# hkchengrex/Cutie

Measured on AMD Instinct MI355X. Metric: frames/sec (480p, 3 objects), higher is better.
Workload: dtype bf16

## Files before the change

cutie_amd/_lib.py:

```python
import ctypes
import os

_HERE = os.path.dirname(os.path.abspath(__file__))
LIB_PATH = os.environ.get('CUTIE_AMD_LIB') or os.path.join(_HERE, 'libcutie_hip.so')
ABI_VERSION = 11
OP_STRUCT_SIZE = 256

_lib = None


class HipLibraryError(RuntimeError):
    pass


def load():
    global _lib
    if _lib is not None:
        return _lib
    if not os.path.exists(LIB_PATH):
        raise HipLibraryError(
            f'{LIB_PATH} not found: build it with `python -c "import __graft_entry__ as g; g.build()"` '
            f'(or `make -C cutie_amd/csrc`).  cutie_amd has no CPU fallback.')
    lib = ctypes.CDLL(LIB_PATH)
    lib.cutie_exec.argtypes = [ctypes.c_void_p, ctypes.c_int, ctypes.c_void_p]
# ... 7 lines not shown
    lib.cutie_graph_destroy.argtypes = [ctypes.c_void_p]
    lib.cutie_graph_destroy.restype = None
    lib.cutie_time_ops.argtypes = [ctypes.c_void_p, ctypes.c_int, ctypes.c_int, ctypes.c_void_p]
    lib.cutie_time_ops.restype = ctypes.c_float
    lib.cutie_hip_last_error.argtypes = []
    lib.cutie_hip_last_error.restype = ctypes.c_char_p
    lib.cutie_hip_abi_version.restype = ctypes.c_int
    lib.cutie_op_struct_size.restype = ctypes.c_int
    lib.cutie_hip_build_flags.restype = ctypes.c_int
    if lib.cutie_hip_abi_version() != ABI_VERSION or lib.cutie_op_struct_size() != OP_STRUCT_SIZE:
        raise HipLibraryError(f'{LIB_PATH} is stale (ABI {lib.cutie_hip_abi_version()}, '
                              f'op size {lib.cutie_op_struct_size()}); rebuild it.')
    _lib = lib
    return lib


EXPORTED_SYMBOLS = ['cutie_exec', 'cutie_exec_one', 'cutie_graph_capture', 'cutie_graph_launch',
                    'cutie_graph_destroy', 'cutie_time_ops', 'cutie_hip_last_error',
                    'cutie_hip_abi_version', 'cutie_op_struct_size', 'cutie_hip_build_flags']


def has_diag_kernels():
    return bool(load().cutie_hip_build_flags() & 1)


def has_png_decode():
    return bool(load().cutie_hip_build_flags() & 2)


def has_jpeg_batch():
    return bool(load().cutie_hip_build_flags() & 4)


def has_mixed_lockstep():
    return bool(load().cutie_hip_build_flags() & 8)


def has_track_stats():
    return bool(load().cutie_hip_build_flags() & 16)


def has_region_filter():
    return bool(load().cutie_hip_build_flags() & 32)


def has_edt_band():
    return bool(load().cutie_hip_build_flags() & 64)


def has_polygons():
    return bool(load().cutie_hip_build_flags() & 128)


class HipExecutor:
    is_mock = False

    def __init__(self):
        import torch
        self.lib = load()
        if not torch.cuda.is_available():
            raise HipLibraryError('no HIP device visible: cutie_amd runs on MI355X only (no CPU fallback).')
        self._torch = torch
        self._raw_stream = getattr(torch._C, '_cuda_getCurrentRawStream', None)
        self.graph_stats = [0, 0]
        self._warned = False

    def stream(self):
        raw = self._raw_stream
        if raw is not None:
            return raw(self._torch.cuda.current_device())
        return self._torch.cuda.current_stream().cuda_stream

    def run(self, arr):
        rc = self.lib.cutie_exec(arr.ctypes.data, len(arr), self.stream())
        if rc != 0:
            raise RuntimeError('cutie_exec failed: ' + self.lib.cutie_hip_last_error().decode())

    def run_on(self, arr, stream):
        rc = self.lib.cutie_exec(arr.ctypes.data, len(arr), stream.cuda_stream)
        if rc != 0:
            raise RuntimeError('cutie_exec failed: ' + self.lib.cutie_hip_last_error().decode())

    GRAPH_CACHE_ENTRIES = 24

    def run_cached(self, arr, cache, head=0):
        if head:
            self.run(arr[:head])
            arr = arr[head:]
        key = arr['p'].tobytes()
        ent = cache.get(key)
        if ent is None:
            if len(cache) >= self.GRAPH_CACHE_ENTRIES:
                old = cache.pop(next(iter(cache)))
                if old not in (0, -1):
                    self.lib.cutie_graph_destroy(old)
            cache[key] = 0
            self.graph_stats[0] += 1
            return self.run(arr)
        if ent == 0:
            ent = self.lib.cutie_graph_capture(arr.ctypes.data, len(arr), self.stream()) or -1
            cache[key] = ent
            if ent == -1 and not self._warned:
                self._warned = True
                import warnings
                warnings.warn('HIP graph capture of a launch plan failed (%s); such plans keep running launch by launch'
                              % self.lib.cutie_hip_last_error().decode())
# ... 28 lines not shown
```

cutie_amd/csrc/api.hip:

```cpp
#include "common.h"
#include <stdarg.h>
#include <stdio.h>
#include <string.h>

static thread_local char g_err[512] = "";

void cutie_set_error(const char* fmt, ...) {
    va_list ap;
    va_start(ap, fmt);
    vsnprintf(g_err, sizeof(g_err), fmt, ap);
    va_end(ap);
}

static int dispatch(const cutie_op* op, hipStream_t s) {
    switch (op->kind) {
        case CUTIE_OP_CONV: return launch_conv(op, s);
        case CUTIE_OP_QUERY_INIT: return (op->flags & 1) ? launch_attention(op, s) : launch_elementwise(op, s);
        case CUTIE_OP_QFFN: return launch_qchain(op, s);
        case CUTIE_OP_STEM: return launch_stem(op, s);
        case CUTIE_OP_ATTN_Q2P: case CUTIE_OP_ATTN_SELF: case CUTIE_OP_ATTN_P2Q:
            return (op->flags & 12) ? launch_qchain(op, s) : launch_attention(op, s);
        case CUTIE_OP_AUX_MASK:
            return launch_attention(op, s);
        case CUTIE_OP_KEY_PREP: case CUTIE_OP_AFF_SCORE: case CUTIE_OP_AFF_SELECT: case CUTIE_OP_AFF_READOUT:
// ... 53 lines not shown
        if (graph) hipGraphDestroy(graph);
        if (rc == 0) cutie_set_error("graph: end capture failed (%d)", (int)e);
        (void)hipGetLastError();
        return nullptr;
    }
    hipGraphExec_t exec = nullptr;
    if (hipGraphInstantiate(&exec, graph, nullptr, nullptr, 0) != hipSuccess) {
        hipGraphDestroy(graph);
        (void)hipGetLastError();
        cutie_set_error("graph: instantiate failed");
        return nullptr;
    }
    GraphHandle* h = new GraphHandle{graph, exec};
    return h;
}

int cutie_graph_launch(void* graph, void* stream) {
    GraphHandle* h = (GraphHandle*)graph;
    if (!h) { cutie_set_error("graph: null handle"); return -4; }
    hipError_t e = hipGraphLaunch(h->exec, (hipStream_t)stream);
    if (e != hipSuccess) { cutie_set_error("graph launch: %s", hipGetErrorString(e)); return -1; }
    return 0;
}

void cutie_graph_destroy(void* graph) {
    GraphHandle* h = (GraphHandle*)graph;
    if (!h) return;
    hipGraphExecDestroy(h->exec);
    hipGraphDestroy(h->graph);
    delete h;
}

float cutie_time_ops(const cutie_op* ops, int n, int iters, void* stream) {
    hipStream_t s = (hipStream_t)stream;
    hipEvent_t a, b;
    if (hipEventCreate(&a) != hipSuccess || hipEventCreate(&b) != hipSuccess) { cutie_set_error("time: event create failed"); return -1.f; }
    if (cutie_exec(ops, n, stream) != 0) return -1.f;
    hipEventRecord(a, s);
    for (int it = 0; it < iters; ++it)
        if (cutie_exec(ops, n, stream) != 0) return -1.f;
    hipEventRecord(b, s);
    hipEventSynchronize(b);
    float ms = 0.f;
    hipEventElapsedTime(&ms, a, b);
    hipEventDestroy(a);
    hipEventDestroy(b);
    return ms / (float)iters;
}

const char* cutie_hip_last_error(void) { return g_err; }
int cutie_hip_abi_version(void) { return 11; }
int cutie_op_struct_size(void) { return (int)sizeof(cutie_op); }
int cutie_hip_build_flags(void) {
    const int forms = 2 | 4 | 8 | 16 | 32 | 64 | 128;
#ifdef CUTIE_DIAG
    return forms | 1;
#else
    return forms;
#endif
}

}
```

cutie_amd/csrc/common.h:

```cpp
#pragma once
#include <hip/hip_runtime.h>
#include <stdint.h>
#include "../../include/cutie_hip.h"

typedef unsigned short bf16_t;
typedef __attribute__((ext_vector_type(8))) __bf16 bf16x8;
typedef __attribute__((ext_vector_type(4))) float f32x4;

__device__ __forceinline__ float bf2f(bf16_t v) { return __uint_as_float(((uint32_t)v) << 16); }

typedef __attribute__((ext_vector_type(2))) __bf16 bf16x2_t;
__device__ __forceinline__ bf16_t f2bf(float f) { return __builtin_bit_cast(bf16_t, (__bf16)f); }

__device__ __forceinline__ uint32_t pack_bf2(float a, float b) {
    const bf16x2_t v = {(__bf16)a, (__bf16)b};
    return __builtin_bit_cast(uint32_t, v);
}

__device__ __forceinline__ uint32_t relu_bf2(uint32_t w) {
    uint32_t neg = (w >> 15) & 0x00010001u;
    return w & ~(neg * 0xffffu);
}

__device__ __forceinline__ float sigmoidf_(float x) { return 1.0f / (1.0f + __expf(-x)); }
// ... 19 lines not shown
    v += __builtin_amdgcn_update_dpp(0, v, 0x141, 0xf, 0xf, false);
    v += __builtin_amdgcn_update_dpp(0, v, 0x140, 0xf, 0xf, false);
    auto r = __builtin_amdgcn_permlane16_swap((unsigned)v, (unsigned)v, false, false);
    const unsigned a = r[0] + r[1];
    auto r2 = __builtin_amdgcn_permlane32_swap(a, a, false, false);
    return (int)(r2[0] + r2[1]);
}

__device__ __forceinline__ float wave_sum(float v) {
#pragma unroll
    for (int o = 32; o > 0; o >>= 1) v += __shfl_xor(v, o, 64);
    return v;
}
__device__ __forceinline__ float wave_sum_dpp(float v) {
    v += __uint_as_float(__builtin_amdgcn_update_dpp(0, (int)__float_as_uint(v), 0xB1, 0xf, 0xf, false));
    v += __uint_as_float(__builtin_amdgcn_update_dpp(0, (int)__float_as_uint(v), 0x4E, 0xf, 0xf, false));
    v += __uint_as_float(__builtin_amdgcn_update_dpp(0, (int)__float_as_uint(v), 0x141, 0xf, 0xf, false));
    v += __uint_as_float(__builtin_amdgcn_update_dpp(0, (int)__float_as_uint(v), 0x140, 0xf, 0xf, false));
    return rows_sum(v);
}
__device__ __forceinline__ float wave_max(float v) {
#pragma unroll
    for (int o = 32; o > 0; o >>= 1) v = fmaxf(v, __shfl_xor(v, o, 64));
    return v;
}

__host__ __device__ __forceinline__ int mixed_count(unsigned word, int clip) { return (int)((word >> (3 * clip)) & 7u); }
__host__ __device__ __forceinline__ int mixed_start(unsigned word, int clip) {
    int s = 0;
    for (int c = 0; c < clip; ++c) s += mixed_count(word, c);
    return s;
}
__host__ __device__ __forceinline__ int mixed_clip_of(unsigned word, int b, int& start) {
    int c = 0, s = 0;
#pragma unroll
    for (int q = 0; q < 7; ++q) {
        const int n = mixed_count(word, c);
        const bool past = b >= s + n;
        s += past ? n : 0;
        c += past ? 1 : 0;
    }
    start = s;
    return c;
}
static inline int mixed_clips(unsigned word, int* objects) {
    int n = 0, total = 0;
    if (word >> 24) { *objects = 0; return 0; }
    while (n < 8 && mixed_count(word, n)) total += mixed_count(word, n++);
    if (n < 8 && (word >> (3 * n))) { *objects = 0; return 0; }
    *objects = total;
    return n;
}

int launch_conv(const cutie_op* op, hipStream_t s);
int launch_elementwise(const cutie_op* op, hipStream_t s);
int launch_attention(const cutie_op* op, hipStream_t s);
int launch_stem(const cutie_op* op, hipStream_t s);
int launch_qchain(const cutie_op* op, hipStream_t s);
int launch_affinity(const cutie_op* op, hipStream_t s);
int launch_bank(const cutie_op* op, hipStream_t s);
int launch_resize_ingest(const cutie_op* op, hipStream_t s);
int launch_jpeg(const cutie_op* op, hipStream_t s);
int launch_png_decode(const cutie_op* op, hipStream_t s);
int launch_png_deflate(const cutie_op* op, int H, int W, hipStream_t s);
int launch_rle_encode(const cutie_op* op, hipStream_t s);
int launch_jf_counts(const cutie_op* op, hipStream_t s);
int launch_jpeg_encode(const cutie_op* op, hipStream_t s);
int launch_matte_composite(const cutie_op* op, hipStream_t s);
int launch_matte_soft(const cutie_op* op, hipStream_t s);
int launch_track_stats(const cutie_op* op, hipStream_t s);
int launch_region_filter(const cutie_op* op, hipStream_t s);
int launch_edt_band(const cutie_op* op, hipStream_t s);
int launch_polygon_trace(const cutie_op* op, hipStream_t s);
void cutie_set_error(const char* fmt, ...);
```

cutie_amd/csrc/conv_igemm.hip:

```cpp
#include "conv_common.h"

template <int BM, int BN, int WM, int WN, int BK, int S, int OCC, int WK>
__global__ __launch_bounds__(WM * WN * WK * 64) void conv_igemm_kernel(ConvParams p) {
    if (p.flags & CUTIE_F_PRIO) __builtin_amdgcn_s_setprio(1);
    constexpr int NTB = WM * WN * WK * 64;
    constexpr int NT = WM * WN * 64;
    constexpr int CPR = BK / 8;
    constexpr int RPT = NT / CPR;
    constexpr int NX = (BM * CPR) / NT;
    constexpr int NWC = (BN * CPR + NT - 1) / NT;
    constexpr int TM = BM / WM / 16;
    constexpr int TN = BN / WN / 16;
    constexpr int KSUB = BK / 32;
    constexpr int NWRAP = BK == 32 ? 4 : BK / 32;
    static_assert((NT == 256 || NT == 512) && NTB <= 1024 && NX >= 1 && TM >= 1 && TN >= 1 && S >= 2 && (BM * CPR) % NT == 0, "bad tile");
    constexpr int LDC = BN + 4;
    constexpr int GRP_CHUNKS = 2 * (BM + BN) * CPR;
    extern __shared__ __attribute__((aligned(16))) u32x4 smem_raw[];
    const int grp = threadIdx.x / NT;
    u32x4 (*smem)[(BM + BN) * CPR] = reinterpret_cast<u32x4 (*)[(BM + BN) * CPR]>(smem_raw + grp * GRP_CHUNKS);

    const int tid = threadIdx.x % NT, lane = tid & 63, wave = tid >> 6;
    int m0, n0;
    {
// ... 400 lines not shown
        if (cl == 0 && x < p.W && oy < p.H) {
            float v = acc + bias0;
            if (act == CUTIE_ACT_RELU) v = fmaxf(v, 0.f);
            else if (act == CUTIE_ACT_SIGMOID) v = sigmoidf_(v);
            else if (act == CUTIE_ACT_SQ1) v = v * v + 1.f;
            const long m = ((long)b * p.H + oy) * p.W + x;
            if (p.flags & CUTIE_F_OUT_F32) reinterpret_cast<float*>(p.y)[m * p.ldy] = v;
            else reinterpret_cast<bf16_t*>(p.y)[m * p.ldy] = f2bf(v);
        }
    }
}

template <int BM, int BN, int WM, int WN, int BK, int S, int OCC, int WK = 1>
static int launch_cfg(ConvParams p, hipStream_t s) {
    if (p.Kpad % BK) { cutie_set_error("conv: Kpad %d not a multiple of BK %d", p.Kpad, BK); return -2; }
    if (BK > 32 && p.Cin < 32) { cutie_set_error("conv: BK %d needs Cin >= 32 (Cin=%d)", BK, p.Cin); return -2; }
    const int nk_all = p.Kpad / BK;
    if (p.splitk > nk_all) { cutie_set_error("conv: splitk %d > K tiles %d", p.splitk, nk_all); return -2; }
    if (nk_all % (p.splitk * WK)) { cutie_set_error("conv: splitk %d x %d K groups must divide the %d K tiles", p.splitk, WK, nk_all); return -2; }
    p.Kslice = p.Kpad / p.splitk;
    constexpr int lds = conv_lds_bytes<BM, BN, BK, WK>();
    static bool attr_set = false;
    if (!attr_set) {
        if (lds > 65536 && hipFuncSetAttribute(reinterpret_cast<const void*>(conv_igemm_kernel<BM, BN, WM, WN, BK, S, OCC, WK>),
                                               hipFuncAttributeMaxDynamicSharedMemorySize, lds) != hipSuccess) {
            cutie_set_error("conv: cannot raise the dynamic LDS limit to %d bytes", lds);
            return -2;
        }
        attr_set = true;
    }
    dim3 grid((p.M + BM - 1) / BM, (p.Cout + BN - 1) / BN, p.splitk);
    hipLaunchKernelGGL((conv_igemm_kernel<BM, BN, WM, WN, BK, S, OCC, WK>), grid, dim3(WM * WN * WK * 64), lds, s, p);
    if (p.splitk > 1) {
        const long nq = (long)p.M * (p.ldp >> 3);
        hipLaunchKernelGGL(conv_splitk_reduce_kernel, dim3((unsigned)((nq + 255) / 256)), dim3(256), 0, s, p);
    }
    return (int)hipGetLastError();
}

int launch_conv(const cutie_op* op, hipStream_t s) {
    ConvParams p;
    p.x1 = (const bf16_t*)op->p[0]; p.x2 = (const bf16_t*)op->p[1]; p.w = (const bf16_t*)op->p[2];
    p.bias = (const float*)op->p[3]; p.res = (const bf16_t*)op->p[4]; p.y = (void*)op->p[5];
    const int32_t* i = op->i;
    p.B = i[0]; p.H = i[1]; p.W = i[2]; p.C1 = i[3]; p.C2 = i[4]; p.ldx1 = i[5]; p.ldx2 = i[6];
    p.OH = i[7]; p.OW = i[8]; p.Cout = i[9]; p.ldy = i[10]; p.KH = i[11]; p.KW = i[12];
    p.stride = i[13]; p.pad = i[14]; p.ldr = i[15]; p.Kpad = i[16];
    p.flags = op->flags; p.OHW = p.OH * p.OW; p.M = p.B * p.OHW; p.Cin = p.C1 + p.C2;
    p.splitk = i[19] > 1 ? i[19] : 1; p.part = (float*)op->p[6];
    p.ldp = (p.Cout + 7) & ~7;
    p.gap = (long long*)op->p[7]; p.zero = (unsigned long long*)op->p[8]; p.nzero = i[21];
    p.pf = (const unsigned char*)op->p[9]; p.pf_bytes = op->p[9] ? i[22] : 0;
    p.pf2 = (const unsigned char*)op->p[10]; p.pf2_bytes = op->p[10] ? i[23] : 0;
    p.res_grp_rows = p.res_grp_stride = 0;
    if ((p.flags & CUTIE_F_RES_BCAST) && op->f[0] > 0.f) {
        const int kg = (int)op->f[0];
        if (kg <= 0 || p.B % kg || op->f[1] < (float)p.OHW || op->f[1] != (float)(int)op->f[1]) { cutie_set_error("conv: residual groups of %d objects do not divide B = %d (or stride %g < OH*OW)", kg, p.B, (double)op->f[1]); return -2; }
        p.res_grp_rows = kg * p.OHW; p.res_grp_stride = (int)op->f[1];
    }
    if ((p.gap || p.zero) && (i[17] < 60 || i[17] >= 200 || ((p.flags & CUTIE_F_OUT_F32) && p.gap) || (p.Cout & 7) || (p.ldy & 7) || (p.res && (p.ldr & 7)))) {
        cutie_set_error("conv: GAP accumulation / zero job need an LDS-DMA tile (60..199), bf16 output, Cout %% 8 == 0 (tile %d)", i[17]);
        return -2;
    }
    if (p.splitk > 1 && (!p.part || (long)p.splitk * p.M * p.ldp > (long)i[20] * 1024)) {
        cutie_set_error("conv: split-K %d needs the fp32 partial scratch (p6, capacity i20 KiB-floats)", p.splitk);
        return -2;
    }
    if ((p.C1 & 7) || (p.C2 & 7) || (p.ldx1 & 7) || (p.C2 && (p.ldx2 & 7)) || (p.Kpad & 31) ||
        p.Kpad < p.KH * p.KW * p.Cin || p.M <= 0 || p.Cout <= 0) {
        cutie_set_error("conv: bad geometry C1=%d C2=%d ldx1=%d ldx2=%d Kpad=%d M=%d Cout=%d",
                        p.C1, p.C2, p.ldx1, p.ldx2, p.Kpad, p.M, p.Cout);
        return -2;
    }
    if (i[17] == 19) {
        const int LP = p.Cin >> 3;
        if (p.Cout != 1 || p.C2 != 0 || p.res || LP > 64 || (LP & (LP - 1)) || LP < 1) {
            cutie_set_error("conv cout1: needs Cout=1, single source, no residual, Cin/8 a power of two <= 64 (Cin=%d)", p.Cin);
            return -2;
        }
        const int ppb = 256 / LP;
        if (!(p.flags & CUTIE_F_PLAIN) && p.KH == 3 && p.KW == 3 && p.stride == 1 && p.pad == 1 && p.OH == p.H && p.OW == p.W && LP >= 8 && LP <= 32 && p.H * p.W >= 4096) {
            if (LP == 16 && !(p.flags & CUTIE_F_TILE_OFF)) {
                constexpr int TR = 8;
                const int blocks = p.B * ((p.H + TR - 1) / TR) * ((p.W + 15) / 16);
                hipLaunchKernelGGL(conv_cout1_tile_kernel<TR>, dim3(blocks), dim3(256), 0, s, p);
                return (int)hipGetLastError();
            }
            constexpr int R = 4;
            const int blocks = p.B * ((p.H + R - 1) / R) * ((p.W + ppb - 1) / ppb);
            hipLaunchKernelGGL(conv_cout1_rows_kernel<R>, dim3(blocks), dim3(256), 0, s, p);
            return (int)hipGetLastError();
        }
        hipLaunchKernelGGL(conv_cout1_kernel, dim3((p.M + ppb - 1) / ppb), dim3(256), (size_t)p.KH * p.KW * LP * 16, s, p);
        return (int)hipGetLastError();
    }
    if (i[17] >= 60 && i[17] < 90) return launch_conv_dma(p, i[17], s);
    if (i[17] >= 100 && i[17] < 200) return launch_conv_pc(p, i[17], s);
    switch (i[17]) {
        case 0: return launch_cfg<128, 128, 2, 2, 32, 4, 2>(p, s);
        case 1: return launch_cfg<128, 64, 2, 2, 32, 4, 3>(p, s);
        case 2: return launch_cfg<64, 64, 2, 2, 32, 4, 4>(p, s);
        case 3: return launch_cfg<256, 16, 4, 1, 32, 4, 3>(p, s);
        case 4: return launch_cfg<64, 128, 2, 2, 32, 4, 3>(p, s);
        case 5: return launch_cfg<64, 64, 2, 2, 64, 4, 3>(p, s);
        case 6: return launch_cfg<64, 128, 2, 2, 64, 3, 2>(p, s);
        case 7: return launch_cfg<128, 128, 2, 2, 64, 2, 2>(p, s);
// ... 26 lines not shown
```

cutie_amd/csrc/conv_pc.hip:

```cpp
#include "conv_common.h"

typedef __amdgpu_buffer_rsrc_t rsrc_t;
#define PC_WORD3 0x00020000
#define PC_RECORDS 0x7fffffff
#define PC_OOB 0x80000000u
#define LDS_PTR(p) ((__attribute__((address_space(3))) void*)(p))
#define PC_WAIT_VM(N) __builtin_amdgcn_s_waitcnt(((N) & 15) | (((N) >> 4) << 14) | (7 << 4) | (15 << 8))
#define PC_WAIT_LGKM0() __builtin_amdgcn_s_waitcnt(15 | (3 << 14) | (7 << 4) | (0 << 8))
#define PC_BARRIER() { asm volatile("" ::: "memory"); __builtin_amdgcn_s_barrier(); asm volatile("" ::: "memory"); }
#ifdef PC_ABL_NO_LOOPBAR
#define PC_LOOP_BARRIER() { asm volatile("" ::: "memory"); }
#else
#define PC_LOOP_BARRIER() PC_BARRIER()
#endif
#ifdef PC_ABL_NO_WAIT
#define PC_LOOP_WAIT_VM(N) ((void)0)
#else
#define PC_LOOP_WAIT_VM(N) PC_WAIT_VM(N)
#endif
#ifdef PC_ABL_SAME_TILE
#define PC_SAME_TILE_GUARD(...)
#else
#define PC_SAME_TILE_GUARD(...) __VA_ARGS__
#endif
// ... 477 lines not shown
                        case 6: if constexpr (NXP > 6) PCH_XPIECE(NXP > 6 ? 6 : 0, sl + 1) break;
                        default: if constexpr (NXP > 7) PCH_XPIECE(NXP > 7 ? 7 : 0, sl + 1) break;
                    }
                }
                PCH_WTILE()
                TL(4)
                const int xin = NS == 3 ? xp : xp + xprev;
                if (xin == 0) { PC_LOOP_WAIT_VM((NS - 2) * NWI); } else if (xin == 1) { PC_LOOP_WAIT_VM((NS - 2) * NWI + 1); } else { PC_LOOP_WAIT_VM((NS - 2) * NWI + 2); }
                TL(5)
                PC_LOOP_BARRIER()
                xprev = xp;
                ++tap;
                if (tap == 9) { tap = 0; ++sl; }
            }
            for (; kt < nk; ++kt) {
                PC_WAIT_VM(0);
                PC_LOOP_BARRIER()
            }
            } else {
            static_assert(NXP <= 8 && NP <= 3, "pair steps: two patch pieces per iteration over four iterations");
            int t = nk < NS - 1 ? nk : NS - 1;
            const int P = (nk + 1) >> 1;
            int ps = 0, pk = 0, pnext = 5;
            int u = 0;
            for (; 2 * (u + NP - 1) + 1 < nk; ++u) {
                TL(3)
                if (u == pnext) { ++ps; pk = 0; pnext += (ps & 1) ? 4 : 5; }
                if (ps + 1 < nslice && pk < 4) {
                    switch (pk) {
                        case 0: if constexpr (NXP > 0) PCH_XPIECE(0, ps + 1) if constexpr (NXP > 1) PCH_XPIECE(NXP > 1 ? 1 : 0, ps + 1) break;
                        case 1: if constexpr (NXP > 2) PCH_XPIECE(NXP > 2 ? 2 : 0, ps + 1) if constexpr (NXP > 3) PCH_XPIECE(NXP > 3 ? 3 : 0, ps + 1) break;
                        case 2: if constexpr (NXP > 4) PCH_XPIECE(NXP > 4 ? 4 : 0, ps + 1) if constexpr (NXP > 5) PCH_XPIECE(NXP > 5 ? 5 : 0, ps + 1) break;
                        default: if constexpr (NXP > 6) PCH_XPIECE(NXP > 6 ? 6 : 0, ps + 1) if constexpr (NXP > 7) PCH_XPIECE(NXP > 7 ? 7 : 0, ps + 1) break;
                    }
                    ++pk;
                }
                for (; t <= 2 * (u + NP - 1) + 1; ++t) PCH_WTILE()
                TL(4)
                PC_LOOP_WAIT_VM((NP - 2) * 2 * NWI);
                TL(5)
                PC_LOOP_BARRIER()
            }
            for (; u < P; ++u) {
                for (; t < nk && t <= 2 * (u + NP - 1) + 1; ++t) PCH_WTILE()
                PC_WAIT_VM(0);
                PC_LOOP_BARRIER()
            }
            }
#undef PCH_WTILE
#undef PCH_XPIECE
        }
        TLE(6)
        TL_DUMP(logical, nb, NC + NPW)
        if (p.pf_bytes > 0) {
            const int id = blockIdx.y * gridDim.x + blockIdx.x;
            const int nbx = (nb + 7) >> 3, kq = id >> 3;
            u32x4 t = {0u, 0u, 0u, 0u};
#pragma unroll
            for (int r = 0; r < 2; ++r) {
                const unsigned char* base = r ? p.pf2 : p.pf;
                const int bytes = r ? p.pf2_bytes : p.pf_bytes;
                const int chunk = (((bytes + nbx - 1) / nbx) + 1023) & ~1023;
                const int b0 = kq * chunk, b1 = min(b0 + chunk, bytes & ~15);
                for (int o = b0 + (pw * 64 + lane) * 16; o < b1; o += NPW * 1024)
                    asm volatile("global_load_dwordx4 %0, %1, off" : "+v"(t) : "v"(base + o) : "memory");
            }
            asm volatile("s_waitcnt vmcnt(0)" : "+v"(t) :: "memory");
        }
        return;
    }

    const int wm = wave / WN, wn = wave % WN;
    const int pm0 = wm * (BM / WM), cn0 = wn * (BN / WN);
    int mrow[TM];
    bool mval[TM];
    int xbase[TM];
#pragma unroll
    for (int b = 0; b < TM; ++b) {
        const int q = pm0 + b * 16 + l15;
        if (HALO) {
            const int qq = q < TH * TW ? q : TH * TW - 1;
            const int qy = qq / TW, qx = qq - qy * TW;
            const int gy = ty0 + qy, gx = tx0 + qx;
            mval[b] = q < TH * TW && gy < p.H && gx < p.W;
            mrow[b] = (bimg * p.H + min(gy, p.H - 1)) * p.W + min(gx, p.W - 1);
            xbase[b] = qy * PW + qx;
        } else {
            mrow[b] = m0 + q;
            mval[b] = mrow[b] < p.M;
            xbase[b] = 0;
        }
    }
    TL(11)
    const bool out_f32 = p.flags & CUTIE_F_OUT_F32;
    const bool vec_ok = (out_f32 ? (p.ldy & 3) == 0 : (p.ldy & (NCH - 1)) == 0) && (!p.res || (p.ldr & (NCH - 1)) == 0);
    float bias[TNP][NCH];
    const float* const bias_p = p.bias ? p.bias : reinterpret_cast<const float*>(p.w);
    const int bias_lim = p.bias ? p.Cout : 0;
    typedef const __attribute__((address_space(1))) float* pc_gf32;
    const pc_gf32 bias_g = (pc_gf32)bias_p;
#pragma unroll
    for (int a = 0; a < TNP; ++a) {
        const int ch0 = n0 + cn0 + a * (PAIR ? 32 : 16) + l4 * NCH;
#pragma unroll
        for (int r = 0; r < NCH; ++r) {
            const float t = bias_g[min(ch0 + r, p.Cout - 1)];
            bias[a][r] = ch0 + r < bias_lim ? t : 0.f;
        }
    }
    unsigned rpre[PRE_RES ? TM : 1][PRE_RES ? TNP : 1][NCH / 2];
    const bool have_res = PRE_RES && p.res && vec_ok;
    if (PRE_RES) {
#pragma unroll
        for (int b = 0; b < TM; ++b)
#pragma unroll
            for (int a = 0; a < TNP; ++a) {
                const int ch0 = n0 + cn0 + a * (PAIR ? 32 : 16) + l4 * NCH;
#pragma unroll
                for (int r = 0; r < NCH / 2; ++r) rpre[b][a][r] = 0u;
                if (have_res && mval[b] && ch0 + NCH <= p.Cout) {
                    const int mres = pc_res_row(p, mrow[b]);
// ... 289 lines not shown
```

cutie_amd/csrc/elementwise.hip:

```cpp
#include "common.h"
#include <math.h>

#define GRID1D(n, bs) dim3((unsigned)(((long)(n) + (bs) - 1) / (bs)))
__global__ void memset32_kernel(uint32_t* d, long n, uint32_t v);

__global__ void maxpool_kernel(const uint4* __restrict__ x, uint4* __restrict__ y, int B, int H, int W, int C8,
                               int OH, int OW, int relu) {
    long idx = (long)blockIdx.x * blockDim.x + threadIdx.x;
    long total = (long)B * OH * OW * C8;
    if (idx >= total) return;
    int c = idx % C8; long t = idx / C8;
    int ow = t % OW; t /= OW; int oh = t % OH; int b = t / OH;
    float m[8];
#pragma unroll
    for (int i = 0; i < 8; ++i) m[i] = relu ? 0.f : -INFINITY;
    for (int dy = 0; dy < 3; ++dy) {
        int ih = oh * 2 - 1 + dy;
        if ((unsigned)ih >= (unsigned)H) continue;
        for (int dx = 0; dx < 3; ++dx) {
            int iw = ow * 2 - 1 + dx;
            if ((unsigned)iw >= (unsigned)W) continue;
            uint4 v = x[(((long)b * H + ih) * W + iw) * C8 + c];
            uint32_t u[4] = {v.x, v.y, v.z, v.w};
#pragma unroll
            for (int i = 0; i < 4; ++i) {
                m[2 * i] = fmaxf(m[2 * i], __uint_as_float(u[i] << 16));
                m[2 * i + 1] = fmaxf(m[2 * i + 1], __uint_as_float(u[i] & 0xffff0000u));
            }
        }
    }
    y[idx] = make_uint4(pack_bf2(m[0], m[1]), pack_bf2(m[2], m[3]), pack_bf2(m[4], m[5]), pack_bf2(m[6], m[7]));
}

__global__ void img_prep_kernel(const float* __restrict__ img, const float* __restrict__ masks, uint4* __restrict__ y,
                                int h0, int w0, int H, int W, int pl, int pt, int K,
                                float m0, float m1, float m2, float s0, float s1, float s2) {
    long idx = (long)blockIdx.x * blockDim.x + threadIdx.x;
    long HW = (long)H * W;
    if (idx >= HW * K) return;
    int k = idx / HW; long pix = idx - (long)k * HW;
    int yy = pix / W, xx = pix - (long)yy * W;
    int sy = yy - pt, sx = xx - pl;
    float r = 0.f, g = 0.f, b = 0.f;
    if ((unsigned)sy < (unsigned)h0 && (unsigned)sx < (unsigned)w0) {
        long o = (long)sy * w0 + sx, plane = (long)h0 * w0;
        r = img[o]; g = img[plane + o]; b = img[2 * plane + o];
    }
    r = (r - m0) / s0; g = (g - m1) / s1; b = (b - m2) / s2;
    float mk = 0.f, others = 0.f;
    if (masks) {
        float sum = 0.f;
        for (int j = 0; j < K; ++j) sum += masks[(long)j * HW + pix];
        mk = masks[(long)k * HW + pix];
        others = fminf(fmaxf(sum - mk, 0.f), 1.f);
    }
    y[idx] = make_uint4(pack_bf2(r, g), pack_bf2(b, mk), pack_bf2(others, 0.f), 0u);
}

__device__ __forceinline__ void up_coord(int o, int n_in, float scale, int& i0, int& i1, float& lam) {
    float src = ((float)o + 0.5f) * scale - 0.5f;
    if (src < 0.f) src = 0.f;
    i0 = (int)src;
    if (i0 > n_in - 1) i0 = n_in - 1;
    i1 = i0 + (i0 < n_in - 1 ? 1 : 0);
    lam = src - (float)i0;
}

template <bool MIXED = false>
__global__ void upsample2x_add_kernel(const uint4* __restrict__ g, const uint4* __restrict__ skip, uint4* __restrict__ y,
                                      int B, int h, int w, int C8, int Kg, long gstride, int prio) {
    if (prio) __builtin_amdgcn_s_setprio(1);
    long idx = (long)blockIdx.x * blockDim.x + threadIdx.x;
    int OH = 2 * h, OW = 2 * w;
    long total = (long)B * OH * OW * C8;
    if (idx >= total) return;
    int c = idx % C8; long t = idx / C8;
    int ox = t % OW; t /= OW; int oy = t % OH; int b = t / OH;
    int y0, y1, x0, x1; float ly, lx;
    up_coord(oy, h, 0.5f, y0, y1, ly);
    up_coord(ox, w, 0.5f, x0, x1, lx);
    const uint4* gb = g + (long)b * h * w * C8;
    uint4 v00 = gb[((long)y0 * w + x0) * C8 + c], v01 = gb[((long)y0 * w + x1) * C8 + c];
    uint4 v10 = gb[((long)y1 * w + x0) * C8 + c], v11 = gb[((long)y1 * w + x1) * C8 + c];
    long grp;
    if (MIXED) { int st; grp = mixed_clip_of((unsigned)Kg, b, st); }
    else grp = Kg > 0 ? b / Kg : 0;
    uint4 sk = skip[(grp * gstride + (long)oy * OW + ox) * C8 + c];
    const uint32_t* a = &v00.x; const uint32_t* bq = &v01.x; const uint32_t* cq = &v10.x; const uint32_t* d = &v11.x;
    const uint32_t* s = &sk.x;
    float w00 = (1.f - ly) * (1.f - lx), w01 = (1.f - ly) * lx, w10 = ly * (1.f - lx), w11 = ly * lx;
    uint32_t out[4];
#pragma unroll
    for (int i = 0; i < 4; ++i) {
        float lo = w00 * __uint_as_float(a[i] << 16) + w01 * __uint_as_float(bq[i] << 16) +
                   w10 * __uint_as_float(cq[i] << 16) + w11 * __uint_as_float(d[i] << 16) + __uint_as_float(s[i] << 16);
        float hi = w00 * __uint_as_float(a[i] & 0xffff0000u) + w01 * __uint_as_float(bq[i] & 0xffff0000u) +
                   w10 * __uint_as_float(cq[i] & 0xffff0000u) + w11 * __uint_as_float(d[i] & 0xffff0000u) +
                   __uint_as_float(s[i] & 0xffff0000u);
        out[i] = pack_bf2(lo, hi);
    }
    y[idx] = make_uint4(out[0], out[1], out[2], out[3]);
}

template <int R = 0>
__device__ __forceinline__ void area_down_bf16_body(const bf16_t* __restrict__ x, bf16_t* __restrict__ y, int B, int H, int W, int C,
                                                    int ldx, int ldy, int rrt, long idx) {
    const int r = R > 0 ? R : rrt;
    int C8 = C >> 3, OH = H / r, OW = W / r;
    long total = (long)B * OH * OW * C8;
    if (idx >= total) return;
    int c = idx % C8; long t = idx / C8;
    int ox = t % OW; t /= OW; int oy = t % OH; int b = t / OH;
    float acc[8] = {0, 0, 0, 0, 0, 0, 0, 0};
    if (R > 0) {
        uint4 v[R > 0 ? R * R : 1];
#pragma unroll
        for (int dy = 0; dy < R; ++dy)
#pragma unroll
            for (int dx = 0; dx < R; ++dx)
                v[dy * R + dx] = *reinterpret_cast<const uint4*>(x + (((long)b * H + oy * R + dy) * W + ox * R + dx) * ldx + c * 8);
#pragma unroll
        for (int e = 0; e < R * R; ++e) {
            const uint32_t* u = &v[e].x;
#pragma unroll
            for (int i = 0; i < 4; ++i) {
                acc[2 * i] += __uint_as_float(u[i] << 16);
                acc[2 * i + 1] += __uint_as_float(u[i] & 0xffff0000u);
            }
        }
    } else
    for (int dy = 0; dy < r; ++dy)
        for (int dx = 0; dx < r; ++dx) {
            const uint4 v = *reinterpret_cast<const uint4*>(x + (((long)b * H + oy * r + dy) * W + ox * r + dx) * ldx + c * 8);
            const uint32_t* u = &v.x;
#pragma unroll
            for (int i = 0; i < 4; ++i) {
                acc[2 * i] += __uint_as_float(u[i] << 16);
                acc[2 * i + 1] += __uint_as_float(u[i] & 0xffff0000u);
            }
        }
    float inv = 1.f / (float)(r * r);
    uint4 o = make_uint4(pack_bf2(acc[0] * inv, acc[1] * inv), pack_bf2(acc[2] * inv, acc[3] * inv),
                         pack_bf2(acc[4] * inv, acc[5] * inv), pack_bf2(acc[6] * inv, acc[7] * inv));
    *reinterpret_cast<uint4*>(y + (((long)b * OH + oy) * OW + ox) * ldy + c * 8) = o;
}
__global__ void area_down_bf16_kernel(const bf16_t* __restrict__ x, bf16_t* __restrict__ y, int B, int H, int W, int C,
                                      int ldx, int ldy, int r) {
    area_down_bf16_body(x, y, B, H, W, C, ldx, ldy, r, (long)blockIdx.x * blockDim.x + threadIdx.x);
}

template <int R = 0>
__device__ __forceinline__ void area_down_f32_body(const float* __restrict__ x, bf16_t* __restrict__ y, int B, int H, int W, int C,
                                                   int ldx, int ldy, int rrt, int Cz, long idx) {
    const int r = R > 0 ? R : rrt;
    int OH = H / r, OW = W / r;
    long total = (long)B * OH * OW;
    if (idx >= total) return;
    int ox = idx % OW; long t = idx / OW; int oy = t % OH; int b = t / OH;
    float inv = 1.f / (float)(r * r);
    bf16_t* yp = y + idx * ldy;
    for (int c = 0; c < C; ++c) {
        float acc = 0.f;
        if (R > 0) {
            float v[R > 0 ? R * R : 1];
#pragma unroll
            for (int dy = 0; dy < R; ++dy)
#pragma unroll
                for (int dx = 0; dx < R; ++dx) v[dy * R + dx] = x[(((long)b * H + oy * R + dy) * W + ox * R + dx) * ldx + c];
#pragma unroll
            for (int e = 0; e < R * R; ++e) acc += v[e];
        } else
        for (int dy = 0; dy < r; ++dy)
            for (int dx = 0; dx < r; ++dx) acc += x[(((long)b * H + oy * r + dy) * W + ox * r + dx) * ldx + c];
        yp[c] = f2bf(acc * inv);
    }
    for (int c = C; c < Cz; ++c) yp[c] = 0;
}
__global__ void area_down_f32_kernel(const float* __restrict__ x, bf16_t* __restrict__ y, int B, int H, int W, int C,
                                     int ldx, int ldy, int r, int Cz) {
    area_down_f32_body(x, y, B, H, W, C, ldx, ldy, r, Cz, (long)blockIdx.x * blockDim.x + threadIdx.x);
}
struct AreaSeg { const void* x; bf16_t* y; int B, H, W, C, ldx, ldy, r, Cz, f32; long n; };
struct Area3 { AreaSeg s[3]; int rt; int prio; };
__global__ void area_down3_kernel(Area3 a) {
    const int prio = a.prio;
    if (prio) __builtin_amdgcn_s_setprio(1);
    long idx = (long)blockIdx.x * blockDim.x + threadIdx.x;
#pragma unroll
    for (int q = 0; q < 3; ++q) {
        const AreaSeg& g = a.s[q];
        if (idx < g.n) {
            const int rr = a.rt ? 0 : g.r;
            if (g.f32) {
                if (rr == 2) area_down_f32_body<2>((const float*)g.x, g.y, g.B, g.H, g.W, g.C, g.ldx, g.ldy, 2, g.Cz, idx);
                else if (rr == 4) area_down_f32_body<4>((const float*)g.x, g.y, g.B, g.H, g.W, g.C, g.ldx, g.ldy, 4, g.Cz, idx);
                else area_down_f32_body<0>((const float*)g.x, g.y, g.B, g.H, g.W, g.C, g.ldx, g.ldy, g.r, g.Cz, idx);
            } else {
                if (rr == 2) area_down_bf16_body<2>((const bf16_t*)g.x, g.y, g.B, g.H, g.W, g.C, g.ldx, g.ldy, 2, idx);
                else if (rr == 4) area_down_bf16_body<4>((const bf16_t*)g.x, g.y, g.B, g.H, g.W, g.C, g.ldx, g.ldy, 4, idx);
                else area_down_bf16_body<0>((const bf16_t*)g.x, g.y, g.B, g.H, g.W, g.C, g.ldx, g.ldy, g.r, idx);
            }
            return;
        }
        idx -= g.n;
    }
}

__global__ void mask_down_mean_kernel(const float* __restrict__ m, float* __restrict__ m16, int K, int H, int W, int r) {
    int h = H / r, w = W / r;
    long idx = (long)blockIdx.x * (blockDim.x >> 6) + (threadIdx.x >> 6);
    int lane = threadIdx.x & 63;
    if (idx >= (long)K * h * w) return;
    int ox = idx % w; long t = idx / w; int oy = t % h; int k = t / h;
    float acc = 0.f;
    for (int e = lane; e < r * r; e += 64) {
        int dy = e / r, dx = e - dy * r;
        acc += m[((long)k * H + oy * r + dy) * W + ox * r + dx];
    }
    acc = wave_sum(acc);
    if (lane == 0) m16[idx] = acc / (float)(r * r);
}
__global__ void mask_down_pair_kernel(const float* __restrict__ m, float* __restrict__ m16, uint4* __restrict__ y, int K, int H, int W, int r,
                                      int ld8) {
    const int h = H / r, w = W / r, hw = h * w;
    const long px = (long)blockIdx.x * (blockDim.x >> 6) + (threadIdx.x >> 6);
    const int lane = threadIdx.x & 63;
    if (px >= hw) return;
    const int ox = px % w, oy = px / w;
    float sum = 0.f;
    for (int k0 = 0; k0 < K; k0 += 4) {
        float acc[4] = {0.f, 0.f, 0.f, 0.f};
        for (int e = lane; e < r * r; e += 64) {
            const int dy = e / r, dx = e - dy * r;
            float v[4];
#pragma unroll
            for (int u = 0; u < 4; ++u) v[u] = m[((long)min(k0 + u, K - 1) * H + oy * r + dy) * W + ox * r + dx];
#pragma unroll
            for (int u = 0; u < 4; ++u) acc[u] += v[u];
        }
#pragma unroll
        for (int u = 0; u < 4; ++u) {
            if (k0 + u >= K) break;
            const float a = wave_sum(acc[u]) / (float)(r * r);
            sum += a;
            if (lane == 0) m16[(long)(k0 + u) * hw + px] = a;
        }
    }
    if (lane == 0)
        for (int k = 0; k < K; ++k) {
            const float mk = m16[(long)k * hw + px];
            const float others = fminf(fmaxf(sum - mk, 0.f), 1.f);
            y[((long)k * hw + px) * ld8] = make_uint4(pack_bf2(mk, others), 0u, 0u, 0u);
        }
}
__global__ void mask_pair_kernel(const float* __restrict__ m16, uint4* __restrict__ y, int K, int hw) {
    long idx = (long)blockIdx.x * blockDim.x + threadIdx.x;
    if (idx >= (long)K * hw) return;
    int k = idx / hw; int p = idx - (long)k * hw;
    float sum = 0.f;
    for (int j = 0; j < K; ++j) sum += m16[(long)j * hw + p];
    float mk = m16[idx];
    float others = fminf(fmaxf(sum - mk, 0.f), 1.f);
    y[idx] = make_uint4(pack_bf2(mk, others), 0u, 0u, 0u);
}

__global__ __launch_bounds__(256) void gap_partial_kernel(const bf16_t* __restrict__ x, float* __restrict__ part, int HW, int C) {
    __shared__ float red[2048 + 32];
    const int b = blockIdx.y, p0 = blockIdx.x * 64;
    const int C8 = C >> 3;
    const int c8 = threadIdx.x % C8, rg = threadIdx.x / C8, nrg = 256 / C8;
    float acc[8] = {0, 0, 0, 0, 0, 0, 0, 0};
    for (int r = rg; r < 64; r += nrg) {
        int p = p0 + r;
        if (p < HW) {
            uint4 v = *reinterpret_cast<const uint4*>(x + ((long)b * HW + p) * C + c8 * 8);
            acc[0] += __uint_as_float(v.x << 16); acc[1] += __uint_as_float(v.x & 0xffff0000u);
            acc[2] += __uint_as_float(v.y << 16); acc[3] += __uint_as_float(v.y & 0xffff0000u);
            acc[4] += __uint_as_float(v.z << 16); acc[5] += __uint_as_float(v.z & 0xffff0000u);
            acc[6] += __uint_as_float(v.w << 16); acc[7] += __uint_as_float(v.w & 0xffff0000u);
        }
    }
#pragma unroll
    for (int i = 0; i < 8; ++i) red[rg * (C + 1) + c8 * 8 + i] = acc[i];
    __syncthreads();
    for (int c = threadIdx.x; c < C; c += 256) {
        float sum = 0.f;
        for (int g = 0; g < nrg; ++g) sum += red[g * (C + 1) + c];
        part[((long)b * gridDim.x + blockIdx.x) * C + c] = sum;
    }
}
__global__ void gap_final_kernel(const float* __restrict__ part, float* __restrict__ y, int nchunk, int C, float inv) {
    const int b = blockIdx.x;
    for (int c = threadIdx.x; c < C; c += blockDim.x) {
        float sum = 0.f;
        for (int k = 0; k < nchunk; ++k) sum += part[((long)b * nchunk + k) * C + c];
        y[(long)b * C + c] = sum * inv;
    }
}

__global__ __launch_bounds__(256) void eca_apply_kernel(const bf16_t* __restrict__ x, const float* __restrict__ part,
                                                        const float* __restrict__ wk, const bf16_t* __restrict__ r,
                                                        bf16_t* __restrict__ y, float* __restrict__ gap_out, int HW, int C, int nchunk,
                                                        const long long* __restrict__ fixed, const bf16_t* __restrict__ pw,
                                                        const float* __restrict__ pb, float* __restrict__ plog, int prio) {
    if (prio) __builtin_amdgcn_s_setprio(1);
    __shared__ float gap[256 + 4], sc[256];
    const int b = blockIdx.y, tid = threadIdx.x;
    const float inv = 1.f / (float)HW;
    const int C8 = C >> 3;
    const int p0 = blockIdx.x * 32;
    uint4 xv[4], rv[4];
    long offs[4];
#pragma unroll
    for (int it = 0; it < 4; ++it) {
        const int q = tid + it * 256;
        const int pp = q / C8, c8 = q - pp * C8, p = p0 + pp;
        const bool ok = q < 32 * C8 && p < HW;
        offs[it] = ok ? ((long)b * HW + p) * C + c8 * 8 : -1;
        const long o = ok ? offs[it] : 0;
        xv[it] = *reinterpret_cast<const uint4*>(x + o);
        rv[it] = *reinterpret_cast<const uint4*>(r + o);
    }
    if (fixed) {
        for (int c = tid; c < C; c += 256) {
            const float mean = (float)((double)fixed[(long)b * C + c] * (1.0 / 16777216.0)) * inv;
            gap[c + 2] = mean;
            if (gap_out && blockIdx.x == 0) gap_out[(long)b * C + c] = mean;
        }
    } else
    for (int c = tid; c < C; c += 256) {
        float sum = 0.f;
        for (int k0 = 0; k0 < nchunk; k0 += 8) {
            float v[8];
#pragma unroll
            for (int u = 0; u < 8; ++u) v[u] = part[((long)b * nchunk + min(k0 + u, nchunk - 1)) * C + c];
#pragma unroll
            for (int u = 0; u < 8; ++u) sum += k0 + u < nchunk ? v[u] : 0.f;
        }
        gap[c + 2] = sum * inv;
        if (gap_out && blockIdx.x == 0) gap_out[(long)b * C + c] = sum * inv;
    }
    if (tid < 2) { gap[tid] = 0.f; gap[C + 2 + tid] = 0.f; }
    __syncthreads();
    for (int c = tid; c < C; c += 256) {
        float a = wk[0] * gap[c] + wk[1] * gap[c + 1] + wk[2] * gap[c + 2] + wk[3] * gap[c + 3] + wk[4] * gap[c + 4];
        sc[(c & 7) * 32 + (c >> 3)] = sigmoidf_(a);
    }
    __syncthreads();
#pragma unroll
    for (int it = 0; it < 4; ++it) {
        if (offs[it] < 0) continue;
        const int q = tid + it * 256;
        const int c8 = q % C8;
        const uint32_t* xu = &xv[it].x; const uint32_t* ru = &rv[it].x;
        uint32_t o[4];
#pragma unroll
        for (int i = 0; i < 4; ++i) {
            float lo = __uint_as_float(xu[i] << 16) * sc[(2 * i) * 32 + c8] + __uint_as_float(ru[i] << 16);
            float hi = __uint_as_float(xu[i] & 0xffff0000u) * sc[(2 * i + 1) * 32 + c8] + __uint_as_float(ru[i] & 0xffff0000u);
            o[i] = pack_bf2(lo, hi);
        }
        *reinterpret_cast<uint4*>(y + offs[it]) = make_uint4(o[0], o[1], o[2], o[3]);
    }
    if (pw) {
        const int c8 = tid & 31;
        const uint4 wv = *reinterpret_cast<const uint4*>(pw + c8 * 8);
        const uint32_t* wu = &wv.x;
        const float bias = pb ? pb[0] : 0.f;
#pragma unroll
        for (int it = 0; it < 4; ++it) {
            float part = 0.f;
            if (offs[it] >= 0) {
                const uint32_t* xu = &xv[it].x; const uint32_t* ru = &rv[it].x;
#pragma unroll
                for (int i = 0; i < 4; ++i) {
                    const float lo = __uint_as_float(xu[i] << 16) * sc[(2 * i) * 32 + c8] + __uint_as_float(ru[i] << 16);
                    const float hi = __uint_as_float(xu[i] & 0xffff0000u) * sc[(2 * i + 1) * 32 + c8] + __uint_as_float(ru[i] & 0xffff0000u);
                    const uint32_t st = pack_bf2(lo, hi);
                    part += fmaxf(__uint_as_float(st << 16), 0.f) * __uint_as_float(wu[i] << 16);
                    part += fmaxf(__uint_as_float(st & 0xffff0000u), 0.f) * __uint_as_float(wu[i] & 0xffff0000u);
                }
            }
            part += __uint_as_float(__builtin_amdgcn_update_dpp(0, (int)__float_as_uint(part), 0xB1, 0xf, 0xf, false));
            part += __uint_as_float(__builtin_amdgcn_update_dpp(0, (int)__float_as_uint(part), 0x4E, 0xf, 0xf, false));
            part += __uint_as_float(__builtin_amdgcn_update_dpp(0, (int)__float_as_uint(part), 0x141, 0xf, 0xf, false));
            part += __uint_as_float(__builtin_amdgcn_update_dpp(0, (int)__float_as_uint(part), 0x140, 0xf, 0xf, false));
            const unsigned pu = __float_as_uint(part);
            const auto rr = __builtin_amdgcn_permlane16_swap(pu, pu, false, false);
            const float tot = __uint_as_float(rr[0]) + __uint_as_float(rr[1]);
            const int q = tid + it * 256, p = p0 + q / C8;
            if (c8 == 0 && offs[it] >= 0) plog[(long)b * HW + p] = tot + bias;
        }
    }
}

__global__ void gru4_kernel(const float* __restrict__ v, float* __restrict__ h, bf16_t* __restrict__ hb, long n, int C, int prio) {
    if (prio) __builtin_amdgcn_s_setprio(1);
    const long idx = (long)blockIdx.x * blockDim.x + threadIdx.x;
    const int C4 = C >> 2;
    if (idx >= n * C4) return;
    const long row = idx / C4; const int c = (int)(idx - row * C4) * 4;
    const float* vr = v + row * 3 * C + c;
    const float4 f4 = *reinterpret_cast<const float4*>(vr), u4 = *reinterpret_cast<const float4*>(vr + C), n4 = *reinterpret_cast<const float4*>(vr + 2 * C);
    const float4 h4 = *reinterpret_cast<const float4*>(h + row * C + c);
    const float fa[4] = {f4.x, f4.y, f4.z, f4.w}, ua[4] = {u4.x, u4.y, u4.z, u4.w}, na[4] = {n4.x, n4.y, n4.z, n4.w}, ha[4] = {h4.x, h4.y, h4.z, h4.w};
    float o[4];
#pragma unroll
    for (int i = 0; i < 4; ++i) {
        const float f = sigmoidf_(fa[i]), u = sigmoidf_(ua[i]), nv = tanhf(na[i]);
        o[i] = f * ha[i] * (1.f - u) + u * nv;
    }
    *reinterpret_cast<float4*>(h + row * C + c) = make_float4(o[0], o[1], o[2], o[3]);
    *reinterpret_cast<uint2*>(hb + row * C + c) = make_uint2(pack_bf2(o[0], o[1]), pack_bf2(o[2], o[3]));
}

__global__ void gru_kernel(const float* __restrict__ v, float* __restrict__ h, bf16_t* __restrict__ hb, long n, int C) {
    long idx = (long)blockIdx.x * blockDim.x + threadIdx.x;
    if (idx >= n * C) return;
    long row = idx / C; int c = idx - row * C;
    const float* vr = v + row * 3 * C;
    float f = sigmoidf_(vr[c]), u = sigmoidf_(vr[C + c]), nv = tanhf(vr[2 * C + c]);
    float nh = f * h[idx] * (1.f - u) + u * nv;
    h[idx] = nh;
    hb[idx] = f2bf(nh);
}

__device__ __forceinline__ float clamp_logit(float p) {
    p = fminf(fmaxf(p, 1e-7f), 1.f - 1e-7f);
    return logf(p / (1.f - p));
}

__global__ void seg_agg_kernel(const float* __restrict__ lg, float* __restrict__ agg, int K, int hw) {
    int p = blockIdx.x * blockDim.x + threadIdx.x;
    if (p >= hw) return;
    float bg = 1.f;
    for (int k = 0; k < K; ++k) {
        float pr = 1.f / (1.f + expf(-lg[(long)k * hw + p]));
        bg *= (1.f - pr);
        agg[(long)(k + 1) * hw + p] = clamp_logit(pr);
    }
    agg[p] = clamp_logit(bg);
}

__global__ void up4_softmax_kernel(const float* __restrict__ agg, float* __restrict__ prob, float* __restrict__ lup,
                                   int P, int h, int w) {
    int OH = 4 * h, OW = 4 * w;
    long idx = (long)blockIdx.x * blockDim.x + threadIdx.x;
    if (idx >= (long)OH * OW) return;
    int ox = idx % OW, oy = idx / OW;
    int y0, y1, x0, x1; float ly, lx;
    up_coord(oy, h, 0.25f, y0, y1, ly);
    up_coord(ox, w, 0.25f, x0, x1, lx);
    float w00 = (1.f - ly) * (1.f - lx), w01 = (1.f - ly) * lx, w10 = ly * (1.f - lx), w11 = ly * lx;
    long o00 = (long)y0 * w + x0, o01 = (long)y0 * w + x1, o10 = (long)y1 * w + x0, o11 = (long)y1 * w + x1;
    long hw = (long)h * w, OHW = (long)OH * OW;
    float mx = -INFINITY;
    for (int c = 0; c < P; ++c) {
        const float* a = agg + c * hw;
        float v = w00 * a[o00] + w01 * a[o01] + w10 * a[o10] + w11 * a[o11];
        if (lup) lup[c * OHW + idx] = v;
        mx = fmaxf(mx, v);
    }
    float sum = 0.f;
    for (int c = 0; c < P; ++c) {
        const float* a = agg + c * hw;
        float v = w00 * a[o00] + w01 * a[o01] + w10 * a[o10] + w11 * a[o11];
// ... 214 lines not shown
    float lo[PMAX][4];
    if (SH) {
        if (lane < 36) {
            const int sly = lane / 6, slx = lane - sly * 6;
            const long o = (long)min(max(4 * cy - 1 + sly, 0), h - 1) * w + min(max(4 * cx - 1 + slx, 0), w - 1);
            float raw[PMAX - 1], Lp[PMAX];
#pragma unroll
            for (int k = 0; k < PMAX - 1; ++k)
                if (k < K) raw[k] = lg[(long)k * h * w + o];
            up4_src<PMAX>(raw, K, Lp);
#pragma unroll
            for (int p = 0; p < PMAX; ++p)
                if (p <= K) srcw[p * 36 + lane] = Lp[p];
        }
        __builtin_amdgcn_wave_barrier();
        __builtin_amdgcn_s_waitcnt(0xc07f);
        __builtin_amdgcn_wave_barrier();
    }
    up4_four<PMAX, KC, SH>(lg, K, h, w, oy, j, out, lo, srcw, 4 * cy - 1, 4 * cx - 1);
    const long base = (long)oy * OW + 4 * j;
#pragma unroll
    for (int p = 0; p < PMAX; ++p)
        if (p <= K) {
            if (lup) *reinterpret_cast<float4*>(lup + p * OHW + base) = make_float4(lo[p][0], lo[p][1], lo[p][2], lo[p][3]);
            *reinterpret_cast<float4*>(prob + p * OHW + base) = make_float4(out[p][0], out[p][1], out[p][2], out[p][3]);
            if (p >= 1) *reinterpret_cast<float4*>(&cellw[(p - 1) * 256 + r * 16 + 4 * q4]) = make_float4(out[p][0], out[p][1], out[p][2], out[p][3]);
        }
    __builtin_amdgcn_wave_barrier();
    __builtin_amdgcn_s_waitcnt(0xc07f);
    float sum = 0.f, mk[PMAX - 1];
#pragma unroll
    for (int k = 0; k < PMAX - 1; ++k)
        if (k < K) {
            float acc = 0.f;
#pragma unroll
            for (int i = 0; i < 4; ++i) acc += cellw[k * 256 + lane + 64 * i];
            const float a = wave_sum(acc) / 256.f;
            sum += a;
            mk[k] = a;
        }
    if (lane == 0) {
#pragma unroll
        for (int k = 0; k < PMAX - 1; ++k)
            if (k < K) {
                m16[(long)k * ncell + cid] = mk[k];
                const float others = fminf(fmaxf(sum - mk[k], 0.f), 1.f);
                pair[((long)k * ncell + cid) * ld8] = make_uint4(pack_bf2(mk[k], others), 0u, 0u, 0u);
            }
    }
}

template <int PMAX, int KC = 0, bool SH = false>
__global__ __launch_bounds__(256) void up4_softmax_md_kernel(const float* __restrict__ lg, float* __restrict__ prob, float* __restrict__ lup,
                                                             int Krt, int h, int w, float* __restrict__ m16, uint4* __restrict__ pair, int ld8, int prio) {
    if (prio) __builtin_amdgcn_s_setprio(1);
    const int K = KC > 0 ? KC : Krt;
    __shared__ float cell[4][PMAX - 1][256];
    __shared__ float srcL[4][SH ? PMAX : 1][36];
    const int OH = 4 * h, OW = 4 * w, ch = OH >> 4, cw = OW >> 4, ncell = ch * cw;
    const int wave = threadIdx.x >> 6, lane = threadIdx.x & 63;
    const int cid = blockIdx.x * 4 + wave;
    if (cid >= ncell) return;
    {
        const long cl = blockIdx.y;
        lg += cl * K * h * w; prob += cl * (K + 1) * (long)OH * OW;
        if (lup) lup += cl * (K + 1) * (long)OH * OW;
        m16 += cl * K * ncell; pair += cl * K * ncell * ld8;
    }
    const int cy = cid / cw, cx = cid - cy * cw;
    const int r = lane >> 2, q4 = lane & 3;
    const int oy = cy * 16 + r, j = cx * 4 + q4;
    const long OHW = (long)OH * OW;
    float out[PMAX][4];
    float lo[PMAX][4];
    if (SH) {
        if (lane < 36) {
            const int sly = lane / 6, slx = lane - sly * 6;
            const long o = (long)min(max(4 * cy - 1 + sly, 0), h - 1) * w + min(max(4 * cx - 1 + slx, 0), w - 1);
            float raw[PMAX - 1], Lp[PMAX];
#pragma unroll
            for (int k = 0; k < PMAX - 1; ++k)
                if (k < K) raw[k] = lg[(long)k * h * w + o];
            up4_src<PMAX>(raw, K, Lp);
#pragma unroll
            for (int p = 0; p < PMAX; ++p)
                if (p <= K) srcL[wave][SH ? p : 0][lane] = Lp[p];
        }
        __builtin_amdgcn_wave_barrier();
        __builtin_amdgcn_s_waitcnt(0xc07f);
        __builtin_amdgcn_wave_barrier();
    }
    up4_four<PMAX, KC, SH>(lg, K, h, w, oy, j, out, lo, &srcL[wave][0][0], 4 * cy - 1, 4 * cx - 1);
    const long base = (long)oy * OW + 4 * j;
#pragma unroll
    for (int p = 0; p < PMAX; ++p)
        if (p <= K) {
            if (lup) *reinterpret_cast<float4*>(lup + p * OHW + base) = make_float4(lo[p][0], lo[p][1], lo[p][2], lo[p][3]);
            *reinterpret_cast<float4*>(prob + p * OHW + base) = make_float4(out[p][0], out[p][1], out[p][2], out[p][3]);
            if (p >= 1) *reinterpret_cast<float4*>(&cell[wave][p - 1][r * 16 + 4 * q4]) = make_float4(out[p][0], out[p][1], out[p][2], out[p][3]);
        }
    __builtin_amdgcn_wave_barrier();
    __builtin_amdgcn_s_waitcnt(0xc07f);
    float sum = 0.f, mk[PMAX - 1];
#pragma unroll
    for (int k = 0; k < PMAX - 1; ++k)
        if (k < K) {
            float acc = 0.f;
#pragma unroll
            for (int i = 0; i < 4; ++i) acc += cell[wave][k][lane + 64 * i];
            const float a = wave_sum(acc) / 256.f;
            sum += a;
            mk[k] = a;
        }
    if (lane == 0) {
#pragma unroll
        for (int k = 0; k < PMAX - 1; ++k)
            if (k < K) {
                m16[(long)k * ncell + cid] = mk[k];
                const float others = fminf(fmaxf(sum - mk[k], 0.f), 1.f);
                pair[((long)k * ncell + cid) * ld8] = make_uint4(pack_bf2(mk[k], others), 0u, 0u, 0u);
            }
    }
}

template <int PMAX, bool SH>
__global__ __launch_bounds__(256) void up4_softmax_md_mixed_kernel(const float* __restrict__ lg, float* __restrict__ prob, float* __restrict__ lup,
                                                                   unsigned counts, int h, int w, float* __restrict__ m16, uint4* __restrict__ pair, int ld8, int prio) {
    if (prio) __builtin_amdgcn_s_setprio(1);
    __shared__ float cell[4][PMAX - 1][256];
    __shared__ float srcL[4][SH ? PMAX : 1][36];
    const int cl = blockIdx.y, Kc = mixed_count(counts, cl), st = mixed_start(counts, cl);
    const long ncell = (long)(h >> 2) * (w >> 2), OHW = (long)16 * h * w;
    lg += (long)st * h * w; prob += (long)(st + cl) * OHW;
    if (lup) lup += (long)(st + cl) * OHW;
    m16 += (long)st * ncell; pair += (long)st * ncell * ld8;
    const int wave = threadIdx.x >> 6;
#define UP4_BODY_(KC) up4_md_body<PMAX, KC, SH>(lg, prob, lup, KC, h, w, m16, pair, ld8, &cell[wave][0][0], &srcL[wave][0][0])
    UP4_MIXED_SWITCH(UP4_BODY_)
#undef UP4_BODY_
}

__global__ void mask_merge_kernel(const void* __restrict__ inmask, const float* __restrict__ pred, const int* __restrict__ src,
                                  float* __restrict__ planes, int h0, int w0, int H, int W, int pl, int pt, int Knew,
                                  int Kold, int nfloat, int fmode) {
    long idx = (long)blockIdx.x * blockDim.x + threadIdx.x;
    long HW = (long)H * W;
    if (idx >= HW) return;
    int yy = idx / W, xx = idx - (long)yy * W;
    int sy = yy - pt, sx = xx - pl;
    bool inside = (unsigned)sy < (unsigned)h0 && (unsigned)sx < (unsigned)w0;
    long so = (long)sy * w0 + sx, plane = (long)h0 * w0;
    int iv = 0; bool covered = false;
    if (!fmode) {
        iv = inside ? ((const int*)inmask)[so] : 0;
        covered = iv > 0;
    } else {
        float mx = 0.f;
        if (inside) { mx = -INFINITY; for (int c = 0; c < nfloat; ++c) mx = fmaxf(mx, ((const float*)inmask)[c * plane + so]); }
        covered = mx > 0.5f;
    }
    for (int t = 0; t < Knew; ++t) {
        int s = src[t];
        float v;
        if (s >= 0) {
            if (!fmode) v = (iv == s) ? 1.f : 0.f;
            else v = inside ? ((const float*)inmask)[s * plane + so] : 0.f;
        } else {
            v = (pred && t < Kold && !covered) ? pred[(long)(t + 1) * HW + idx] : 0.f;
        }
        planes[(long)t * HW + idx] = v;
    }
}

__global__ void agg_softmax_kernel(const float* __restrict__ planes, float* __restrict__ prob, int K, long HW) {
    long p = (long)blockIdx.x * blockDim.x + threadIdx.x;
// ... 453 lines not shown
            for (int k = 0; k < 4; ++k) {
                const int ox = min(ox0 + k, OW - 1);
                const float fx = fmaxf((ox + 0.5f) * sx - 0.5f, 0.f);
                const int x0 = min((int)fx, W - 1), x1 = min(x0 + 1, W - 1);
                const float lx = fx - (float)x0;
                const float a = r0[x0], b = r0[x1], cc = r1[x0], d = r1[x1];
                const float v = (1.f - ly) * ((1.f - lx) * a + lx * b) + ly * ((1.f - lx) * cc + lx * d);
                sum[k] += (int)(uint8_t)(int)(v * 255.f);
            }
        }
#pragma unroll
        for (int k = 0; k < 4; ++k)
            if (q == 0 || sum[k] > best[k]) { best[k] = sum[k]; arg[k] = q; }
    }
    OUT* o = out + (long)oy * OW + ox0;
    if constexpr (sizeof(OUT) == 1) {
        if (packed) {
            *(uint32_t*)o = (uint32_t)(uint8_t)lut[arg[0]] | (uint32_t)(uint8_t)lut[arg[1]] << 8 | (uint32_t)(uint8_t)lut[arg[2]] << 16 |
                            (uint32_t)(uint8_t)lut[arg[3]] << 24;
            return;
        }
    } else {
        if (packed) {
            *(int4*)o = make_int4(lut[arg[0]], lut[arg[1]], lut[arg[2]], lut[arg[3]]);
            return;
        }
    }
#pragma unroll
    for (int k = 0; k < 4; ++k)
        if (ox0 + k < OW) o[k] = (OUT)lut[arg[k]];
}

int launch_elementwise(const cutie_op* op, hipStream_t s) {
    const int32_t* i = op->i;
    const uint64_t* p = op->p;
    const int BS = 256;
    const int PRIO = (op->flags & CUTIE_F_PRIO) ? 1 : 0;
    switch (op->kind) {
        case CUTIE_OP_MAXPOOL: {
            int C8 = i[3] / 8;
            long n = (long)i[0] * i[4] * i[5] * C8;
            hipLaunchKernelGGL(maxpool_kernel, GRID1D(n, BS), dim3(BS), 0, s, (const uint4*)p[0], (uint4*)p[1], i[0], i[1], i[2], C8, i[4], i[5], op->flags & 1);
            break;
        }
        case CUTIE_OP_IMG_PREP: {
            int K = p[1] ? i[6] : 1;
            long n = (long)i[2] * i[3] * K;
            hipLaunchKernelGGL(img_prep_kernel, GRID1D(n, BS), dim3(BS), 0, s, (const float*)p[0], (const float*)p[1], (uint4*)p[2],
                               i[0], i[1], i[2], i[3], i[4], i[5], K, op->f[0], op->f[1], op->f[2], op->f[3], op->f[4], op->f[5]);
            break;
        }
        case CUTIE_OP_UPSAMPLE2X_ADD: {
            int C8 = i[3] / 8;
            long n = (long)i[0] * 4 * i[1] * i[2] * C8;
            if (i[6]) {
                int objs; const int nc = mixed_clips((unsigned)i[6], &objs);
                if (nc < 1 || objs != i[0] || i[4] != 0 || i[5] < 4 * i[1] * i[2]) { cutie_set_error("upsample2x_add (mixed form): the counts 0x%x do not add up to B = %d (or i4 != 0, or the stride is below one map)", i[6], i[0]); return -2; }
                hipLaunchKernelGGL(upsample2x_add_kernel<true>, GRID1D(n, BS), dim3(BS), 0, s, (const uint4*)p[0], (const uint4*)p[1], (uint4*)p[2], i[0], i[1], i[2], C8, i[6], (long)i[5], PRIO);
                break;
            }
            if (i[4] < 0 || (i[4] > 0 && (i[0] % i[4] || i[5] < 4 * i[1] * i[2]))) { cutie_set_error("upsample2x_add: skip groups of %d objects do not divide B = %d (or their stride is below one map)", i[4], i[0]); return -2; }
            hipLaunchKernelGGL(upsample2x_add_kernel<false>, GRID1D(n, BS), dim3(BS), 0, s, (const uint4*)p[0], (const uint4*)p[1], (uint4*)p[2], i[0], i[1], i[2], C8, i[4], (long)i[5], PRIO);
            break;
        }
        case CUTIE_OP_AREA_DOWN: {
            int r = i[6];
            long np = (long)i[0] * (i[1] / r) * (i[2] / r);
            if (op->flags & 1)
                hipLaunchKernelGGL(area_down_f32_kernel, GRID1D(np, BS), dim3(BS), 0, s, (const float*)p[0], (bf16_t*)p[1], i[0], i[1], i[2], i[3], i[4], i[5], r, i[7]);
            else
                hipLaunchKernelGGL(area_down_bf16_kernel, GRID1D(np * (i[3] / 8), BS), dim3(BS), 0, s, (const bf16_t*)p[0], (bf16_t*)p[1], i[0], i[1], i[2], i[3], i[4], i[5], r);
            break;
        }
        case CUTIE_OP_AREA_DOWN3: {
            Area3 a;
            long total = 0;
            for (int q = 0; q < 3; ++q) {
                const int32_t* j = i + 8 * q;
                AreaSeg& g = a.s[q];
                g.x = (const void*)p[2 * q]; g.y = (bf16_t*)p[2 * q + 1];
                g.B = j[0]; g.H = j[1]; g.W = j[2]; g.C = j[3]; g.ldx = j[4]; g.ldy = j[5]; g.r = j[6]; g.Cz = j[7];
                g.f32 = (op->flags >> q) & 1;
                if (g.r < 1 || (!g.f32 && (g.C & 7))) { cutie_set_error("area_down3: segment %d: r >= 1, C %% 8 for bf16 input", q); return -2; }
                const long np = (long)g.B * (g.H / g.r) * (g.W / g.r);
                g.n = g.f32 ? np : np * (g.C / 8);
                total += g.n;
            }
            a.rt = (op->flags >> 3) & 1;
            a.prio = PRIO;
            hipLaunchKernelGGL(area_down3_kernel, GRID1D(total, BS), dim3(BS), 0, s, a);
            break;
        }
        case CUTIE_OP_MASK_DOWN: {
            int K = i[0], r = i[3], h = i[1] / r, w = i[2] / r;
            long n = (long)K * h * w;
            float* m16 = (float*)p[2];
            if (!m16) { cutie_set_error("mask_down: m16 buffer required"); return -2; }
            hipLaunchKernelGGL(mask_down_pair_kernel, GRID1D((long)h * w * 64, BS), dim3(BS), 0, s, (const float*)p[0], m16, (uint4*)p[1], K, i[1], i[2], r,
                               i[4] > 8 ? i[4] / 8 : 1);
            break;
        }
        case CUTIE_OP_GAP: {
            if (i[2] > 256 || (i[2] & 7) || 256 % (i[2] / 8)) { cutie_set_error("gap: C must divide 256 octet-wise (C=%d)", i[2]); return -2; }
            if (!p[2]) { cutie_set_error("gap: scratch buffer required"); return -2; }
            int nchunk = (i[1] + 63) / 64;
            hipLaunchKernelGGL(gap_partial_kernel, dim3(nchunk, i[0]), dim3(256), 0, s, (const bf16_t*)p[0], (float*)p[2], i[1], i[2]);
            if (!(op->flags & 1))
                hipLaunchKernelGGL(gap_final_kernel, dim3(i[0]), dim3(256), 0, s, (const float*)p[2], (float*)p[1], nchunk, i[2], 1.f / (float)i[1]);
            break;
        }
        case CUTIE_OP_ECA_APPLY: {
            if (i[2] > 256 || (i[2] & 7)) { cutie_set_error("eca: C <= 256, C %% 8"); return -2; }
            if (p[6] && (i[2] != 256 || !p[8])) { cutie_set_error("eca: the fused 1x1 head needs C = 256 and an output"); return -2; }
            int nchunk = (i[1] + 63) / 64;
            hipLaunchKernelGGL(eca_apply_kernel, dim3((i[1] + 31) / 32, i[0]), dim3(256), 0, s, (const bf16_t*)p[0], (const float*)p[5], (const float*)p[2],
                               (const bf16_t*)p[3], (bf16_t*)p[4], (float*)p[1], i[1], i[2], nchunk, (op->flags & 1) ? (const long long*)p[5] : nullptr,
                               (const bf16_t*)p[6], (const float*)p[7], (float*)p[8], PRIO);
            break;
        }
        case CUTIE_OP_GRU: {
            long n = (long)i[0] * i[1];
            if (!(op->flags & 1) && (i[1] & 3) == 0 && (((uintptr_t)p[0] | (uintptr_t)p[1]) & 15) == 0 && ((uintptr_t)p[2] & 7) == 0)
                hipLaunchKernelGGL(gru4_kernel, GRID1D(n / 4, BS), dim3(BS), 0, s, (const float*)p[0], (float*)p[1], (bf16_t*)p[2], (long)i[0], i[1], PRIO);
            else
                hipLaunchKernelGGL(gru_kernel, GRID1D(n, BS), dim3(BS), 0, s, (const float*)p[0], (float*)p[1], (bf16_t*)p[2], (long)i[0], i[1]);
            break;
        }
        case CUTIE_OP_SEG_AGG:
            hipLaunchKernelGGL(seg_agg_kernel, GRID1D(i[1], BS), dim3(BS), 0, s, (const float*)p[0], (float*)p[1], i[0], i[1]);
            break;
        case CUTIE_OP_UP4_SOFTMAX: {
            long n = (long)16 * i[1] * i[2];
            if (op->flags & 1) {
                if (i[0] > 16) { cutie_set_error("up4_softmax: the fused form holds P <= 16 planes in registers (P=%d)", i[0]); return -2; }
                const bool vec = !(op->flags & 2) && i[0] <= 8 && (((uintptr_t)p[1] | (uintptr_t)p[2]) & 15) == 0;
                const int nclip = i[4] > 1 ? i[4] : 1;
                if (nclip > 1 && !vec) { cutie_set_error("up4_softmax: several clips per launch need the four-pixel form (P <= 8, aligned outputs)"); return -2; }
                if (i[5]) {
                    int objs; const int nc = mixed_clips((unsigned)i[5], &objs);
                    if (nc < 1 || nc != i[4] || !vec || (op->flags & 8)) { cutie_set_error("up4_softmax (mixed form): %d clips in the counts 0x%x, i4 = %d; needs the four-pixel form with compile-time object counts", nc, i[5], i[4]); return -2; }
                    if (op->flags & 4) {
                        if (!p[3] || !p[4] || (i[1] & 3) || (i[2] & 3) || i[3] < 8 || (i[3] & 7)) { cutie_set_error("up4_softmax: the mask-down form needs h, w multiples of 4, m16 and pair"); return -2; }
                        const int ncell = (i[1] / 4) * (i[2] / 4);
                        if (op->flags & 16)
                            hipLaunchKernelGGL((up4_softmax_md_mixed_kernel<8, false>), dim3((ncell + 3) / 4, nc), dim3(256), 0, s, (const float*)p[0], (float*)p[1], (float*)p[2], (unsigned)i[5],
                                               i[1], i[2], (float*)p[3], (uint4*)p[4], i[3] / 8, PRIO);
                        else
                            hipLaunchKernelGGL((up4_softmax_md_mixed_kernel<8, true>), dim3((ncell + 3) / 4, nc), dim3(256), 0, s, (const float*)p[0], (float*)p[1], (float*)p[2], (unsigned)i[5],
                                               i[1], i[2], (float*)p[3], (uint4*)p[4], i[3] / 8, PRIO);
                    } else {
                        const long n4 = (long)4 * i[1] * i[2];
                        hipLaunchKernelGGL(up4_softmax_fused4_mixed_kernel<8>, dim3((unsigned)((n4 + BS - 1) / BS), nc), dim3(BS), 0, s, (const float*)p[0], (float*)p[1], (float*)p[2], (unsigned)i[5], i[1], i[2], PRIO);
                    }
                    break;
                }
                if (op->flags & 4) {
                    if (!vec || !p[3] || !p[4] || (i[1] & 3) || (i[2] & 3) || i[3] < 8 || (i[3] & 7)) { cutie_set_error("up4_softmax: the mask-down form needs P <= 8, h, w multiples of 4, m16 and pair"); return -2; }
                    const int ncell = (i[1] / 4) * (i[2] / 4);
#define UP4_MD_(KC, SH) hipLaunchKernelGGL((up4_softmax_md_kernel<8, KC, SH>), dim3((ncell + 3) / 4, nclip), dim3(256), 0, s, (const float*)p[0], (float*)p[1], (float*)p[2], i[0] - 1, \
                                       i[1], i[2], (float*)p[3], (uint4*)p[4], i[3] / 8, PRIO)
#define UP4_MD(KC) { if (op->flags & 16) UP4_MD_(KC, false); else UP4_MD_(KC, true); }
                    switch ((op->flags & 8) ? 0 : i[0] - 1) {
                        case 1: UP4_MD(1); break; case 2: UP4_MD(2); break; case 3: UP4_MD(3); break; case 4: UP4_MD(4); break;
                        case 5: UP4_MD(5); break; case 6: UP4_MD(6); break; case 7: UP4_MD(7); break; default: UP4_MD(0); break;
                    }
#undef UP4_MD
#undef UP4_MD_
                    break;
                }
                if (vec) {
                    const long n4 = (long)4 * i[1] * i[2];
#define UP4_F4(KC) hipLaunchKernelGGL((up4_softmax_fused4_kernel<8, KC>), dim3((unsigned)((n4 + BS - 1) / BS), nclip), dim3(BS), 0, s, (const float*)p[0], (float*)p[1], (float*)p[2], i[0] - 1, i[1], i[2], PRIO)
                    switch ((op->flags & 8) ? 0 : i[0] - 1) {
                        case 1: UP4_F4(1); break; case 2: UP4_F4(2); break; case 3: UP4_F4(3); break; case 4: UP4_F4(4); break;
                        case 5: UP4_F4(5); break; case 6: UP4_F4(6); break; case 7: UP4_F4(7); break; default: UP4_F4(0); break;
                    }
#undef UP4_F4
                    break;
                }
                if (i[0] <= 8) hipLaunchKernelGGL(up4_softmax_fused_kernel<8>, GRID1D(n, BS), dim3(BS), 0, s, (const float*)p[0], (float*)p[1], (float*)p[2], i[0] - 1, i[1], i[2]);
                else hipLaunchKernelGGL(up4_softmax_fused_kernel<16>, GRID1D(n, BS), dim3(BS), 0, s, (const float*)p[0], (float*)p[1], (float*)p[2], i[0] - 1, i[1], i[2]);
                break;
            }
            hipLaunchKernelGGL(up4_softmax_kernel, GRID1D(n, BS), dim3(BS), 0, s, (const float*)p[0], (float*)p[1], (float*)p[2], i[0], i[1], i[2]);
            break;
        }
        case CUTIE_OP_MASK_MERGE: {
            long n = (long)i[2] * i[3];
            hipLaunchKernelGGL(mask_merge_kernel, GRID1D(n, BS), dim3(BS), 0, s, (const void*)p[0], (const float*)p[1], (const int*)p[2], (float*)p[3],
                               i[0], i[1], i[2], i[3], i[4], i[5], i[6], i[7], i[8], op->flags & 1);
            break;
        }
        case CUTIE_OP_AGG_SOFTMAX:
            hipLaunchKernelGGL(agg_softmax_kernel, GRID1D(i[1], BS), dim3(BS), 0, s, (const float*)p[0], (float*)p[1], i[0], (long)i[1]);
            break;
        case CUTIE_OP_LINEAR: {
            if ((i[2] & 7) || (i[3] & 3) || i[2] < 256) { cutie_set_error("linear: Kd %% 8, ldx %% 4, Kd >= 256 required (Kd=%d)", i[2]); return -2; }
            const int add_rows = i[5] > 0 ? i[5] : 1;
            const bool ln = op->flags & 2;
            if (ln && (i[2] != 256 || !p[6] || !p[7] || (i[3] & 3))) { cutie_set_error("linear: fused LayerNorm needs Kd == 256, gamma and beta"); return -2; }
            if ((ln || i[6] > 0) && (i[2] & 127)) { cutie_set_error("linear: LayerNorm / add_cols need Kd %% 128 == 0"); return -2; }
            if (i[6] > 0 && (i[6] & 15)) { cutie_set_error("linear: add_cols must be a multiple of 16"); return -2; }
            if ((i[2] & 511) == 0 && i[2] >= 1024 && !ln)
                hipLaunchKernelGGL(linear_mfma_kernel<16>, dim3((i[1] + 15) / 16, (i[0] + 15) / 16), dim3(1024), 0, s, (const float*)p[0], (const float*)p[1], (const bf16_t*)p[2],
                                   (const float*)p[3], (const float*)p[4], (float*)p[5], i[0], i[1], i[2], i[3], i[4], add_rows, op->flags & 1, i[6],
                                   (const float*)nullptr, (const float*)nullptr, (float*)nullptr, 1e-5f);
            else if ((i[2] & 127) == 0)
                hipLaunchKernelGGL(linear_mfma_kernel<4>, dim3((i[1] + 15) / 16, (i[0] + 15) / 16), dim3(256), 0, s, (const float*)p[0], (const float*)p[1], (const bf16_t*)p[2],
                                   (const float*)p[3], (const float*)p[4], (float*)p[5], i[0], i[1], i[2], i[3], i[4], add_rows, op->flags & 1, i[6],
                                   ln ? (const float*)p[6] : nullptr, (const float*)p[7], (float*)p[8], op->f[0] > 0.f ? op->f[0] : 1e-5f);
            else if (i[2] >= 512)
                hipLaunchKernelGGL(linear_small_kernel<64>, dim3((i[1] + 3) / 4, (i[0] + 15) / 16), dim3(256), 0, s, (const float*)p[0], (const float*)p[1], (const bf16_t*)p[2],
                                   (const float*)p[3], (const float*)p[4], (float*)p[5], i[0], i[1], i[2], i[3], i[4], add_rows, op->flags & 1);
// ... 161 lines not shown
```

cutie_amd/csrc/qchain.hip:

```cpp
#include "attention_common.h"

#define QACC_SCALE 4294967296.f
#define QACC_INV (1.f / 4294967296.f)

struct QIn {
    const float* x;
    const long long* acc;
    const float* abias;
    const float* add;
    const float* ln_g; const float* ln_b;
    float* ln_out;
    float* x_out;
    const bf16_t* W; const float* bias;
    unsigned long long* tl;
    int prio;
};
struct QOut { const bf16_t* W; long long* acc; };

#ifdef ATT_TIMELINE
#define ATL(ID) { if (in.tl && (threadIdx.x & 63) == 0) { unsigned long long* o_ = in.tl + ((((long)blockIdx.z * gridDim.y + blockIdx.y) * gridDim.x + blockIdx.x) * 16 + (threadIdx.x >> 6)) * 16; \
                  o_[ID] = __builtin_readcyclecounter(); if ((ID) == 0) o_[14] = wall_clock64(); else o_[15] = wall_clock64(); } }
#else
#define ATL(ID)
#endif
// ... 60 lines not shown
#pragma unroll
    for (int j = 0; j < 4; ++j) { uint32_t h_, l_; split_bf2(v[2 * j], v[2 * j + 1], h_, l_); hi[j] = h_; lo[j] = l_; }
}
__device__ __forceinline__ void split4(const float* v, proj_u4& hi, proj_u4& lo) {
#pragma unroll
    for (int j = 0; j < 2; ++j) { uint32_t h_, l_; split_bf2(v[2 * j], v[2 * j + 1], h_, l_); hi[j] = h_; lo[j] = l_; }
    hi[2] = hi[3] = lo[2] = lo[3] = 0u;
}

#define Q2C_PF 4
#define Q2C_VLD 40
struct Q2CChunk { q2p_u32x4 k[2], v[2]; };
__device__ __forceinline__ void q2c_load(Q2CChunk& L, const bf16_t* __restrict__ kvb, int p0, int HW, int ldkv, int voff, int lane) {
    const int c16 = lane & 15, g = lane >> 4;
#pragma unroll
    for (int t = 0; t < 2; ++t) {
        const int p = min(p0 + t * 16 + c16, HW - 1);
        L.k[t] = *reinterpret_cast<const q2p_u32x4*>(kvb + (long)p * ldkv + 8 * g);
    }
    const bf16_t* vp = kvb + (long)min(p0 + (lane >> 1), HW - 1) * ldkv + voff + (lane & 1) * 16;
    L.v[0] = *reinterpret_cast<const q2p_u32x4*>(vp);
    L.v[1] = *reinterpret_cast<const q2p_u32x4*>(vp + 8);
}

template <int KT>
__device__ __forceinline__ bool aux_fg_vals(const float* v, int K, int k) {
    float bg = 1.f, mx = 0.f, mine_l = 0.f;
#pragma unroll
    for (int j = 0; j < KT; ++j) {
        const float pr = __frcp_rn(1.f + __expf(-v[j]));
        bg *= j < K ? (1.f - pr) : 1.f;
        mx = fmaxf(mx, j < K ? pr : 0.f);
        mine_l = j == k ? v[j] : mine_l;
    }
    const float lo = 1e-7f, hi = 1.f - 1e-7f;
    const float mine = fminf(fmaxf(__frcp_rn(1.f + __expf(-mine_l)), lo), hi);
    return mine >= fminf(fmaxf(mx, lo), hi) && mine >= fminf(fmaxf(bg, lo), hi);
}
__device__ __forceinline__ bool aux_fg_late(const float* __restrict__ lg, int K, int HW, int k, int p) {
    float bg = 1.f, mx = 0.f, mine = 0.f;
    for (int j = 0; j < K; ++j) {
        const float pr = __frcp_rn(1.f + __expf(-lg[(long)j * HW + p]));
        bg *= (1.f - pr);
        mx = fmaxf(mx, pr);
        mine = j == k ? pr : mine;
    }
    const float lo = 1e-7f, hi = 1.f - 1e-7f;
    mine = fminf(fmaxf(mine, lo), hi);
    return mine >= fminf(fmaxf(mx, lo), hi) && mine >= fminf(fmaxf(bg, lo), hi);
}

template <bool QPRE, bool ACC, int KT, int NW, bool MIXED = false>
__global__ __launch_bounds__(NW * 64) void q2p_chain_kernel(QIn in, QOut out, const bf16_t* __restrict__ kv, const float* __restrict__ lg,
                                                           int HW, int HWp, int ldkv, int voff, int hstride, const float* __restrict__ qpre, int Kg) {
    if (in.prio) __builtin_amdgcn_s_setprio(1);
    constexpr int Q = 16, NT = NW * 64;
    constexpr bool EARLY = KT > 0;
    constexpr int PPT = 2048 / NT;
    constexpr int UPW = 16 / NW;
    constexpr int SO_BYTES = NW * 16 * 33 * 4, ST_BYTES = 16 * PROJ_XLD * 4 + NW * 64 * 16;
    __shared__ __attribute__((aligned(16))) unsigned char sbuf[SO_BYTES > ST_BYTES ? SO_BYTES : ST_BYTES];
    float (*sO)[16][33] = reinterpret_cast<float (*)[16][33]>(sbuf);
    __shared__ float sM[NW][16], sL[NW][16];
    __shared__ float sQ[16][33];
    __shared__ int sCnt;
    extern __shared__ uint8_t dynlds[];
    const int hh = blockIdx.x, k = blockIdx.y;
    int K, kin;
    if (MIXED) {
        int st;
        const int cl = mixed_clip_of((unsigned)Kg, k, st);
        K = mixed_count((unsigned)Kg, cl); kin = k - st;
    } else {
        K = Kg; kin = k % Kg;
    }
    lg += (long)(k - kin) * HW;
    const int wave = threadIdx.x >> 6, lane = threadIdx.x & 63;
    const int c16 = lane & 15, g = lane >> 4;
    uint8_t* sFg = dynlds;
    bf16_t* sV = reinterpret_cast<bf16_t*>(dynlds + HWp) + wave * 32 * Q2C_VLD;
    const float scale = rsqrtf(32.f);
    ATL(0)
    QRows<UPW> R;
    float4 qp0, qp1;
    if (QPRE) {
        const float* qr = qpre + ((long)k * 16 + c16) * 256 + hh * 32 + 8 * g;
        qp0 = *reinterpret_cast<const float4*>(qr); qp1 = *reinterpret_cast<const float4*>(qr + 4);
    } else {
        qrows_issue<NW, UPW, ACC, true, true>(in, k, R);
    }
    float lgv[EARLY ? PPT : 1][EARLY ? KT : 1];
    if (EARLY) {
#pragma unroll
        for (int i = 0; i < PPT; ++i) {
            const int p = min((int)threadIdx.x + NT * i, HW - 1);
#pragma unroll
            for (int j = 0; j < KT; ++j) lgv[i][j] = lg[(long)min(j, K - 1) * HW + p];
        }
    }
    const int tile = wave & 1, ks0 = (wave >> 1) * UPW;
    proj_u4 wq[UPW], wo[UPW];
    if (!QPRE) proj16_load<UPW>(in.W, hh * 32 + tile * 16, ks0, wq);
#pragma unroll
    for (int t = 0; t < UPW; ++t) proj16_load<1>(out.W, (wave * UPW + t) * 16, hh, &wo[t]);
    const bf16_t* kvb = kv + (long)k * HW * ldkv + hh * hstride;
    const int nchunk = (HW + 31) >> 5;
    if (threadIdx.x == 0) sCnt = 0;
// ... 99 lines not shown
        o0 = __builtin_amdgcn_mfma_f32_16x16x32_bf16(va0.b, ph.b, o0, 0, 0, 0);
        o0 = __builtin_amdgcn_mfma_f32_16x16x32_bf16(va0.b, pl.b, o0, 0, 0, 0);
        o1 = __builtin_amdgcn_mfma_f32_16x16x32_bf16(va1.b, ph.b, o1, 0, 0, 0);
        o1 = __builtin_amdgcn_mfma_f32_16x16x32_bf16(va1.b, pl.b, o1, 0, 0, 0);
    };
#pragma unroll
    for (int j = 0; j < Q2C_PF; ++j)
        if (wave + NW * j < nchunk) chunk(pf[j], (wave + NW * j) * 32);
    for (int ch = wave + NW * Q2C_PF; ch < nchunk; ch += NW) {
        Q2CChunk L;
        q2c_load(L, kvb, ch * 32, HW, ldkv, voff, lane);
        chunk(L, ch * 32);
    }
    ATL(3)
    l = rows_sum(l);
    if (g == 0) { sM[wave][c16] = m; sL[wave][c16] = l; }
#pragma unroll
    for (int r = 0; r < 4; ++r) { sO[wave][c16][4 * g + r] = o0[r]; sO[wave][c16][16 + 4 * g + r] = o1[r]; }
    QSYNC();
    ATL(4)
    for (int e = threadIdx.x; e < 512; e += NT) {
        const int i = e >> 5, d = e & 31;
        float Mg = -INFINITY;
#pragma unroll
        for (int w = 0; w < NW; ++w) Mg = fmaxf(Mg, sM[w][i]);
        float num = 0.f, den = 0.f;
#pragma unroll
        for (int w = 0; w < NW; ++w) {
            const float f = (sM[w][i] == -INFINITY) ? 0.f : __expf(sM[w][i] - Mg);
            num += sO[w][i][d] * f;
            den += sL[w][i] * f;
        }
        sQ[i][d] = num / den;
    }
    QSYNC();
    ATL(5)
    {
        proj_u4 hi, lo;
#pragma unroll
        for (int j = 0; j < 4; ++j) { uint32_t h_, l_; split_bf2(sQ[c16][8 * g + 2 * j], sQ[c16][8 * g + 2 * j + 1], h_, l_); hi[j] = h_; lo[j] = l_; }
#pragma unroll
        for (int t = 0; t < UPW; ++t) {
            f32x4 acc = {0.f, 0.f, 0.f, 0.f};
            acc = __builtin_amdgcn_mfma_f32_16x16x32_bf16(as_frag(lo), as_frag(wo[t]), acc, 0, 0, 0);
            acc = __builtin_amdgcn_mfma_f32_16x16x32_bf16(as_frag(hi), as_frag(wo[t]), acc, 0, 0, 0);
            long long* ap = out.acc + ((long)k * 16 + 4 * g) * 256 + (wave * UPW + t) * 16 + c16;
#pragma unroll
            for (int r = 0; r < 4; ++r) qacc_add(ap + r * 256, acc[r]);
        }
    }
    ATL(6)
}

__global__ __launch_bounds__(512) void self_chain_kernel(QIn in, QOut out) {
    if (in.prio) __builtin_amdgcn_s_setprio(1);
    __shared__ float sX[2][16 * PROJ_XLD];
    __shared__ f32x4 sRed[4][6][64];
    __shared__ float sP[3][16][33];
    const int hh = blockIdx.x, k = blockIdx.y, lane = threadIdx.x & 63, wave = threadIdx.x >> 6, c = lane & 15, g = lane >> 4;
    const int kq = wave & 3, th = wave >> 2;
    const float scale = rsqrtf(32.f);
    ATL(0)
    QRows<2> R;
    qrows_issue<8, 2, true, true, true>(in, k, R);
    proj_u4 wv[3][2];
#pragma unroll
    for (int t = 0; t < 3; ++t) { const int tl_ = th * 3 + t; proj16_load<2>(in.W, (tl_ >> 1) * 256 + hh * 32 + (tl_ & 1) * 16, 2 * kq, wv[t]); }
    proj_u4 wo[2];
#pragma unroll
    for (int t = 0; t < 2; ++t) {
        const bf16_t* wr = out.W + (long)((wave * 2 + t) * 16 + c) * 256 + hh * 32 + 4 * g;
        const uint2 a = *reinterpret_cast<const uint2*>(wr), b = *reinterpret_cast<const uint2*>(wr + 16);
        wo[t][0] = a.x; wo[t][1] = a.y; wo[t][2] = b.x; wo[t][3] = b.y;
    }
    qrows_finish<8, 2, true, true, true>(in, k, R, sX[0], sX[1], hh == 0);
    ATL(1)
    QSYNC();
#pragma unroll
    for (int t = 0; t < 3; ++t) sRed[kq][th * 3 + t][lane] = proj16_mma<2>(sX[th * 3 + t < 4 ? 0 : 1], 2 * kq, wv[t]);
    QSYNC();
    ATL(2)
    if (threadIdx.x < 6 * 64) {
        const int t = threadIdx.x >> 6;
        f32x4 a = sRed[0][t][lane];
#pragma unroll
        for (int w = 1; w < 4; ++w) { const f32x4 b = sRed[w][t][lane]; a[0] += b[0]; a[1] += b[1]; a[2] += b[2]; a[3] += b[3]; }
        const int col = (t & 1) * 16 + c;
        const float bv = in.bias[(t >> 1) * 256 + hh * 32 + col];
#pragma unroll
        for (int r = 0; r < 4; ++r) sP[t >> 1][4 * g + r][col] = (a[r] + bv) * (t < 2 ? scale : 1.f);
    }
    QSYNC();
    ATL(3)
    float kf[8], qf[8];
#pragma unroll
    for (int j = 0; j < 8; ++j) { kf[j] = sP[1][c][8 * g + j]; qf[j] = sP[0][c][8 * g + j]; }
    proj_u4 khi, klo, qhi, qlo;
    split8(kf, khi, klo);
    split8(qf, qhi, qlo);
    f32x4 s = {0.f, 0.f, 0.f, 0.f};
    s = mfma3(khi, klo, qhi, qlo, s);
    const float mx = rows_max(fmaxf(fmaxf(s[0], s[1]), fmaxf(s[2], s[3])));
    float pe[4];
#pragma unroll
    for (int r = 0; r < 4; ++r) pe[r] = __expf(s[r] - mx);
    const float inv = 1.f / rows_sum((pe[0] + pe[1]) + (pe[2] + pe[3]));
#pragma unroll
    for (int r = 0; r < 4; ++r) pe[r] *= inv;
    proj_u4 phi, plo;
    split4(pe, phi, plo);
    float ot[2][4];
#pragma unroll
    for (int dt = 0; dt < 2; ++dt) {
        float vf[4];
#pragma unroll
        for (int j = 0; j < 4; ++j) vf[j] = sP[2][4 * g + j][dt * 16 + c];
        proj_u4 vhi, vlo;
        split4(vf, vhi, vlo);
        f32x4 o = {0.f, 0.f, 0.f, 0.f};
        o = mfma3(vhi, vlo, phi, plo, o);
#pragma unroll
        for (int r = 0; r < 4; ++r) ot[dt][r] = o[r];
    }
    ATL(4)
    {
        const float of[8] = {ot[0][0], ot[0][1], ot[0][2], ot[0][3], ot[1][0], ot[1][1], ot[1][2], ot[1][3]};
        proj_u4 ohi, olo;
        split8(of, ohi, olo);
#pragma unroll
        for (int t = 0; t < 2; ++t) {
            f32x4 acc = {0.f, 0.f, 0.f, 0.f};
            acc = __builtin_amdgcn_mfma_f32_16x16x32_bf16(as_frag(olo), as_frag(wo[t]), acc, 0, 0, 0);
            acc = __builtin_amdgcn_mfma_f32_16x16x32_bf16(as_frag(ohi), as_frag(wo[t]), acc, 0, 0, 0);
            long long* ap = out.acc + ((long)k * 16 + 4 * g) * 256 + (wave * 2 + t) * 16 + c;
#pragma unroll
            for (int r = 0; r < 4; ++r) qacc_add(ap + r * 256, acc[r]);
        }
    }
    ATL(5)
}

struct QFfn { const bf16_t* W1; const float* b1; const bf16_t* W2; long long* acc; int FF; };
template <int HS>
__global__ __launch_bounds__(256) void qffn_kernel(QIn in, QFfn a) {
    if (in.prio) __builtin_amdgcn_s_setprio(1);
    constexpr int T1 = HS / 64;
    constexpr int KS2 = HS / 32;
    constexpr int HLD = HS + 4;
    __shared__ float sX[16 * PROJ_XLD];
    __shared__ float sH[16 * HLD];
    const int sl = blockIdx.x, k = blockIdx.y, wave = threadIdx.x >> 6, lane = threadIdx.x & 63, c = lane & 15, g = lane >> 4;
    ATL(0)
    QRows<4> R;
    qrows_issue<4, 4, true, false, true>(in, k, R);
    proj_u4 w1[T1][8], w2[4][KS2];
#pragma unroll
    for (int t = 0; t < T1; ++t) proj16_load<8>(a.W1, sl * HS + (wave * T1 + t) * 16, 0, w1[t]);
#pragma unroll
    for (int t = 0; t < 4; ++t) proj16_load<KS2>(a.W2, (wave * 4 + t) * 16, sl * KS2, w2[t], a.FF);
    qrows_finish<4, 4, true, false, true>(in, k, R, sX, nullptr, sl == 0);
    ATL(1)
    QSYNC();
#pragma unroll
    for (int t = 0; t < T1; ++t) {
        const f32x4 acc = proj16_mma<8>(sX, 0, w1[t]);
        const int col = (wave * T1 + t) * 16 + c;
        const float bv = a.b1[sl * HS + col];
#pragma unroll
        for (int r = 0; r < 4; ++r) sH[(4 * g + r) * HLD + col] = fmaxf(acc[r] + bv, 0.f);
    }
    ATL(2)
    QSYNC();
#pragma unroll
    for (int t = 0; t < 4; ++t) {
        const f32x4 acc = proj16_mma<KS2>(sH, 0, w2[t], HLD);
        long long* ap = a.acc + ((long)k * 16 + 4 * g) * 256 + (wave * 4 + t) * 16 + c;
#pragma unroll
        for (int r = 0; r < 4; ++r) qacc_add(ap + r * 256, acc[r]);
    }
    ATL(3)
}

struct NextQ { const float* ln_g; const float* ln_b; const bf16_t* W; const float* bias; float* q_out; float* xn_out; };
__global__ __launch_bounds__(256) void p2q_chain_kernel(QIn in, const bf16_t* __restrict__ q, bf16_t* __restrict__ y, int HW, int ldq, NextQ nq) {
    if (in.prio) __builtin_amdgcn_s_setprio(1);
    constexpr int C = 256;
    __shared__ float sX[2][16 * PROJ_XLD];
    __shared__ float ks[16][36], vs[16][36];
    const int hh = blockIdx.y, k = blockIdx.z;
    const int wave = threadIdx.x >> 6, lane = threadIdx.x & 63, c = lane & 15, g = lane >> 4;
    const int isv = wave >> 1, col = (wave & 1) * 16;
    const float scale = rsqrtf(32.f);
    ATL(0)
    if (nq.W && blockIdx.x == gridDim.x - 1) {
        QIn in2 = in;
        in2.ln_g = nq.ln_g; in2.ln_b = nq.ln_b; in2.ln_out = nq.xn_out;
        QRows<4> R2;
        qrows_issue<4, 4, true, true, true>(in2, k, R2);
        proj_u4 wq[4];
        proj16_load<4>(nq.W, hh * 32 + col, 4 * isv, wq);
        qrows_finish<4, 4, true, true, true>(in2, k, R2, sX[0], nullptr, hh == 0);
        QSYNC();
        f32x4* red = reinterpret_cast<f32x4*>(sX[1]);
        red[wave * 64 + lane] = proj16_mma<4>(sX[0], 4 * isv, wq);
        QSYNC();
        if (wave < 2) {
            const f32x4 a = red[wave * 64 + lane], b = red[(wave + 2) * 64 + lane];
            const float bv = nq.bias[hh * 32 + col + c];
#pragma unroll
            for (int r = 0; r < 4; ++r) nq.q_out[((long)k * 16 + 4 * g + r) * C + hh * 32 + col + c] = (a[r] + b[r] + bv) * scale;
        }
        return;
    }
    QRows<4> R;
    qrows_issue<4, 4, true, true, false>(in, k, R);
    proj_u4 wv[8];
    proj16_load<8>(in.W, isv * C + hh * 32 + col, 0, wv);
    const int pbase = blockIdx.x * 256 + wave * 64;
    proj_u4 qv[4];
#pragma unroll
    for (int t = 0; t < 4; ++t) {
        const int p = min(pbase + t * 16 + c, HW - 1);
        qv[t] = *reinterpret_cast<const proj_u4*>(q + ((long)k * HW + p) * ldq + hh * 32 + 8 * g);
    }
    qrows_finish<4, 4, true, true, false>(in, k, R, sX[0], sX[1], false);
    ATL(1)
    QSYNC();
    {
        const f32x4 a = proj16_mma<8>(sX[isv], 0, wv);
        const float bv = in.bias[isv * C + hh * 32 + col + c];
#pragma unroll
        for (int r = 0; r < 4; ++r) {
            if (isv) vs[4 * g + r][col + c] = a[r] + bv;
            else ks[4 * g + r][col + c] = (a[r] + bv) * scale;
        }
    }
    QSYNC();
    ATL(2)
    if (pbase >= HW) return;
    float kf[8];
#pragma unroll
    for (int j = 0; j < 8; ++j) kf[j] = ks[c][8 * g + j];
    proj_u4 khi, klo, vhi[2], vlo[2];
    split8(kf, khi, klo);
#pragma unroll
    for (int dt = 0; dt < 2; ++dt) {
        float vf[4];
#pragma unroll
        for (int j = 0; j < 4; ++j) vf[j] = vs[4 * g + j][dt * 16 + c];
        split4(vf, vhi[dt], vlo[dt]);
    }
#pragma unroll
    for (int t = 0; t < 4; ++t) {
        const int p = pbase + t * 16 + c;
        f32x4 s = {0.f, 0.f, 0.f, 0.f};
        s = __builtin_amdgcn_mfma_f32_16x16x32_bf16(as_frag(klo), as_frag(qv[t]), s, 0, 0, 0);
        s = __builtin_amdgcn_mfma_f32_16x16x32_bf16(as_frag(khi), as_frag(qv[t]), s, 0, 0, 0);
        const float mx = rows_max(fmaxf(fmaxf(s[0], s[1]), fmaxf(s[2], s[3])));
        float pe[4];
#pragma unroll
        for (int r = 0; r < 4; ++r) pe[r] = __expf(s[r] - mx);
        const float inv = 1.f / rows_sum((pe[0] + pe[1]) + (pe[2] + pe[3]));
#pragma unroll
        for (int r = 0; r < 4; ++r) pe[r] *= inv;
        proj_u4 phi, plo;
        split4(pe, phi, plo);
#pragma unroll
        for (int dt = 0; dt < 2; ++dt) {
            f32x4 o = {0.f, 0.f, 0.f, 0.f};
            o = mfma3(vhi[dt], vlo[dt], phi, plo, o);
            if (p < HW)
                *reinterpret_cast<uint2*>(y + ((long)k * HW + p) * C + hh * 32 + dt * 16 + 4 * g) = make_uint2(pack_bf2(o[0], o[1]), pack_bf2(o[2], o[3]));
        }
    }
    ATL(3)
}

#ifdef CUTIE_DIAG
struct P2QOut { const bf16_t* Wo; const float* bo; const bf16_t* res; };
#define P2O_LD 264
#define P2O_LDS_BYTES (2 * 16 * PROJ_XLD * 4 + 8 * 2 * 16 * 36 * 4 + 64 * P2O_LD * 2)
__global__ __launch_bounds__(512) void p2q_out_kernel(QIn in, const bf16_t* __restrict__ q, bf16_t* __restrict__ y, int HW, int ldq, NextQ nq, P2QOut po, int ntiles) {
    constexpr int C = 256;
    extern __shared__ uint8_t dynlds[];
    float* const sX0 = reinterpret_cast<float*>(dynlds);
    float* const sX1 = sX0 + 16 * PROJ_XLD;
    float (*sKV)[16][36] = reinterpret_cast<float (*)[16][36]>(dynlds + 2 * 16 * PROJ_XLD * 4);
    bf16_t* const sO = reinterpret_cast<bf16_t*>(dynlds + 2 * 16 * PROJ_XLD * 4 + 8 * 2 * 16 * 36 * 4);
    const int k = blockIdx.y;
    const int wave = threadIdx.x >> 6, lane = threadIdx.x & 63, c = lane & 15, g = lane >> 4;
    const float scale = rsqrtf(32.f);
    ATL(0)
    if ((int)blockIdx.x >= ntiles) {
        const int hh = blockIdx.x - ntiles, isv = (wave >> 1) & 1, col = (wave & 1) * 16;
        QIn in2 = in;
        in2.ln_g = nq.ln_g; in2.ln_b = nq.ln_b; in2.ln_out = nq.xn_out;
        QRows<2> R2;
        qrows_issue<8, 2, true, true, true>(in2, k, R2);
        proj_u4 wq[4];
        if (wave < 4) proj16_load<4>(nq.W, hh * 32 + col, 4 * isv, wq);
        qrows_finish<8, 2, true, true, true>(in2, k, R2, sX0, nullptr, hh == 0);
        QSYNC();
        f32x4* red = reinterpret_cast<f32x4*>(sX1);
        if (wave < 4) red[wave * 64 + lane] = proj16_mma<4>(sX0, 4 * isv, wq);
        QSYNC();
        if (wave < 2) {
            const f32x4 a = red[wave * 64 + lane], b = red[(wave + 2) * 64 + lane];
            const float bv = nq.bias[hh * 32 + col + c];
#pragma unroll
            for (int r = 0; r < 4; ++r) nq.q_out[((long)k * 16 + 4 * g + r) * C + hh * 32 + col + c] = (a[r] + b[r] + bv) * scale;
        }
        return;
    }
    const int hh = wave;
    QRows<2> R;
    qrows_issue<8, 2, true, true, false>(in, k, R);
    proj_u4 wk[2][8], wv[2][8];
#pragma unroll
    for (int t = 0; t < 2; ++t) proj16_load<8>(in.W, hh * 32 + t * 16, 0, wk[t]);
#pragma unroll
    for (int t = 0; t < 2; ++t) proj16_load<8>(in.W, C + hh * 32 + t * 16, 0, wv[t]);
    const int pbase = blockIdx.x * 64;
    proj_u4 qv[4];
#pragma unroll
    for (int t = 0; t < 4; ++t) {
        const int p = min(pbase + t * 16 + c, HW - 1);
        qv[t] = *reinterpret_cast<const proj_u4*>(q + ((long)k * HW + p) * ldq + hh * 32 + 8 * g);
    }
// ... 91 lines not shown
#pragma unroll
            for (int t = 0; t < 4; ++t) acc[ct][t] = f32x4{0.f, 0.f, 0.f, 0.f};
#pragma unroll
        for (int s_ = 0; s_ < 8; ++s_) {
#pragma unroll
            for (int t = 0; t < 4; ++t) {
                const proj_u4 b = *reinterpret_cast<const proj_u4*>(sO + (t * 16 + c) * P2O_LD + s_ * 32 + 8 * g);
#pragma unroll
                for (int ct = 0; ct < 2; ++ct) acc[ct][t] = __builtin_amdgcn_mfma_f32_16x16x32_bf16(as_frag(wo[ct][s_]), as_frag(b), acc[ct][t], 0, 0, 0);
            }
        }
#pragma unroll
        for (int t = 0; t < 4; ++t) {
            const int p = pbase + t * 16 + c;
#pragma unroll
            for (int ct = 0; ct < 2; ++ct) {
                float v[4] = {acc[ct][t][0] + bo[ct].x, acc[ct][t][1] + bo[ct].y, acc[ct][t][2] + bo[ct].z, acc[ct][t][3] + bo[ct].w};
                v[0] += __uint_as_float(rs[ct][t].x << 16); v[1] += __uint_as_float(rs[ct][t].x & 0xffff0000u);
                v[2] += __uint_as_float(rs[ct][t].y << 16); v[3] += __uint_as_float(rs[ct][t].y & 0xffff0000u);
                if (p < HW)
                    *reinterpret_cast<uint2*>(y + ((long)k * HW + p) * C + hh * 32 + ct * 16 + 4 * g) = make_uint2(pack_bf2(v[0], v[1]), pack_bf2(v[2], v[3]));
            }
        }
    }
    ATL(4)
}

#endif

static bool qin_from_op(const cutie_op* op, QIn& in, QOut& out, const char* who, int xslot, int lnout_slot, bool no_proj = false) {
    const uint64_t* p = op->p;
    in = QIn{};
    out = QOut{};
    in.prio = (op->flags & CUTIE_F_PRIO) ? 1 : 0;
    in.x = (const float*)p[xslot];
    in.ln_out = lnout_slot >= 0 ? (float*)p[lnout_slot] : nullptr;
    in.W = (const bf16_t*)p[5]; in.bias = (const float*)p[6]; in.add = (const float*)p[7];
    in.ln_g = (const float*)p[8]; in.ln_b = (const float*)p[9];
    if (op->flags & 4) {
        if (!p[10]) { cutie_set_error("%s: flags&4 needs p10 = the fixed-point accumulator", who); return false; }
        in.acc = (const long long*)p[10]; in.abias = (const float*)p[11];
    }
    if (op->flags & 8) {
        if (!p[12] || !p[13]) { cutie_set_error("%s: flags&8 needs p12 = Wo and p13 = the accumulator", who); return false; }
        out.W = (const bf16_t*)p[12]; out.acc = (long long*)p[13];
    }
#ifdef ATT_TIMELINE
    in.tl = (unsigned long long*)p[15];
#endif
    if (!in.x || (!in.W && !no_proj)) { cutie_set_error("%s: chain form needs the rows and the projection weight", who); return false; }
    return true;
}

int launch_qchain(const cutie_op* op, hipStream_t s) {
    const int32_t* i = op->i;
    const uint64_t* p = op->p;
    QIn in; QOut out;
    switch (op->kind) {
        case CUTIE_OP_ATTN_Q2P: {
            if (i[1] != 16 || i[3] != 256 || i[4] != 8 || (i[7] > 0 && i[7] != 256)) { cutie_set_error("attn_q2p (chain form): Q = 16, C = 256, 8 heads, dense rows"); return -2; }
            if ((op->flags & 11) != 11) { cutie_set_error("attn_q2p (chain form): flags 1 | 2 | 8 required"); return -2; }
            if (!qin_from_op(op, in, out, "attn_q2p", 0, 3, (op->flags & 16) != 0)) return -2;
            if (!p[1] || !p[2]) { cutie_set_error("attn_q2p (chain form): kv and the mask logits required"); return -2; }
            const int HWp = (i[2] + 15) & ~15;
            const bool qp = (op->flags & 16) != 0, ac = !qp && (op->flags & 4);
            const float* qpre = nullptr;
            if (qp) { qpre = (const float*)p[0]; in.x = nullptr; in.W = nullptr; in.ln_out = nullptr; }
            else if (!in.add || !in.ln_g || !in.ln_b || !in.bias || (ac && !in.abias)) {
                cutie_set_error("attn_q2p (chain form): query embedding, LayerNorm, the projection bias and (flags&4) the accumulator's bias are required");
                return -2;
            }
            const bool mixed = i[10] != 0;
            int Kg = i[9] > 0 ? i[9] : i[0];
            if (mixed) {
                int objs; const int nc = mixed_clips((unsigned)i[10], &objs);
                if (nc < 1 || objs != i[0] || i[9] != 0) { cutie_set_error("attn_q2p (chain form, mixed): the counts 0x%x do not add up to K = %d (or i9 != 0)", i[10], i[0]); return -2; }
                Kg = i[10];
            } else if (i[0] % Kg) { cutie_set_error("attn_q2p (chain form): clips of %d objects do not divide K = %d", Kg, i[0]); return -2; }
            const int kt = Kg <= 4 ? 1 : Kg <= 8 ? 2 : 0;
            const int var = mixed ? 9 + (qp ? 2 : ac ? 1 : 0) : (qp ? 6 : ac ? 3 : 0) + kt;
            constexpr int NWV = 8;
            typedef void (*Kern)(QIn, QOut, const bf16_t*, const float*, int, int, int, int, int, const float*, int);
            static const Kern kerns[12] = {
                q2p_chain_kernel<false, false, 0, NWV>, q2p_chain_kernel<false, false, 4, NWV>, q2p_chain_kernel<false, false, 8, NWV>,
                q2p_chain_kernel<false, true, 0, NWV>, q2p_chain_kernel<false, true, 4, NWV>, q2p_chain_kernel<false, true, 8, NWV>,
                q2p_chain_kernel<true, false, 0, NWV>, q2p_chain_kernel<true, false, 4, NWV>, q2p_chain_kernel<true, false, 8, NWV>,
                q2p_chain_kernel<false, false, 8, NWV, true>, q2p_chain_kernel<false, true, 8, NWV, true>, q2p_chain_kernel<true, false, 8, NWV, true>};
            const Kern kern = kerns[var];
            const size_t dyn = (size_t)HWp + NWV * 32 * Q2C_VLD * 2;
            if (dyn > 96 * 1024) { cutie_set_error("attn_q2p (chain form): HW = %d does not fit the LDS flag array", i[2]); return -2; }
            static bool attr_set[12] = {};
            if (!attr_set[var]) {
                if (hipFuncSetAttribute(reinterpret_cast<const void*>(kern), hipFuncAttributeMaxDynamicSharedMemorySize, 96 * 1024) != hipSuccess) {
                    cutie_set_error("attn_q2p (chain form): cannot raise the dynamic LDS limit");
                    return -2;
                }
                attr_set[var] = true;
            }
            const int hstride = i[8] > 0 ? i[8] : 32;
            hipLaunchKernelGGL(kern, dim3(8, i[0]), dim3(NWV * 64), dyn, s, in, out, (const bf16_t*)p[1], (const float*)p[2], i[2], HWp, i[5], i[6], hstride, qpre, Kg);
            break;
        }
        case CUTIE_OP_ATTN_SELF:
            if (i[1] != 16 || i[2] != 256 || i[3] != 8 || (i[6] > 0 && i[6] != 256)) { cutie_set_error("attn_self (chain form): Q = 16, C = 256, 8 heads, dense rows"); return -2; }
            if ((op->flags & 14) != 14) { cutie_set_error("attn_self (chain form): flags 2 | 4 | 8 required"); return -2; }
            if (!qin_from_op(op, in, out, "attn_self", 0, 3)) return -2;
            if (!in.add || !in.ln_g || !in.ln_b || !in.bias || !in.abias) { cutie_set_error("attn_self (chain form): query embedding, LayerNorm and both biases are required"); return -2; }
            hipLaunchKernelGGL(self_chain_kernel, dim3(8, i[0]), dim3(512), 0, s, in, out);
            break;
        case CUTIE_OP_ATTN_P2Q:
            if (i[1] != 16 || i[3] != 256 || i[4] != 8 || (i[7] > 0 && i[7] != 256)) { cutie_set_error("attn_p2q (chain form): Q = 16, C = 256, 8 heads, dense rows"); return -2; }
            if ((op->flags & 6) != 6) { cutie_set_error("attn_p2q (chain form): flags 2 | 4 required"); return -2; }
            if (!qin_from_op(op, in, out, "attn_p2q", 1, -1)) return -2;
            in.ln_g = in.ln_b = nullptr;
            if (!p[0] || !p[3]) { cutie_set_error("attn_p2q (chain form): q and y required"); return -2; }
            if (!in.add || !in.bias || !in.abias) { cutie_set_error("attn_p2q (chain form): query embedding and both biases are required"); return -2; }
        {
            NextQ nq = {};
            if (op->flags & 16) {
                if (!p[8] || !p[9] || !p[12] || !p[13] || !p[14] || !p[15]) { cutie_set_error("attn_p2q (chain form): flags&16 needs p8, p9, p12, p13, p14, p15"); return -2; }
                nq = NextQ{(const float*)p[8], (const float*)p[9], (const bf16_t*)p[12], (const float*)p[13], (float*)p[14], (float*)p[15]};
            }
#ifdef CUTIE_DIAG
            if (op->flags & 32) {
                if (!p[2] || !p[4] || (p[2] & 15) || (p[4] & 7) || (p[3] & 7) || p[3] == p[0]) { cutie_set_error("attn_p2q (flags&32): p2 = Wo | bias (16-byte aligned), p4 = residual, y 8-byte aligned required"); return -2; }
                static bool attr_set = false;
                if (!attr_set) {
                    if (hipFuncSetAttribute(reinterpret_cast<const void*>(p2q_out_kernel), hipFuncAttributeMaxDynamicSharedMemorySize, P2O_LDS_BYTES) != hipSuccess) {
                        cutie_set_error("attn_p2q (flags&32): cannot raise the dynamic LDS limit");
                        return -2;
                    }
                    attr_set = true;
                }
                const bf16_t* Wo = (const bf16_t*)p[2];
                const P2QOut po = {Wo, reinterpret_cast<const float*>(Wo + 256 * 256), (const bf16_t*)p[4]};
                const int ntiles = (i[2] + 63) / 64;
                hipLaunchKernelGGL(p2q_out_kernel, dim3(ntiles + (nq.W ? 8 : 0), i[0]), dim3(512), P2O_LDS_BYTES, s, in, (const bf16_t*)p[0], (bf16_t*)p[3], i[2], i[5], nq, po, ntiles);
                break;
            }
#else
            if (op->flags & 32) { cutie_set_error("attn_p2q (flags&32: output projection inside): only in the diagnostic library (make DIAG=1)"); return -2; }
#endif
            hipLaunchKernelGGL(p2q_chain_kernel, dim3((i[2] + 255) / 256 + (nq.W ? 1 : 0), 8, i[0]), dim3(256), 0, s, in, (const bf16_t*)p[0], (bf16_t*)p[3], i[2], i[5], nq);
        }
            break;
        case CUTIE_OP_QFFN: {
            const int HS = i[2] > 0 ? i[2] : 64;
            if ((i[0] & 15) || i[1] < HS || (i[1] % HS) || (HS != 64 && HS != 128) || !p[0] || !p[2] || !p[3] || !p[4] || !p[6] || !p[7]) {
                cutie_set_error("qffn: rows %% 16, FF %% slice == 0, slice 64 | 128 and x, gamma, beta, W1, W2, accumulator required (rows=%d FF=%d slice=%d)", i[0], i[1], HS);
                return -2;
            }
            in = QIn{};
            in.prio = (op->flags & CUTIE_F_PRIO) ? 1 : 0;
            in.x = (const float*)p[0]; in.x_out = (float*)p[1]; in.ln_g = (const float*)p[2]; in.ln_b = (const float*)p[3];
            if (!p[10] || !p[11] || !p[5]) { cutie_set_error("qffn: the input accumulator, its bias and linear1's bias are required"); return -2; }
            in.acc = (const long long*)p[10]; in.abias = (const float*)p[11];
#ifdef ATT_TIMELINE
            in.tl = (unsigned long long*)p[15];
#endif
            QFfn a = {(const bf16_t*)p[4], (const float*)p[5], (const bf16_t*)p[6], (long long*)p[7], i[1]};
            if (HS == 64) hipLaunchKernelGGL(qffn_kernel<64>, dim3(i[1] / 64, i[0] / 16), dim3(256), 0, s, in, a);
            else hipLaunchKernelGGL(qffn_kernel<128>, dim3(i[1] / 128, i[0] / 16), dim3(256), 0, s, in, a);
            break;
        }
        default:
            cutie_set_error("qchain: unknown op kind %d", op->kind);
            return -3;
    }
    return (int)hipGetLastError();
}
```

cutie_amd/model/cutie.py:

```python
import logging
from typing import Dict, Iterable, List

import torch
import torch.nn as nn

from .. import _lib, frame_context
from . import plans
from .param_spec import build_spec
from .weights import fold_bn, pack_conv, pack_linear, linear_as_conv

log = logging.getLogger()
BF16, F32 = torch.bfloat16, torch.float32


def nhwc_of(t, C=None):
    p = t.permute(0, 2, 3, 1)
    if p.dtype != BF16 or not p.is_contiguous():
        p = p.to(BF16).contiguous()
    return p


def group_nhwc_of(t, dtype=BF16):
    assert t.shape[0] == 1, 'batch size 1 only (flip_aug is not supported yet)'
    p = t[0].permute(0, 2, 3, 1)
# ... 52 lines not shown
                        continue
                    if name.endswith('.downsample.0'):
                        conv(name, bn=name[:-1] + '1')
                    else:
                        conv(name, bn=name.replace('.conv', '.bn'))
        for name in ['pix_feat_proj', 'key_proj.pix_feat_proj', 'key_proj.key_proj', 'key_proj.d_proj', 'key_proj.e_proj',
                     'mask_decoder.sensory_update.g16_conv', 'mask_decoder.sensory_update.g8_conv',
                     'mask_decoder.decoder_feat_proc.transforms.0', 'mask_decoder.decoder_feat_proc.transforms.1',
                     'mask_decoder.up_16_8.out_conv.downsample', 'mask_decoder.up_16_8.out_conv.conv1',
                     'mask_decoder.up_16_8.out_conv.conv2', 'mask_decoder.up_8_4.out_conv.conv1',
                     'mask_decoder.up_8_4.out_conv.conv2', 'mask_decoder.pred']:
            conv(name)
        conv('mask_decoder.sensory_update.g4_conv', segs=[(up[2], up[2]), (1, 8)])
        sg = 'mask_decoder.sensory_update.'
        W[sg + 'g_all'] = pack_conv(torch.cat([sd[sg + 'g16_conv.weight'], sd[sg + 'g8_conv.weight'], sd[sg + 'g4_conv.weight']], 1),
                                    sd[sg + 'g16_conv.bias'] + sd[sg + 'g8_conv.bias'] + sd[sg + 'g4_conv.bias'], dev,
                                    segs=[(up[0], up[0]), (up[1], up[1]), (up[2], up[2]), (1, 64)])
        conv('mask_decoder.sensory_update.transform', segs=[(CS, CS), (CS, CS)])
        conv('mask_encoder.sensory_update.transform', segs=[(CV, CV), (CS, CS)])
        conv('pixel_fuser.sensory_compress', segs=[(CS, CS), (2, 64)])
        ca_blocks = []
        for fz in ('mask_encoder.fuser', 'pixel_fuser.fuser'):
            conv(fz + '.distributor.x_transform')
            conv(fz + '.distributor.g_transform')
            ca_blocks += [fz + '.block1', fz + '.block2']
        t = 'object_transformer'
        ot = m['object_transformer']
        C = m['embed_dim']
        for b in range(ot['num_blocks']):
            q = f'{t}.blocks.{b}'
            ca_blocks.append(q + '.pixel_ffn.conv')
            rp, sa, rq = q + '.read_from_pixel.cross_attn', q + '.self_attn.self_attn', q + '.read_from_query.cross_attn'
            Wp, bp = sd[rp + '.in_proj_weight'], sd[rp + '.in_proj_bias']
            Ws, bs = sd[sa + '.in_proj_weight'], sd[sa + '.in_proj_bias']
            Wq, bq = sd[rq + '.in_proj_weight'], sd[rq + '.in_proj_bias']
            wm = torch.cat([Wp[C:2 * C], Wp[2 * C:], Wq[:C]], 0)
            bm = torch.cat([bp[C:2 * C], bp[2 * C:], bq[:C]], 0)
            wpe = torch.cat([Wp[C:2 * C], torch.zeros(C, C), Wq[:C]], 0)
            self._pe_wb[b] = wpe.float()
            we_ = sd[t + '.pixel_emb_proj.weight'].float().reshape(C, -1)
            W[q + '.pixel_proj_x'] = pack_conv(torch.cat([wm.float(), wpe.float() @ we_], 1).reshape(3 * C, 2 * C, 1, 1),
                                               bm.float() + wpe.float() @ sd[t + '.pixel_emb_proj.bias'].float(), dev, segs=[(C, C), (C, C)])
            W[q + '.read_from_pixel.q'] = pack_linear(Wp[:C], bp[:C], dev)
            W[q + '.read_from_pixel.out'] = pack_linear(sd[rp + '.out_proj.weight'], sd[rp + '.out_proj.bias'], dev)
            W[q + '.self_attn.qkv'] = pack_linear(Ws, bs, dev)
            W[q + '.self_attn.out'] = pack_linear(sd[sa + '.out_proj.weight'], sd[sa + '.out_proj.bias'], dev)
            W[q + '.read_from_query.kv'] = pack_linear(Wq[C:], bq[C:], dev)
            W[q + '.read_from_query.out'] = linear_as_conv(sd[rq + '.out_proj.weight'], sd[rq + '.out_proj.bias'], dev)
            for ln in ('.read_from_pixel.norm', '.self_attn.norm', '.ffn.norm'):
                W[q + ln + '.weight'] = sd[q + ln + '.weight'].to(dev).contiguous()
                W[q + ln + '.bias'] = sd[q + ln + '.bias'].to(dev).contiguous()
            W[q + '.ffn.linear1'] = pack_linear(sd[q + '.ffn.linear1.weight'], sd[q + '.ffn.linear1.bias'], dev)
            W[q + '.ffn.linear2'] = pack_linear(sd[q + '.ffn.linear2.weight'], sd[q + '.ffn.linear2.bias'], dev)
        conv(t + '.pixel_init_proj')
        for b in range(ot['num_blocks'] + 1):
            conv(f'{t}.mask_pred.{b}.1')
        for name in ca_blocks:
            conv(name + '.conv1')
            conv(name + '.conv2')
            W[name + '.conv.weight'] = sd[name + '.conv.weight'].reshape(-1).to(dev).contiguous()
        W[t + '.summary_to_query_init'] = pack_linear(sd[t + '.summary_to_query_init.weight'], sd[t + '.summary_to_query_init.bias'], dev)
        W[t + '.summary_to_query_emb'] = pack_linear(sd[t + '.summary_to_query_emb.weight'], sd[t + '.summary_to_query_emb.bias'], dev)
        u = 'object_summarizer'
        w_in, b_in = sd[u + '.input_proj.weight'].float(), sd[u + '.input_proj.bias'].float()
        w0 = torch.cat([sd[u + '.feature_pred.0.weight'].float(), sd[u + '.weights_pred.0.weight'].float()], 0)
        b0 = torch.cat([sd[u + '.feature_pred.0.bias'].float(), sd[u + '.weights_pred.0.bias'].float()], 0)
        self._sum_w0 = w0
        W[u + '.in_fw0'] = linear_as_conv(w0 @ w_in, b0 + w0 @ b_in, dev)
        wf2, ww2 = sd[u + '.feature_pred.2.weight'].float(), sd[u + '.weights_pred.2.weight'].float()
        cf, cw = wf2.shape[1], ww2.shape[1]
        w2 = torch.zeros(wf2.shape[0] + ww2.shape[0], cf + cw)
        w2[:wf2.shape[0], :cf] = wf2
        w2[wf2.shape[0]:, cf:] = ww2
        W[u + '.fw2'] = linear_as_conv(w2, torch.cat([sd[u + '.feature_pred.2.bias'].float(), sd[u + '.weights_pred.2.bias'].float()], 0), dev)

    def pe_rb(self, h, w, b):
        key = ('pe_rb', h, w, b)
        if key not in self._pe:
            e = plans.positional_encoding(h, w, self.m['embed_dim'], self.m['pixel_pe_scale'], self.m['pixel_pe_temperature'])
            e = e.reshape(h * w, -1).float()
            self._pe[key] = (e @ self._pe_wb[b].t()).to(BF16).to(self.device).contiguous()
        return self._pe[key]

    def pe_sum(self, h, w):
        key = ('pe_sum', h, w)
        if key not in self._pe:
            e = plans.positional_encoding(h, w, self.m['embed_dim'], self.m['pixel_pe_scale'], self.m['pixel_pe_temperature'])
            self._pe[key] = (e.reshape(h * w, -1).float() @ self._sum_w0.t()).to(BF16).to(self.device).contiguous()
        return self._pe[key]

    def rep_embedding(self, which, K):
        key = (which, K)
        if key not in self._rep:
            e = self.sd[f'object_transformer.{which}.weight']
            self._rep[key] = e.repeat(K, 1).to(self.device).contiguous()
        return self._rep[key]

    def mask_down_bufs(self, K, h, w, clips=1):
        mb = self.__dict__.setdefault('_md_bufs', {})
        if (K, h, w, clips) not in mb:
            mb[(K, h, w, clips)] = (torch.zeros((K, h, w, 64), dtype=BF16, device=self.device), torch.zeros((K, h, w), dtype=F32, device=self.device))
        return mb[(K, h, w, clips)]

    def query_bufs(self, K):
        qb = self.__dict__.setdefault('_query_bufs', {})
        if K not in qb:
            M = K * self.m['object_transformer']['num_queries']
            qb[K] = tuple(torch.zeros((M, self.m['embed_dim']), dtype=F32, device=self.device) for _ in range(2))
        return qb[K]

    def fork(self):
        e = object.__new__(Engine)
        e.__dict__.update(self.__dict__)
        e._plans = {}
        e._arenas = {}
        e.pool = plans.SlotPool()
        e.__dict__.pop('_splitk_part', None)
        e.__dict__.pop('_streams', None)
        e.__dict__.pop('_query_bufs', None)
        e.__dict__.pop('_md_bufs', None)
        e.__dict__.pop('_qinit_state', None)
        return e

    def plan(self, key, builder, *args):
        p = self._plans.get(key)
        if p is None:
            p = builder(self, *args)
            p.ol.finalize()
            kind = 'side' if key[0] in ('enc', 'key') else ('win' if key[0] == 'encw' else 'main')
            arenas = self.__dict__.setdefault('_arenas', {})
            if kind not in arenas:
                arenas[kind] = plans.Arena(self.device)
            p.pack_into(arenas[kind])
            self._plans[key] = p
        return p


class _Container(nn.Module):
    pass


class CUTIE(nn.Module):
    def __init__(self, cfg, *, single_object=False):
        super().__init__()
        if single_object:
            raise NotImplementedError('single_object=True is a training-time variant; not on the inference path')
        self.cfg = cfg
        m = cfg.model if hasattr(cfg, 'model') else cfg['model']
        self.model_cfg = m
        self.ms_dims = m['pixel_encoder']['ms_dims']
        self.key_dim, self.value_dim = m['key_dim'], m['value_dim']
        self.sensory_dim, self.pixel_dim, self.embed_dim = m['sensory_dim'], m['pixel_dim'], m['embed_dim']
        self.single_object = single_object
        self.object_transformer_enabled = m['object_transformer']['num_blocks'] > 0
        if not self.object_transformer_enabled:
            raise NotImplementedError('num_blocks == 0 is not supported')
        self._spec = build_spec(m)
        g = torch.Generator().manual_seed(0)
        for name, (shape, role) in self._spec.items():
            self._register(name, shape, role, g)
        self.register_buffer('pixel_mean', torch.tensor(m['pixel_mean'], dtype=F32).view(-1, 1, 1), False)
        self.register_buffer('pixel_std', torch.tensor(m['pixel_std'], dtype=F32).view(-1, 1, 1), False)
        self._eng = None
        self._key_cache = None
        self.eval()

    def _register(self, name, shape, role, g):
        parts = name.split('.')
        mod = self
        for p in parts[:-1]:
            if not hasattr(mod, p):
                mod.add_module(p, _Container())
            mod = getattr(mod, p)
        leaf = parts[-1]
        if role in ('w', 'emb', 'eca'):
            fan_in = max(1, int(torch.tensor(shape[1:]).prod())) if len(shape) > 1 else 1
            t = torch.randn(shape, generator=g) * (1.0 / fan_in ** 0.5)
            mod.register_parameter(leaf, nn.Parameter(t))
        elif role in ('b', 'bn_b', 'ln_b'):
            mod.register_parameter(leaf, nn.Parameter(torch.zeros(shape)))
        elif role in ('bn_w', 'ln_w'):
            mod.register_parameter(leaf, nn.Parameter(torch.ones(shape)))
        elif role == 'bn_mean':
            mod.register_buffer(leaf, torch.zeros(shape))
        elif role == 'bn_var':
            mod.register_buffer(leaf, torch.ones(shape))
        elif role == 'bn_nbt':
            mod.register_buffer(leaf, torch.tensor(0, dtype=torch.long))
# ... 333 lines not shown
```

cutie_amd/model/plans.py:

```python
import math
import os

import numpy as np
import torch

from .. import _lib
from .. import ops as O
from ..ops import Dyn
from .param_spec import resnet_layers

BF16, F32 = torch.bfloat16, torch.float32


class Act:
    __slots__ = ('t', 'B', 'H', 'W', 'C', 'ld')

    def __init__(self, t, B, H, W, C, ld=None):
        self.t, self.B, self.H, self.W, self.C, self.ld = t, B, H, W, C, (C if ld is None else ld)


def positional_encoding(h, w, dim_total, scale, temperature):
    dim = int(math.ceil(dim_total / 4) * 2)
    inv_freq = 1.0 / (temperature ** (torch.arange(0, dim, 2).float() / dim))
    py = torch.arange(h, dtype=torch.float32)
# ... 179 lines not shown
        arr = self.ol.finalize()
        ptrs = arr['p'].astype(np.int64)
        items = []
        for name, t in self.bufs.items():
            if name in self.persistent or t.numel() == 0:
                continue
            base, nbytes = t.data_ptr(), t.numel() * t.element_size()
            hit = (ptrs >= base) & (ptrs < base + nbytes)
            if not hit.any():
                continue
            rows = np.nonzero(hit.any(axis=1))[0]
            items.append(dict(name=name, base=base, nbytes=nbytes, first=int(rows[0]), last=int(rows[-1]), hit=hit, t=t))
        items.sort(key=lambda b: (b['first'], -b['nbytes']))
        placed = []
        total = 0
        for b in items:
            size = -(-b['nbytes'] // ARENA_ALIGN) * ARENA_ALIGN
            live = sorted((o, e) for (o, e, last) in placed if last >= b['first'])
            off = 0
            for o, e in live:
                if off + size <= o:
                    break
                off = max(off, e)
            b['off'] = off
            placed.append((off, off + size, b['last']))
            total = max(total, off + size)
        self.arena = arena
        self._arena_slots = []
        for b in items:
            idx, slot = np.nonzero(b['hit'])
            for i, sl in zip(idx, slot):
                self._arena_slots.append((int(i), int(sl), b['off'] + int(ptrs[i, sl] - b['base'])))
            self._arena_views[b['name']] = (b['off'], tuple(b['t'].shape), b['t'].dtype)
        self.ol.keep = [k for k in self.ol.keep if not any(k is b['t'] for b in items)]
        arena.plans.append(self)
        arena.require(total)
        self.rebind_arena()
        self.meta['arena_bytes'] = total
        self.meta['unpacked_bytes'] = sum(b['nbytes'] for b in items)

    def rebind_arena(self):
        if self.arena is None or self.arena.tensor is None:
            return
        base = self.arena.base()
        p = self.ol.arr['p']
        for (i, sl, off) in self._arena_slots:
            p[i, sl] = base + off
            self.ol.recs[i][4][sl] = base + off
        for name, (off, shape, dtype) in self._arena_views.items():
            n = int(np.prod(shape)) * torch.empty((), dtype=dtype).element_size()
            self.bufs[name] = self.arena.tensor[off:off + n].view(dtype).view(shape)

    graph_head = 0

    def run(self, **dyn):
        if not self.tuned:
            self.tuned = True
            self.autotune_convs(**dyn)
        if ARENA_POISON and self.arena is not None and self.arena.tensor is not None:
            self.arena.tensor.fill_(0xFF)
        ol = self.ol
        ex = _lib.get_executor()
        if GRAPHS and len(ol.recs) >= GRAPH_MIN_OPS and hasattr(ex, 'run_cached'):
            if ol.arr is None:
                ol.finalize()
            if dyn:
                ol.bind(**dyn)
            ex.run_cached(ol.arr, self._graphs, self.graph_head)
        else:
            ol.run(**dyn)

    def run_part(self, lo, hi, first=True, **dyn):
        if not self.tuned:
            self.tuned = True
            self.autotune_convs(**dyn)
        if first and ARENA_POISON and self.arena is not None and self.arena.tensor is not None:
            self.arena.tensor.fill_(0xFF)
        ol = self.ol
        if ol.arr is None:
            ol.finalize()
        if dyn:
            ol.bind(**dyn)
        _lib.get_executor().run(ol.arr[lo:hi])

    def autotune_convs(self, **dyn):
        from .. import _lib
        ex = _lib.get_executor()
        ex = getattr(ex, 'ex', ex)
        if ex.is_mock or not hasattr(ex, 'time_ops'):
            return
        ol = self.ol
        if ol.arr is None:
            ol.finalize()
        ol.bind(**dyn)
        arr = ol.arr
        cache = self.eng.tile_cache
        tuned_any = False
        for n in range(len(arr)):
            if arr['kind'][n] != O.CONV:
                continue
            i = arr['i'][n]
            M, cout, cin = int(i[0]) * int(i[7]) * int(i[8]), int(i[9]), int(i[3]) + int(i[4])
            fl = int(arr['flags'][n])
            key = O.conv_tile_key(M, cout, cin, int(i[11]), int(i[13]), fl & O.F_RELU_IN, fl & O.F_OUT_F32, int(i[1]), int(i[2]))
            best = cache.get(key)
            twin = self.korder_ref and int(i[0]) % self.korder_ref == 0
# ... 518 lines not shown
```

cutie_amd/ops.py:

```python
import os

import numpy as np
import torch

from . import _lib

NI, NF, NP = 24, 6, 16
OP_DTYPE = np.dtype([('kind', '<i4'), ('flags', '<i4'), ('i', '<i4', (NI,)), ('f', '<f4', (NF,)), ('p', '<u8', (NP,))])
assert OP_DTYPE.itemsize == _lib.OP_STRUCT_SIZE

(CONV, MAXPOOL, IMG_PREP, UPSAMPLE2X_ADD, AREA_DOWN, MASK_DOWN, GAP, ECA_APPLY, GRU, SEG_AGG, UP4_SOFTMAX,
 MASK_MERGE, AGG_SOFTMAX, LINEAR, LAYERNORM, QUERY_INIT, AUX_MASK, ATTN_Q2P, ATTN_SELF, ATTN_P2Q, SUMMARIZE,
 ADD_PE, KEY_PREP, AFF_SCORE, AFF_SELECT, AFF_READOUT, MEMSET32, COPY2D, AXPY, USAGE_TICK, RANK_SELECT,
 GATHER_ROWS, CONSOL_AFF, CONSOL_READ, CAST, PROB_TO_ID, RESIZE, FLIP_W, AREA_DOWN3, QFFN, STEM, BANK_WRITE) = range(1, 43)

KIND_NAMES = {}
for _n in ('CONV MAXPOOL IMG_PREP UPSAMPLE2X_ADD AREA_DOWN MASK_DOWN GAP ECA_APPLY GRU SEG_AGG UP4_SOFTMAX MASK_MERGE '
           'AGG_SOFTMAX LINEAR LAYERNORM QUERY_INIT AUX_MASK ATTN_Q2P ATTN_SELF ATTN_P2Q SUMMARIZE ADD_PE KEY_PREP '
           'AFF_SCORE AFF_SELECT AFF_READOUT MEMSET32 COPY2D AXPY USAGE_TICK RANK_SELECT GATHER_ROWS CONSOL_AFF '
           'CONSOL_READ CAST PROB_TO_ID RESIZE FLIP_W AREA_DOWN3 QFFN STEM').split():
    KIND_NAMES[globals()[_n]] = _n

F_RELU_IN, F_OUT_F32, F_RES_BCAST = 1, 2, 4
F_PRIO, F_AFF_PRIO = 256, 64
# ... 28 lines not shown
            126: (128, 128, 64), 127: (64, 128, 64), 129: (96, 64, 64), 130: (32, 64, 64), 131: (64, 128, 64),
            132: (64, 64, 64), 133: (96, 128, 64), 134: (320, 64, 64),
            140: (64, 64, 64), 141: (96, 64, 64), 142: (96, 64, 64), 143: (32, 64, 64), 144: (128, 64, 64),
            145: (96, 64, 64), 146: (128, 64, 64), 147: (32, 64, 64)}
PC_HALO = {120: (8, 8), 121: (4, 16), 122: (8, 16), 123: (8, 16), 124: (8, 8), 125: (4, 8), 126: (8, 16), 127: (4, 16),
           129: (10, 9), 130: (5, 6), 131: (6, 9), 132: (6, 9), 133: (10, 9), 134: (20, 16),
           145: (10, 9), 146: (8, 16), 147: (5, 6)}

ALL_TILES = {**TILES, **DMA_TILES, **PC_TILES}


def korder_class(tile, splitk=1):
    if tile in PC_HALO:
        return 'halo'
    if tile in TILE_WK or splitk != 1:
        return ('split', tile, splitk)
    if tile in (3, COUT1_TILE):
        return ('small', tile)
    return 'stream' if (tile in DMA_TILES or tile in PC_TILES) else 'igemm'


def pc_tile_ok(tile, *, cin, kh, stride=1, pad=None, c2=0):
    if cin % 64 or (c2 and (c2 % 64 or (cin - c2) % 64)) or kh > 5:
        return False
    if tile in PC_HALO:
        return kh == 3 and stride == 1 and (pad is None or pad == 1)
    return True


def pc_blocks(tile, B, OH, OW, cout):
    bm, bn, _ = PC_TILES[tile]
    if tile in PC_HALO:
        th, tw = PC_HALO[tile]
        return B * -(-OH // th) * -(-OW // tw) * -(-cout // bn)
    return -(-(B * OH * OW) // bm) * -(-cout // bn)


def dma_tiles_enabled():
    return os.environ.get('CUTIE_AMD_DMA_TILES', '1') not in ('', '0')


def dma_tile_ok(tile, *, cin, kh, c2=0):
    bk = DMA_TILES[tile][2]
    return cin % bk == 0 and (c2 == 0 or (c2 % bk == 0 and (cin - c2) % bk == 0)) and kh * kh <= 32


def conv_side_jobs_ok(*, cin, cout, kh, c2=0):
    return dma_tiles_enabled() and dma_tile_ok(60, cin=cin, kh=kh, c2=c2) and cout % 8 == 0 and cout > 16


NUM_CU = 256
WEIGHT_PREFETCH = int(os.environ.get('CUTIE_AMD_WPF', str(8 << 20)))
WEIGHT_PREFETCH_BLOCK = int(os.environ.get('CUTIE_AMD_WPF_BLOCK', str(48 << 10)))


COUT1_TILE = 19


def cout1_ok(cout, cin, c2=0, res=False):
    lp = cin // 8
    return cout == 1 and c2 == 0 and not res and cin % 8 == 0 and 1 <= lp <= 64 and (lp & (lp - 1)) == 0


def tile_candidates(M, cout, cin, kpad=None, geom=None):
    if cout <= 16:
        return [3] + ([COUT1_TILE] if cout1_ok(cout, cin) else [])
    out = []
    for t, (bm, bn, bk) in TILES.items():
        if t == 3 or (bk > 32 and cin < 32):
            continue
        wk = TILE_WK.get(t, 1)
        if wk > 1 and (kpad is None or (kpad // bk) % wk or kpad // bk < 2 * wk):
            continue
        if bn == 128 and cout <= 64:
            continue
        if bm * 2 > max(M, 64) * 2 and bm > 64:
            continue
        out.append(t)
    if dma_tiles_enabled() and geom is not None and dma_tile_ok(60, cin=cin, kh=geom['kh'], c2=geom.get('c2', 0)):
        for t, (bm, bn, bk) in DMA_TILES.items():
            if not (bn == 128 and cout <= 64) and not (bm > 64 and bm > max(M, 64)) and not (bm == 256 and M < 16384) \
                    and dma_tile_ok(t, cin=cin, kh=geom['kh'], c2=geom.get('c2', 0)):
                out.append(t)
    if dma_tiles_enabled() and geom is not None:
        for t, (bm, bn, bk) in PC_TILES.items():
            if pc_tile_ok(t, cin=cin, kh=geom['kh'], stride=geom.get('stride', 1), pad=geom.get('pad'), c2=geom.get('c2', 0)) \
                    and not (bn == 128 and cout <= 64) and not (bm > 64 and bm > max(M, 64)) and not (bm == 256 and M < 16384):
                out.append(t)
    return out


SPLITK_PART_FLOATS = 16 << 20
_splitk_scratch = {}


def splitk_scratch(device, owner=None):
    dev = torch.device(device)
    store = _splitk_scratch if owner is None else owner.__dict__.setdefault('_splitk_part', {})
    key = str(dev)
    if key not in store:
        n = SPLITK_PART_FLOATS if dev.type == 'cuda' else 1024
        store[key] = torch.zeros(n, dtype=torch.float32, device=device)
    return store[key]


def splitk_candidates(M, cout, kpad, tile):
# ... 104 lines not shown
        self.name, self.offset = name, offset


def _ptr(t):
    if t is None:
        return 0
    if isinstance(t, int):
        return t
    return t.data_ptr()


def _need_form(has, words):
    try:
        known = getattr(_lib._executor, 'is_mock', False) or has()
    except _lib.HipLibraryError:
        known = True
    if not known:
        raise _lib.HipLibraryError(f'{_lib.LIB_PATH} is stale ({words}); rebuild it.')


def _u8_plane(who, name, t, hw=None):
    shaped = t.dim() == 2 if hw is None else tuple(t.shape) == tuple(hw)
    if t.dtype != torch.uint8 or not shaped or not t.is_contiguous():
        if hw is None or (min(hw) >= 1 and hw[0] * hw[1] < 1 << 31):
            raise ValueError(f"{who}: {name} is a contiguous uint8 {'[H, W]' if hw is None else list(hw)}, not {t.dtype} {tuple(t.shape)}")
    H, W = hw if hw is not None else (int(t.shape[0]), int(t.shape[1]))
    if H < 1 or W < 1 or H * W >= 1 << 31:
        raise ValueError(f'{who}: a plane of {H} x {W}: H, W >= 1 and H * W < 2^31')
    return H, W


def _object_ids(who, name, objects):
    if torch.is_tensor(objects):
        if objects.dtype != torch.int32 or objects.dim() != 1 or not objects.is_contiguous():
            raise ValueError(f'{who}: {name} on the device are a contiguous int32 [n]')
        return int(objects.numel()), objects, None
    listed = [int(v) for v in objects]
    return len(listed), None, listed


JPEG_SYNC_ROUNDS = 4


class OpList:
    PRIO_KINDS = frozenset((UPSAMPLE2X_ADD, AREA_DOWN3, ECA_APPLY, GRU, UP4_SOFTMAX, ATTN_Q2P, ATTN_SELF, ATTN_P2Q, QFFN))

    def __init__(self, scratch_owner=None, touch_next_weights=True, prio=True):
        self.prio = prio
        self.scratch_owner = scratch_owner
        self.touch_next_weights = touch_next_weights
        self.recs = []
        self.keep = []
        self.wbytes = {}
        self.dyn = {}
        self.arr = None
        self._words = None

    def add(self, kind, flags=0, ints=(), floats=(), ptrs=()):
        idx = len(self.recs)
        if kind in self.PRIO_KINDS and self.prio:
            flags |= F_PRIO
        pl = []
        for slot, t in enumerate(ptrs):
            if isinstance(t, Dyn):
                self.dyn.setdefault(t.name, []).append((idx, slot, t.offset))
                pl.append(0)
            else:
                if isinstance(t, torch.Tensor):
                    self.keep.append(t)
                pl.append(_ptr(t))
        self.recs.append((kind, flags, [int(v) for v in ints], [float(v) for v in floats], pl))
        self.arr = self._words = None
        return idx

    def finalize(self):
        arr = np.zeros(len(self.recs), dtype=OP_DTYPE)
        for n, (kind, flags, ints, floats, ptrs) in enumerate(self.recs):
            arr['kind'][n] = kind
            arr['flags'][n] = flags
            arr['i'][n, :len(ints)] = ints
            arr['f'][n, :len(floats)] = floats
            arr['p'][n, :len(ptrs)] = ptrs
        self.arr = arr
        self._words = None
        self.wire_next_weights()
        return arr

    def wire_next_weights(self):
        arr = self.arr
        convs = [n for n in range(len(arr)) if arr['kind'][n] == CONV]
        for n in convs:
            arr['p'][n, 9:11] = 0
            arr['i'][n, 22:24] = 0
        if not (WEIGHT_PREFETCH and self.touch_next_weights):
            return
        nxt, nxt2 = None, None
        for n in reversed(convs):
            i = arr['i'][n]
            pc = int(i[17]) in PC_TILES
            if nxt is not None and pc:
                budget = WEIGHT_PREFETCH_BLOCK * -(-pc_blocks(int(i[17]), int(i[0]), int(i[7]), int(i[8]), int(i[9])) // 8)
                n1 = min(nxt[1], WEIGHT_PREFETCH, budget)
                arr['p'][n, 9], arr['i'][n, 22] = nxt[0], n1
                n2 = min(nxt2[1], WEIGHT_PREFETCH, budget - n1) if (nxt2 is not None and not nxt[2]) else 0
                if n2 > 0:
                    arr['p'][n, 10], arr['i'][n, 23] = nxt2[0], n2
            nxt, nxt2 = (int(arr['p'][n, 2]), self.wbytes[n], pc), nxt

    def patch_ints(self, op, start, values):
        values = [int(v) for v in values]
        ints = self.recs[op][2]
        end = start + len(values)
        if len(ints) < end:
            ints.extend([0] * (end - len(ints)))
        ints[start:end] = values
        if self.arr is not None:
            self.arr['i'][op, start:end] = values

    def bind(self, **tensors):
        if self.arr is None:
            self.finalize()
        words = self._words
        if words is None:
            assert OP_DTYPE.itemsize == 256 and OP_DTYPE.fields['p'][1] == 128
            words = self._words = ({name: tuple((idx * 32 + 16 + slot, off) for (idx, slot, off) in sl) for name, sl in self.dyn.items()},
                                   memoryview(self.arr).cast('B').cast('Q'))
        table, mv = words
        for name, t in tensors.items():
            sl = table.get(name)
            if sl is None:
                continue
            base = 0 if t is None else (t if type(t) is int else t.data_ptr())
            if base:
                for w, off in sl:
                    mv[w] = base + off
            else:
                for w, off in sl:
                    mv[w] = 0

    def run(self, _stream=None, **tensors):
        if self.arr is None:
            self.finalize()
        if tensors:
            self.bind(**tensors)
        ex = _lib.get_executor()
        if _stream is None:
            ex.run(self.arr)
        elif hasattr(ex, 'run_on'):
            ex.run_on(self.arr, _stream)
        else:
            with torch.cuda.stream(_stream):
                ex.run(self.arr)

    def __len__(self):
        return len(self.recs)

    def conv(self, x1, w, y, *, B, H, W, C1, ldx1, OH, OW, ldy, stride=1, pad=0, x2=None, C2=0, ldx2=0,
             res=None, ldr=0, res_bcast=False, relu_in=False, act=ACT_NONE, out_f32=False, tile=None, splitk=1,
             gap_acc=None, zero=None, prio=False, res_group=None):
        flags = (F_RELU_IN if relu_in else 0) | (F_OUT_F32 if out_f32 else 0) | (F_RES_BCAST if res_bcast else 0) | (act << ACT_SHIFT) | F_TILE_OFF | \
            (F_PRIO if prio else 0)
        assert C1 + C2 == w.cin_padded, (C1, C2, w.cin_padded)
        M = B * OH * OW
        side = gap_acc is not None or zero is not None
        if tile is None:
            tile = static_tile(M, w.cout, C1 + C2, w.kh, C2, res is not None, side)
        if side:
            assert (tile in DMA_TILES or tile in PC_TILES) and not out_f32 and w.cout % 8 == 0 and ldy % 8 == 0, 'GAP accumulation needs an LDS-DMA conv (see conv_side_jobs_ok)'
        part = splitk_scratch(w.weight.device, self.scratch_owner)
        self.wbytes[len(self.recs)] = w.weight.numel() * w.weight.element_size()
        return self.add(CONV, flags,
                        [B, H, W, C1, C2, ldx1, ldx2, OH, OW, w.cout, ldy, w.kh, w.kw, stride, pad, ldr, w.kpad, tile, w.cin_real,
                         splitk, part.numel() // 1024, 0 if zero is None else zero.numel()],
                        self._res_group(res_group, res_bcast, B, OH * OW), [x1, x2, w.weight, w.bias, res, y, part, gap_acc, zero])

    @staticmethod
    def _res_group(res_group, res_bcast, B, OHW):
        if res_group is None:
            return []
        kg, stride = int(res_group[0]), int(res_group[1])
        assert res_bcast and kg > 0 and B % kg == 0 and stride >= OHW and stride < (1 << 24), (res_group, B, OHW)
        return [float(kg), float(stride)]

    def maxpool(self, x, y, *, B, H, W, C, relu=False):
        OH, OW = (H + 2 - 3) // 2 + 1, (W + 2 - 3) // 2 + 1
        return self.add(MAXPOOL, 1 if relu else 0, [B, H, W, C, OH, OW], [], [x, y])

    STEM_MAX_IMAGES = 12

    def stem(self, image, masks, w, y, *, h0, w0, H, W, pad_left, pad_top, K, mean, std, relu=True, more_images=(), mask_stride=0, counts=None):
        assert w.cout == 64 and w.kh == 7 and w.cin_padded == 8 and H % 16 == 0 and W % 16 == 0
        more = list(more_images)
        assert len(more) < self.STEM_MAX_IMAGES
        if counts is not None:
            assert len(counts) == 1 + len(more) and len(counts) > 1
            ints = [h0, w0, H, W, pad_left, pad_top, max(counts), w.kpad, len(counts), 0, pack_counts(counts)]
            return self.add(STEM, 1 if relu else 0, ints, list(mean) + list(std), [image, masks, w.weight, w.bias, y] + more)
        ints = [h0, w0, H, W, pad_left, pad_top, K, w.kpad] + ([1 + len(more), int(mask_stride)] if more else [])
        return self.add(STEM, 1 if relu else 0, ints, list(mean) + list(std), [image, masks, w.weight, w.bias, y] + more)

    def img_prep(self, image, masks, y, *, h0, w0, H, W, pad_left, pad_top, K, mean, std):
        return self.add(IMG_PREP, 0, [h0, w0, H, W, pad_left, pad_top, K], list(mean) + list(std), [image, masks, y])

    def upsample2x_add(self, g, skip, y, *, B, h, w, C, skip_group=None):
        ints = [B, h, w, C]
        if skip_group is not None and not isinstance(skip_group[0], int):
            counts, stride = skip_group
            assert sum(counts) == B and stride >= 4 * h * w
            ints += [0, int(stride), pack_counts(counts)]
        elif skip_group is not None:
            kg, stride = int(skip_group[0]), int(skip_group[1])
            assert kg > 0 and B % kg == 0 and stride >= 4 * h * w
            ints += [kg, stride]
        return self.add(UPSAMPLE2X_ADD, 0, ints, [], [g, skip, y])

    def area_down(self, x, y, *, B, H, W, C, ldx, ldy, r, f32_in=False, Cz=None):
        return self.add(AREA_DOWN, 1 if f32_in else 0, [B, H, W, C, ldx, ldy, r, C if Cz is None else Cz], [], [x, y])

    def area_down3(self, segs):
        assert len(segs) == 3
        ints, ptrs, flags = [], [], 0
        for q, g in enumerate(segs):
            ints += [g['B'], g['H'], g['W'], g['C'], g['ldx'], g['ldy'], g['r'], g['C'] if g.get('Cz') is None else g['Cz']]
# ... 22 lines not shown
        if part is None:
            part = self._last_gap_scratch
        return self.add(ECA_APPLY, 0, [B, HW, C], [], [x, gap, wk, r, y, part] + tail)

    def gru(self, values, h, hb, *, n, C):
        return self.add(GRU, GRU_SCALAR, [n, C], [], [values, h, hb])

    def seg_agg(self, logits, agg, *, K, hw):
        return self.add(SEG_AGG, 0, [K, hw], [], [logits, agg])

    def up4_softmax(self, agg, prob, logits_up, *, P, h, w, from_logits=False, mask_down=None, clips=1):
        if not isinstance(clips, int):
            counts = [int(k) for k in clips]
            assert from_logits and len(counts) > 1 and h % 4 == 0 and w % 4 == 0 and not UP4_RTK, 'the mixed form: compile-time object counts'
            ints = [max(counts) + 1, h, w, 0, len(counts), pack_counts(counts)]
            if mask_down is not None:
                m16, pair, ints[3] = mask_down
                return self.add(UP4_SOFTMAX, 1 | 4 | UP4_LANES, ints, [], [agg, prob, logits_up, m16, pair])
            return self.add(UP4_SOFTMAX, 1, ints, [], [agg, prob, logits_up])
        if mask_down is not None:
            assert from_logits and P <= 8 and h % 4 == 0 and w % 4 == 0
            m16, pair, pitch = mask_down
            return self.add(UP4_SOFTMAX, 1 | 4 | UP4_RTK | UP4_LANES, [P, h, w, pitch, clips], [], [agg, prob, logits_up, m16, pair])
        assert clips == 1 or (from_logits and P <= 8)
        return self.add(UP4_SOFTMAX, (1 | UP4_RTK) if from_logits else 0, [P, h, w, 0, clips], [], [agg, prob, logits_up])

    def mask_merge(self, inmask, pred, src, planes, *, h0, w0, H, W, pad_left, pad_top, Knew, Kold, nfloat, float_mode):
        return self.add(MASK_MERGE, 1 if float_mode else 0, [h0, w0, H, W, pad_left, pad_top, Knew, Kold, nfloat], [],
                        [inmask, pred, src, planes])

    def agg_softmax(self, planes, prob, *, K, HW):
        return self.add(AGG_SOFTMAX, 0, [K, HW], [], [planes, prob])

    def linear(self, x, w, y, *, M, ldx=None, ldy=None, x_add=None, add_rows=0, res=None, relu=False, add_cols=0,
               ln=None, ln_out=None, eps=1e-5):
        flags = (1 if relu else 0) | (2 if ln is not None else 0)
        return self.add(LINEAR, flags,
                        [M, w.n, w.kd, w.kd if ldx is None else ldx, w.n if ldy is None else ldy, add_rows, add_cols], [eps],
                        [x, x_add, w.weight, w.bias, res, y, ln[0] if ln else None, ln[1] if ln else None, ln_out])

    def layernorm(self, x, g, b, y, *, M, C):
        return self.add(LAYERNORM, 0, [M, C], [], [x, g, b, y])

    def query_init(self, obj_mem, y, *, rows, C):
        return self.add(QUERY_INIT, 0, [rows, C], [], [obj_mem, y])

    def query_init2(self, obj_mem, query, query_emb, *, rows, w_init, res_init, w_emb, res_emb, zero=None):
        assert w_init.kd == 256 and w_init.n == 256 and w_emb.kd == 256 and w_emb.n == 256 and rows % 16 == 0
        nz = 0
        if zero is not None:
            nb = zero.numel() * zero.element_size()
            assert nb % 16 == 0 and zero.is_contiguous()
            nz = nb // 16
        return self.add(QUERY_INIT, 1, [rows, 256, nz], [], [obj_mem, query, query_emb, w_init.weight, w_init.bias, res_init,
                                                             w_emb.weight, w_emb.bias, res_emb, zero])

    def aux_mask(self, logits, fg, nfg, *, K, HW):
        self.memset32(nfg, K, 0)
        return self.add(AUX_MASK, 0, [K, HW], [], [logits, fg, nfg])

    @staticmethod
    def _proj(proj):
        ln = proj.get('ln') or (None, None)
        assert proj['W'].kd == 256
        return proj.get('ldx', 256), proj.get('ln_out'), [proj['W'].weight, proj['W'].bias, proj.get('emb'), ln[0], ln[1]]

    QACC_SCALE = 4294967296.0

    @staticmethod
    def _proj_extras(flags, ints, ptrs, acc_in, out_proj):
        ints = list(ints) + [0] * (9 - len(ints))
        ptrs = list(ptrs) + [None] * (14 - len(ptrs))
        if acc_in is not None:
            assert acc_in[0].dtype == torch.int64
            flags |= 4
            ptrs[10], ptrs[11] = acc_in[0], acc_in[1]
        if out_proj is not None:
            assert out_proj[0].kd == 256 and out_proj[0].n == 256 and out_proj[1].dtype == torch.int64
            flags |= 8
            ptrs[12], ptrs[13] = out_proj[0].weight, out_proj[1]
        return flags, ints, ptrs

    def attn_q2p(self, q, kv, fg, nfg, y, *, K, Q, HW, C, heads, ldkv, voff, logits=None, proj=None, acc_in=None, out_proj=None, q_pre=None, hstride=None,
                 clip_objects=None):
        hs = 0 if hstride in (None, C // heads) else hstride
        mixed = []
        if clip_objects is not None and not isinstance(clip_objects, int):
            assert out_proj is not None and sum(clip_objects) == K and len(clip_objects) > 1, 'clips in lock step need the chain form'
            mixed, clip_objects = [pack_counts(clip_objects)], None
        kg = 0 if clip_objects in (None, K) else int(clip_objects)
        assert kg == 0 or (out_proj is not None and K % kg == 0), 'clips in lock step need the chain form'
        if q_pre is not None:
            assert proj is None and acc_in is None and out_proj is not None and logits is not None
            flags, ints, ptrs = self._proj_extras(3 | 16, [K, Q, HW, C, heads, ldkv, voff, 256], [q_pre, kv, logits, None, None], None, out_proj)
            ints[8] = hs
            return self.add(ATTN_Q2P, flags, ints + [kg] + mixed, [], ptrs)
        if proj is not None:
            assert logits is not None
            ldx, ln_out, tail = self._proj(proj)
            assert out_proj is not None or acc_in is None, 'the chain form of ATTN_Q2P needs out_proj'
            flags, ints, ptrs = self._proj_extras(3, [K, Q, HW, C, heads, ldkv, voff, ldx], [proj['x'], kv, logits, ln_out, y] + tail, acc_in, out_proj)
            assert hs == 0 or out_proj is not None, 'a head stride needs the chain form'
            ints[8] = hs
            return self.add(ATTN_Q2P, flags, ints + [kg] + mixed, [], ptrs)
        assert acc_in is None and out_proj is None
        if logits is not None:
            return self.add(ATTN_Q2P, 1, [K, Q, HW, C, heads, ldkv, voff], [], [q, kv, logits, None, y])
        return self.add(ATTN_Q2P, 0, [K, Q, HW, C, heads, ldkv, voff], [], [q, kv, fg, nfg, y])

    def attn_self(self, qk, v, y, *, K, Q, C, heads, ldqk=0, ldv=0, proj=None, acc_in=None, out_proj=None):
        if proj is not None:
            ldx, ln_out, tail = self._proj(proj)
            assert out_proj is not None or acc_in is None, 'the chain form of ATTN_SELF needs out_proj'
            flags, ints, ptrs = self._proj_extras(2, [K, Q, C, heads, 0, 0, ldx], [proj['x'], None, y, ln_out, None] + tail, acc_in, out_proj)
            return self.add(ATTN_SELF, flags, ints, [], ptrs)
        assert acc_in is None and out_proj is None
        return self.add(ATTN_SELF, 0, [K, Q, C, heads, ldqk, ldv], [], [qk, v, y])

    def attn_p2q(self, q, kq, vq, y, *, K, Q, HW, C, heads, ldq, ldkv=0, proj=None, acc_in=None, next_q=None, out=None):
        if proj is not None:
            ldx, _, tail = self._proj(proj)
            flags, ints, ptrs = self._proj_extras(2, [K, Q, HW, C, heads, ldq, ldkv, ldx], [q, proj['x'], None, y, None] + tail[:3], acc_in, None)
            if out is not None:
                assert acc_in is not None and out['Wo'].dtype == torch.uint8 and out['Wo'].numel() == 256 * 256 * 2 + 256 * 4
                flags |= 32
                ptrs[2], ptrs[4] = out['Wo'], out['res']
            if next_q is not None:
                assert acc_in is not None and next_q['W'].kd == 256 and next_q['W'].n == 256
                flags |= 16
                ptrs = ptrs + [None] * (16 - len(ptrs))
                ptrs[8], ptrs[9] = next_q['ln']
                ptrs[12], ptrs[13], ptrs[14], ptrs[15] = next_q['W'].weight, next_q['W'].bias, next_q['q_out'], next_q['xn_out']
            return self.add(ATTN_P2Q, flags, ints, [], ptrs)
        assert acc_in is None
        return self.add(ATTN_P2Q, 0, [K, Q, HW, C, heads, ldq, ldkv], [], [q, kq, vq, y])

    def qffn(self, x, x_out, acc_out, *, rows, ln, W1, W2, acc_in=None, hid_slice=64):
        FF = W1.n
        assert W1.kd == 256 and W2.kd == FF and W2.n == 256 and FF % hid_slice == 0 and hid_slice in (64, 128) and rows % 16 == 0
        assert acc_out.dtype == torch.int64
        ints = [rows, FF, hid_slice]
        ptrs = [x, x_out, ln[0], ln[1], W1.weight, W1.bias, W2.weight, acc_out] + [None] * 6
        if acc_in is not None:
            assert acc_in[0].dtype == torch.int64
            ptrs[10], ptrs[11] = acc_in[0], acc_in[1]
        return self.add(QFFN, 0, ints, [], ptrs)

    def summarize(self, feat, wl, m16, y, *, K, HW, C, Q, scratch=None, feat_f32=False, ldf=None, ldw=None):
        if scratch is None:
            scratch = torch.zeros((K, -(-HW // 128), Q, C + 1), dtype=torch.float32, device=m16.device)
        return self.add(SUMMARIZE, 1 if feat_f32 else 0, [K, HW, C, Q, C if ldf is None else ldf, Q if ldw is None else ldw], [], [feat, wl, m16, y, scratch])

    def add_pe(self, x, pe, y, *, B, n):
        return self.add(ADD_PE, 0, [B, n], [], [x, pe, y])

    def key_prep(self, key, aux, hi, lo, sc, *, n, query):
        return self.add(KEY_PREP, (1 | KEYPREP_LOOP) if query else 0, [n], [], [key, aux, hi, lo, sc])

    AFF_CSTRIDE = 32

    def aff_score(self, Ahi, Alo, scale, Bhi, Blo, c, out, cand_val, cand_idx, count, *, HW, HWp, ranges, cap, mode, gmax_precedes_tau=False, nq=None, dma=None,
                  frames=1, extra_lds_kb=0, prio=False, banks=None):
        ranges = [(s, n) for (s, n) in ranges if n > 0]
        assert 1 <= len(ranges) <= 3
        G = sum(-(-n // 16) for _, n in ranges)
        ints = [HW, HWp, len(ranges)]
        for r in range(3):
            ints += list(ranges[r]) if r < len(ranges) else [0, 0]
        ints += [G, cap, mode, 2 if nq is None else nq, 0, int(extra_lds_kb), int(bool(dma))]
        if frames > 1:
            ints[1] = frames * HWp
            ints += [HWp]
        ptrs = [Ahi, Alo, scale, Bhi, Blo, c, out, cand_val, cand_idx, count]
        flags = (1 if (gmax_precedes_tau and mode == 1) else 0) | (F_AFF_PRIO if prio else 0)
        if banks is not None:
            assert frames > 1 and frames % banks[1] == 0 and ints[12] == 2 and HWp % 128 == 0
            ints += [banks[1]]
            ptrs += [None, banks[0]]
            flags |= 4
        return self.add(AFF_SCORE, flags, ints, [], ptrs)

    def aff_select(self, gmax, tau, *, HW, HWp, G, top_k, clear_count=None, ticks=(), zero=None, frames=1, prio=False):
        if zero is not None:
            assert not ticks
            return self.add(AFF_SELECT, 1 | SELECT_COARSE | (F_AFF_PRIO if prio else 0), [HW, HWp, G, top_k, zero[1], 0, frames], [], [gmax, tau, clear_count, zero[0], None])
        ticks = list(ticks) + [(None, 0)] * (2 - len(ticks))
        assert len(ticks) == 2
        return self.add(AFF_SELECT, SELECT_COARSE | (F_AFF_PRIO if prio else 0), [HW, HWp, G, top_k, ticks[0][1], ticks[1][1], frames], [], [gmax, tau, clear_count, ticks[0][0], ticks[1][0]])

    def aff_readout(self, cand_val, cand_idx, count, vptrs, usage, y, overflow, *, HW, cap, top_k, K, CV, frames=1, HWp=0, usage_stride=0, prio=False, banks=1, usage_fx=False):
        assert banks == 1 or frames % banks == 0
        return self.add(AFF_READOUT, (F_AFF_PRIO if prio else 0) | (1 if usage_fx else 0), [HW, cap, top_k, K, CV, frames, HWp, usage_stride, banks], [], [cand_val, cand_idx, count, vptrs, usage, y, overflow])

    def memset32(self, dst, n, value=0):
        return self.add(MEMSET32, 0, [n, value], [], [dst])

    def bank_write(self, copies=(), fills=()):
        copies, fills = list(copies), list(fills)
        idx = None
# ... 545 lines not shown
```

Before: 1168.

## Chain weight-prefetch touches across elementwise, attention and qchain launches

Generalizes the L2 weight-prefetch touch, which was previously only in the pointwise conv tail, into a shared device helper. Elementwise, GRU, ECA, area-down, up4-softmax and attention/qchain kernels now each accept two touch ranges. The planner assigns each upcoming weight-carrying launch (conv, query init, attention chains, QFFN) to an earlier launch with spare budget, so that launch pulls those weights into cache ahead of use. This aims to hide weight-fetch latency at the start of weight-heavy kernels. The cost is extra memory traffic and tail work in the touching kernels, plus more complex plan wiring.

```diff
diff --git a/cutie_amd/_lib.py b/cutie_amd/_lib.py
--- a/cutie_amd/_lib.py
+++ b/cutie_amd/_lib.py
@@ -83,6 +83,10 @@
     return bool(load().cutie_hip_build_flags() & 128)
 
 
+def has_chain_touch():
+    return bool(load().cutie_hip_build_flags() & 256)
+
+
 class HipExecutor:
     is_mock = False
 
diff --git a/cutie_amd/csrc/api.hip b/cutie_amd/csrc/api.hip
--- a/cutie_amd/csrc/api.hip
+++ b/cutie_amd/csrc/api.hip
@@ -129,7 +129,7 @@
 int cutie_hip_abi_version(void) { return 11; }
 int cutie_op_struct_size(void) { return (int)sizeof(cutie_op); }
 int cutie_hip_build_flags(void) {
-    const int forms = 2 | 4 | 8 | 16 | 32 | 64 | 128;
+    const int forms = 2 | 4 | 8 | 16 | 32 | 64 | 128 | 256;
 #ifdef CUTIE_DIAG
     return forms | 1;
 #else
diff --git a/cutie_amd/csrc/common.h b/cutie_amd/csrc/common.h
--- a/cutie_amd/csrc/common.h
+++ b/cutie_amd/csrc/common.h
@@ -95,6 +95,29 @@
     return n;
 }
 
+typedef __attribute__((ext_vector_type(4))) unsigned int touch_u32x4;
+struct TouchArgs { const unsigned char* a; const unsigned char* b; int a_bytes, b_bytes; };
+__device__ __forceinline__ void touch_ranges(const unsigned char* a, int a_bytes, const unsigned char* b, int b_bytes,
+                                             int block_linear_id, int nblocks, int thread, int nthreads) {
+    if (a_bytes <= 0 && b_bytes <= 0) return;
+    const int nbx = (nblocks + 7) >> 3, kq = block_linear_id >> 3;
+    touch_u32x4 t = {0u, 0u, 0u, 0u};
+#pragma unroll
+    for (int r = 0; r < 2; ++r) {
+        const unsigned char* base = r ? b : a;
+        const int bytes = r ? b_bytes : a_bytes;
+        const int chunk = (((bytes + nbx - 1) / nbx) + 1023) & ~1023;
+        const int b0 = kq * chunk, b1 = min(b0 + chunk, bytes & ~15);
+        for (int o = b0 + thread * 16; o < b1; o += nthreads * 16)
+            asm volatile("global_load_dwordx4 %0, %1, %2" : "+v"(t) : "v"(o), "s"(base) : "memory");
+    }
+    asm volatile("s_waitcnt vmcnt(0)" : "+v"(t) :: "memory");
+}
+static inline bool touch_range_ok(uint64_t ptr, long bytes) { return bytes >= 0 && bytes < (1L << 30) && (bytes == 0 || (ptr & 15) == 0); }
+static inline TouchArgs touch_args(uint64_t a, long a_bytes, uint64_t b, long b_bytes) {
+    return TouchArgs{(const unsigned char*)a, (const unsigned char*)b, a ? (int)a_bytes : 0, b ? (int)b_bytes : 0};
+}
+
 int launch_conv(const cutie_op* op, hipStream_t s);
 int launch_elementwise(const cutie_op* op, hipStream_t s);
 int launch_attention(const cutie_op* op, hipStream_t s);
diff --git a/cutie_amd/csrc/conv_igemm.hip b/cutie_amd/csrc/conv_igemm.hip
--- a/cutie_amd/csrc/conv_igemm.hip
+++ b/cutie_amd/csrc/conv_igemm.hip
@@ -476,6 +476,7 @@
     p.gap = (long long*)op->p[7]; p.zero = (unsigned long long*)op->p[8]; p.nzero = i[21];
     p.pf = (const unsigned char*)op->p[9]; p.pf_bytes = op->p[9] ? i[22] : 0;
     p.pf2 = (const unsigned char*)op->p[10]; p.pf2_bytes = op->p[10] ? i[23] : 0;
+    if (!touch_range_ok(op->p[9], i[22]) || !touch_range_ok(op->p[10], i[23])) { cutie_set_error("conv: a touch range (p9 / i22, p10 / i23) must be 16-byte aligned, its size >= 0"); return -2; }
     p.res_grp_rows = p.res_grp_stride = 0;
     if ((p.flags & CUTIE_F_RES_BCAST) && op->f[0] > 0.f) {
         const int kg = (int)op->f[0];
diff --git a/cutie_amd/csrc/conv_pc.hip b/cutie_amd/csrc/conv_pc.hip
--- a/cutie_amd/csrc/conv_pc.hip
+++ b/cutie_amd/csrc/conv_pc.hip
@@ -553,21 +553,7 @@
         }
         TLE(6)
         TL_DUMP(logical, nb, NC + NPW)
-        if (p.pf_bytes > 0) {
-            const int id = blockIdx.y * gridDim.x + blockIdx.x;
-            const int nbx = (nb + 7) >> 3, kq = id >> 3;
-            u32x4 t = {0u, 0u, 0u, 0u};
-#pragma unroll
-            for (int r = 0; r < 2; ++r) {
-                const unsigned char* base = r ? p.pf2 : p.pf;
-                const int bytes = r ? p.pf2_bytes : p.pf_bytes;
-                const int chunk = (((bytes + nbx - 1) / nbx) + 1023) & ~1023;
-                const int b0 = kq * chunk, b1 = min(b0 + chunk, bytes & ~15);
-                for (int o = b0 + (pw * 64 + lane) * 16; o < b1; o += NPW * 1024)
-                    asm volatile("global_load_dwordx4 %0, %1, off" : "+v"(t) : "v"(base + o) : "memory");
-            }
-            asm volatile("s_waitcnt vmcnt(0)" : "+v"(t) :: "memory");
-        }
+        touch_ranges(p.pf, p.pf_bytes, p.pf2, p.pf2_bytes, blockIdx.y * gridDim.x + blockIdx.x, nb, pw * 64 + lane, NPW * 64);
         return;
     }
 
diff --git a/cutie_amd/csrc/elementwise.hip b/cutie_amd/csrc/elementwise.hip
--- a/cutie_amd/csrc/elementwise.hip
+++ b/cutie_amd/csrc/elementwise.hip
@@ -67,9 +67,8 @@
 }
 
 template <bool MIXED = false>
-__global__ void upsample2x_add_kernel(const uint4* __restrict__ g, const uint4* __restrict__ skip, uint4* __restrict__ y,
-                                      int B, int h, int w, int C8, int Kg, long gstride, int prio) {
-    if (prio) __builtin_amdgcn_s_setprio(1);
+__device__ __forceinline__ void upsample2x_add_body(const uint4* __restrict__ g, const uint4* __restrict__ skip, uint4* __restrict__ y,
+                                                    int B, int h, int w, int C8, int Kg, long gstride) {
     long idx = (long)blockIdx.x * blockDim.x + threadIdx.x;
     int OH = 2 * h, OW = 2 * w;
     long total = (long)B * OH * OW * C8;
@@ -101,6 +100,13 @@
     }
     y[idx] = make_uint4(out[0], out[1], out[2], out[3]);
 }
+template <bool MIXED = false>
+__global__ void upsample2x_add_kernel(const uint4* __restrict__ g, const uint4* __restrict__ skip, uint4* __restrict__ y,
+                                      int B, int h, int w, int C8, int Kg, long gstride, int prio, TouchArgs tc) {
+    if (prio) __builtin_amdgcn_s_setprio(1);
+    upsample2x_add_body<MIXED>(g, skip, y, B, h, w, C8, Kg, gstride);
+    touch_ranges(tc.a, tc.a_bytes, tc.b, tc.b_bytes, blockIdx.x, gridDim.x, threadIdx.x, blockDim.x);
+}
 
 template <int R = 0>
 __device__ __forceinline__ void area_down_bf16_body(const bf16_t* __restrict__ x, bf16_t* __restrict__ y, int B, int H, int W, int C,
@@ -181,10 +187,8 @@
     area_down_f32_body(x, y, B, H, W, C, ldx, ldy, r, Cz, (long)blockIdx.x * blockDim.x + threadIdx.x);
 }
 struct AreaSeg { const void* x; bf16_t* y; int B, H, W, C, ldx, ldy, r, Cz, f32; long n; };
-struct Area3 { AreaSeg s[3]; int rt; int prio; };
-__global__ void area_down3_kernel(Area3 a) {
-    const int prio = a.prio;
-    if (prio) __builtin_amdgcn_s_setprio(1);
+struct Area3 { AreaSeg s[3]; int rt; int prio; TouchArgs tc; };
+__device__ __forceinline__ void area_down3_body(const Area3& a) {
     long idx = (long)blockIdx.x * blockDim.x + threadIdx.x;
 #pragma unroll
     for (int q = 0; q < 3; ++q) {
@@ -204,6 +208,12 @@
         }
         idx -= g.n;
     }
+}
+__global__ void area_down3_kernel(Area3 a) {
+    const int prio = a.prio;
+    if (prio) __builtin_amdgcn_s_setprio(1);
+    area_down3_body(a);
+    touch_ranges(a.tc.a, a.tc.a_bytes, a.tc.b, a.tc.b_bytes, blockIdx.x, gridDim.x, threadIdx.x, blockDim.x);
 }
 
 __global__ void mask_down_mean_kernel(const float* __restrict__ m, float* __restrict__ m16, int K, int H, int W, int r) {
@@ -302,7 +312,7 @@
                                                         const float* __restrict__ wk, const bf16_t* __restrict__ r,
                                                         bf16_t* __restrict__ y, float* __restrict__ gap_out, int HW, int C, int nchunk,
                                                         const long long* __restrict__ fixed, const bf16_t* __restrict__ pw,
-                                                        const float* __restrict__ pb, float* __restrict__ plog, int prio) {
+                                                        const float* __restrict__ pb, float* __restrict__ plog, int prio, TouchArgs tc) {
     if (prio) __builtin_amdgcn_s_setprio(1);
     __shared__ float gap[256 + 4], sc[256];
     const int b = blockIdx.y, tid = threadIdx.x;
@@ -392,10 +402,10 @@
             if (c8 == 0 && offs[it] >= 0) plog[(long)b * HW + p] = tot + bias;
         }
     }
-}
-
-__global__ void gru4_kernel(const float* __restrict__ v, float* __restrict__ h, bf16_t* __restrict__ hb, long n, int C, int prio) {
-    if (prio) __builtin_amdgcn_s_setprio(1);
+    touch_ranges(tc.a, tc.a_bytes, tc.b, tc.b_bytes, blockIdx.y * gridDim.x + blockIdx.x, gridDim.x * gridDim.y, tid, 256);
+}
+
+__device__ __forceinline__ void gru4_body(const float* __restrict__ v, float* __restrict__ h, bf16_t* __restrict__ hb, long n, int C) {
     const long idx = (long)blockIdx.x * blockDim.x + threadIdx.x;
     const int C4 = C >> 2;
     if (idx >= n * C4) return;
@@ -412,6 +422,11 @@
     }
     *reinterpret_cast<float4*>(h + row * C + c) = make_float4(o[0], o[1], o[2], o[3]);
     *reinterpret_cast<uint2*>(hb + row * C + c) = make_uint2(pack_bf2(o[0], o[1]), pack_bf2(o[2], o[3]));
+}
+__global__ void gru4_kernel(const float* __restrict__ v, float* __restrict__ h, bf16_t* __restrict__ hb, long n, int C, int prio, TouchArgs tc) {
+    if (prio) __builtin_amdgcn_s_setprio(1);
+    gru4_body(v, h, hb, n, C);
+    touch_ranges(tc.a, tc.a_bytes, tc.b, tc.b_bytes, blockIdx.x, gridDim.x, threadIdx.x, blockDim.x);
 }
 
 __global__ void gru_kernel(const float* __restrict__ v, float* __restrict__ h, bf16_t* __restrict__ hb, long n, int C) {
@@ -732,7 +747,7 @@
 
 template <int PMAX, int KC = 0, bool SH = false>
 __global__ __launch_bounds__(256) void up4_softmax_md_kernel(const float* __restrict__ lg, float* __restrict__ prob, float* __restrict__ lup,
-                                                             int Krt, int h, int w, float* __restrict__ m16, uint4* __restrict__ pair, int ld8, int prio) {
+                                                             int Krt, int h, int w, float* __restrict__ m16, uint4* __restrict__ pair, int ld8, int prio, TouchArgs tc) {
     if (prio) __builtin_amdgcn_s_setprio(1);
     const int K = KC > 0 ? KC : Krt;
     __shared__ float cell[4][PMAX - 1][256];
@@ -740,7 +755,8 @@
     const int OH = 4 * h, OW = 4 * w, ch = OH >> 4, cw = OW >> 4, ncell = ch * cw;
     const int wave = threadIdx.x >> 6, lane = threadIdx.x & 63;
     const int cid = blockIdx.x * 4 + wave;
-    if (cid >= ncell) return;
+    const int tid_lin = blockIdx.y * gridDim.x + blockIdx.x, tnb = gridDim.x * gridDim.y;
+    if (cid >= ncell) { touch_ranges(tc.a, tc.a_bytes, tc.b, tc.b_bytes, tid_lin, tnb, threadIdx.x, 256); return; }
     {
         const long cl = blockIdx.y;
         lg += cl * K * h * w; prob += cl * (K + 1) * (long)OH * OW;
@@ -801,6 +817,7 @@
                 pair[((long)k * ncell + cid) * ld8] = make_uint4(pack_bf2(mk[k], others), 0u, 0u, 0u);
             }
     }
+    touch_ranges(tc.a, tc.a_bytes, tc.b, tc.b_bytes, tid_lin, tnb, threadIdx.x, 256);
 }
 
 template <int PMAX, bool SH>
@@ -1360,15 +1377,17 @@
         }
         case CUTIE_OP_UPSAMPLE2X_ADD: {
             int C8 = i[3] / 8;
+            if (!touch_range_ok(p[3], i[7]) || !touch_range_ok(p[4], i[8])) { cutie_set_error("upsample2x_add: a touch range (p3 / i7, p4 / i8) must be 16-byte aligned, its size >= 0"); return -2; }
+            const TouchArgs tc = touch_args(p[3], i[7], p[4], i[8]);
             long n = (long)i[0] * 4 * i[1] * i[2] * C8;
             if (i[6]) {
                 int objs; const int nc = mixed_clips((unsigned)i[6], &objs);
                 if (nc < 1 || objs != i[0] || i[4] != 0 || i[5] < 4 * i[1] * i[2]) { cutie_set_error("upsample2x_add (mixed form): the counts 0x%x do not add up to B = %d (or i4 != 0, or the stride is below one map)", i[6], i[0]); return -2; }
-                hipLaunchKernelGGL(upsample2x_add_kernel<true>, GRID1D(n, BS), dim3(BS), 0, s, (const uint4*)p[0], (const uint4*)p[1], (uint4*)p[2], i[0], i[1], i[2], C8, i[6], (long)i[5], PRIO);
+                hipLaunchKernelGGL(upsample2x_add_kernel<true>, GRID1D(n, BS), dim3(BS), 0, s, (const uint4*)p[0], (const uint4*)p[1], (uint4*)p[2], i[0], i[1], i[2], C8, i[6], (long)i[5], PRIO, tc);
                 break;
             }
             if (i[4] < 0 || (i[4] > 0 && (i[0] % i[4] || i[5] < 4 * i[1] * i[2]))) { cutie_set_error("upsample2x_add: skip groups of %d objects do not divide B = %d (or their stride is below one map)", i[4], i[0]); return -2; }
-            hipLaunchKernelGGL(upsample2x_add_kernel<false>, GRID1D(n, BS), dim3(BS), 0, s, (const uint4*)p[0], (const uint4*)p[1], (uint4*)p[2], i[0], i[1], i[2], C8, i[4], (long)i[5], PRIO);
+            hipLaunchKernelGGL(upsample2x_add_kernel<false>, GRID1D(n, BS), dim3(BS), 0, s, (const uint4*)p[0], (const uint4*)p[1], (uint4*)p[2], i[0], i[1], i[2], C8, i[4], (long)i[5], PRIO, tc);
             break;
         }
         case CUTIE_OP_AREA_DOWN: {
@@ -1396,6 +1415,11 @@
             }
             a.rt = (op->flags >> 3) & 1;
             a.prio = PRIO;
+            if (op->f[0] != (float)(int)op->f[0] || op->f[1] != (float)(int)op->f[1] || !touch_range_ok(p[6], (long)op->f[0]) || !touch_range_ok(p[7], (long)op->f[1])) {
+                cutie_set_error("area_down3: a touch range (p6 / f0, p7 / f1) must be 16-byte aligned, its size a whole number >= 0");
+                return -2;
+            }
+            a.tc = touch_args(p[6], (long)op->f[0], p[7], (long)op->f[1]);
             hipLaunchKernelGGL(area_down3_kernel, GRID1D(total, BS), dim3(BS), 0, s, a);
             break;
         }
@@ -1421,15 +1445,17 @@
             if (i[2] > 256 || (i[2] & 7)) { cutie_set_error("eca: C <= 256, C %% 8"); return -2; }
             if (p[6] && (i[2] != 256 || !p[8])) { cutie_set_error("eca: the fused 1x1 head needs C = 256 and an output"); return -2; }
             int nchunk = (i[1] + 63) / 64;
+            if (!touch_range_ok(p[9], i[3]) || !touch_range_ok(p[10], i[4])) { cutie_set_error("eca: a touch range (p9 / i3, p10 / i4) must be 16-byte aligned, its size >= 0"); return -2; }
             hipLaunchKernelGGL(eca_apply_kernel, dim3((i[1] + 31) / 32, i[0]), dim3(256), 0, s, (const bf16_t*)p[0], (const float*)p[5], (const float*)p[2],
                                (const bf16_t*)p[3], (bf16_t*)p[4], (float*)p[1], i[1], i[2], nchunk, (op->flags & 1) ? (const long long*)p[5] : nullptr,
-                               (const bf16_t*)p[6], (const float*)p[7], (float*)p[8], PRIO);
+                               (const bf16_t*)p[6], (const float*)p[7], (float*)p[8], PRIO, touch_args(p[9], i[3], p[10], i[4]));
             break;
         }
         case CUTIE_OP_GRU: {
             long n = (long)i[0] * i[1];
+            if (!touch_range_ok(p[3], i[2]) || !touch_range_ok(p[4], i[3])) { cutie_set_error("gru: a touch range (p3 / i2, p4 / i3) must be 16-byte aligned, its size >= 0"); return -2; }
             if (!(op->flags & 1) && (i[1] & 3) == 0 && (((uintptr_t)p[0] | (uintptr_t)p[1]) & 15) == 0 && ((uintptr_t)p[2] & 7) == 0)
-                hipLaunchKernelGGL(gru4_kernel, GRID1D(n / 4, BS), dim3(BS), 0, s, (const float*)p[0], (float*)p[1], (bf16_t*)p[2], (long)i[0], i[1], PRIO);
+                hipLaunchKernelGGL(gru4_kernel, GRID1D(n / 4, BS), dim3(BS), 0, s, (const float*)p[0], (float*)p[1], (bf16_t*)p[2], (long)i[0], i[1], PRIO, touch_args(p[3], i[2], p[4], i[3]));
             else
                 hipLaunchKernelGGL(gru_kernel, GRID1D(n, BS), dim3(BS), 0, s, (const float*)p[0], (float*)p[1], (bf16_t*)p[2], (long)i[0], i[1]);
             break;
@@ -1465,8 +1491,10 @@
                 if (op->flags & 4) {
                     if (!vec || !p[3] || !p[4] || (i[1] & 3) || (i[2] & 3) || i[3] < 8 || (i[3] & 7)) { cutie_set_error("up4_softmax: the mask-down form needs P <= 8, h, w multiples of 4, m16 and pair"); return -2; }
                     const int ncell = (i[1] / 4) * (i[2] / 4);
+                    if (!touch_range_ok(p[5], i[6]) || !touch_range_ok(p[6], i[7])) { cutie_set_error("up4_softmax: a touch range (p5 / i6, p6 / i7) must be 16-byte aligned, its size >= 0"); return -2; }
+                    const TouchArgs tc = touch_args(p[5], i[6], p[6], i[7]);
 #define UP4_MD_(KC, SH) hipLaunchKernelGGL((up4_softmax_md_kernel<8, KC, SH>), dim3((ncell + 3) / 4, nclip), dim3(256), 0, s, (const float*)p[0], (float*)p[1], (float*)p[2], i[0] - 1, \
-                                       i[1], i[2], (float*)p[3], (uint4*)p[4], i[3] / 8, PRIO)
+                                       i[1], i[2], (float*)p[3], (uint4*)p[4], i[3] / 8, PRIO, tc)
 #define UP4_MD(KC) { if (op->flags & 16) UP4_MD_(KC, false); else UP4_MD_(KC, true); }
                     switch ((op->flags & 8) ? 0 : i[0] - 1) {
                         case 1: UP4_MD(1); break; case 2: UP4_MD(2); break; case 3: UP4_MD(3); break; case 4: UP4_MD(4); break;
diff --git a/cutie_amd/csrc/qchain.hip b/cutie_amd/csrc/qchain.hip
--- a/cutie_amd/csrc/qchain.hip
+++ b/cutie_amd/csrc/qchain.hip
@@ -136,7 +136,12 @@
 
 template <bool QPRE, bool ACC, int KT, int NW, bool MIXED = false>
 __global__ __launch_bounds__(NW * 64) void q2p_chain_kernel(QIn in, QOut out, const bf16_t* __restrict__ kv, const float* __restrict__ lg,
-                                                           int HW, int HWp, int ldkv, int voff, int hstride, const float* __restrict__ qpre, int Kg) {
+                                                           int HW, int HWp, int ldkv, int voff, int hstride, const float* __restrict__ qpre, int Kg, TouchArgs tc) {
+    if (blockIdx.x >= 8) {
+        const int ne = gridDim.x - 8;
+        touch_ranges(tc.a, tc.a_bytes, tc.b, tc.b_bytes, blockIdx.y * ne + (blockIdx.x - 8), ne * gridDim.y, threadIdx.x, NW * 64);
+        return;
+    }
     if (in.prio) __builtin_amdgcn_s_setprio(1);
     constexpr int Q = 16, NT = NW * 64;
     constexpr bool EARLY = KT > 0;
@@ -342,7 +347,7 @@
     ATL(6)
 }
 
-__global__ __launch_bounds__(512) void self_chain_kernel(QIn in, QOut out) {
+__global__ __launch_bounds__(512) void self_chain_kernel(QIn in, QOut out, TouchArgs tc) {
     if (in.prio) __builtin_amdgcn_s_setprio(1);
     __shared__ float sX[2][16 * PROJ_XLD];
     __shared__ f32x4 sRed[4][6][64];
@@ -428,11 +433,12 @@
         }
     }
     ATL(5)
+    touch_ranges(tc.a, tc.a_bytes, tc.b, tc.b_bytes, blockIdx.y * gridDim.x + blockIdx.x, gridDim.x * gridDim.y, threadIdx.x, 512);
 }
 
 struct QFfn { const bf16_t* W1; const float* b1; const bf16_t* W2; long long* acc; int FF; };
 template <int HS>
-__global__ __launch_bounds__(256) void qffn_kernel(QIn in, QFfn a) {
+__global__ __launch_bounds__(256) void qffn_kernel(QIn in, QFfn a, TouchArgs tc) {
     if (in.prio) __builtin_amdgcn_s_setprio(1);
     constexpr int T1 = HS / 64;
     constexpr int KS2 = HS / 32;
@@ -469,10 +475,11 @@
         for (int r = 0; r < 4; ++r) qacc_add(ap + r * 256, acc[r]);
     }
     ATL(3)
+    touch_ranges(tc.a, tc.a_bytes, tc.b, tc.b_bytes, blockIdx.y * gridDim.x + blockIdx.x, gridDim.x * gridDim.y, threadIdx.x, 256);
 }
 
 struct NextQ { const float* ln_g; const float* ln_b; const bf16_t* W; const float* bias; float* q_out; float* xn_out; };
-__global__ __launch_bounds__(256) void p2q_chain_kernel(QIn in, const bf16_t* __restrict__ q, bf16_t* __restrict__ y, int HW, int ldq, NextQ nq) {
+__global__ __launch_bounds__(256) void p2q_chain_kernel(QIn in, const bf16_t* __restrict__ q, bf16_t* __restrict__ y, int HW, int ldq, NextQ nq, TouchArgs tc) {
     if (in.prio) __builtin_amdgcn_s_setprio(1);
     constexpr int C = 256;
     __shared__ float sX[2][16 * PROJ_XLD];
@@ -481,6 +488,7 @@
     const int wave = threadIdx.x >> 6, lane = threadIdx.x & 63, c = lane & 15, g = lane >> 4;
     const int isv = wave >> 1, col = (wave & 1) * 16;
     const float scale = rsqrtf(32.f);
+    const int tlin = (blockIdx.z * gridDim.y + blockIdx.y) * gridDim.x + blockIdx.x, tnb = gridDim.x * gridDim.y * gridDim.z;
     ATL(0)
     if (nq.W && blockIdx.x == gridDim.x - 1) {
         QIn in2 = in;
@@ -500,6 +508,7 @@
 #pragma unroll
             for (int r = 0; r < 4; ++r) nq.q_out[((long)k * 16 + 4 * g + r) * C + hh * 32 + col + c] = (a[r] + b[r] + bv) * scale;
         }
+        touch_ranges(tc.a, tc.a_bytes, tc.b, tc.b_bytes, tlin, tnb, threadIdx.x, 256);
         return;
     }
     QRows<4> R;
@@ -527,7 +536,7 @@
     }
     QSYNC();
     ATL(2)
-    if (pbase >= HW) return;
+    if (pbase >= HW) { touch_ranges(tc.a, tc.a_bytes, tc.b, tc.b_bytes, tlin, tnb, threadIdx.x, 256); return; }
     float kf[8];
 #pragma unroll
     for (int j = 0; j < 8; ++j) kf[j] = ks[c][8 * g + j];
@@ -564,6 +573,7 @@
         }
     }
     ATL(3)
+    touch_ranges(tc.a, tc.a_bytes, tc.b, tc.b_bytes, tlin, tnb, threadIdx.x, 256);
 }
 
 #ifdef CUTIE_DIAG
@@ -761,10 +771,20 @@
     return true;
 }
 
+static bool qtouch_from_op(const cutie_op* op, const char* who, int pa, int ia, int pb, int ib, TouchArgs& tc) {
+    if (!touch_range_ok(op->p[pa], op->i[ia]) || !touch_range_ok(op->p[pb], op->i[ib])) {
+        cutie_set_error("%s: a touch range (p%d / i%d, p%d / i%d) must be 16-byte aligned, its size >= 0", who, pa, ia, pb, ib);
+        return false;
+    }
+    tc = touch_args(op->p[pa], op->i[ia], op->p[pb], op->i[ib]);
+    return true;
+}
+
 int launch_qchain(const cutie_op* op, hipStream_t s) {
     const int32_t* i = op->i;
     const uint64_t* p = op->p;
     QIn in; QOut out;
+    TouchArgs tc = {};
     switch (op->kind) {
         case CUTIE_OP_ATTN_Q2P: {
             if (i[1] != 16 || i[3] != 256 || i[4] != 8 || (i[7] > 0 && i[7] != 256)) { cutie_set_error("attn_q2p (chain form): Q = 16, C = 256, 8 heads, dense rows"); return -2; }
@@ -789,7 +809,7 @@
             const int kt = Kg <= 4 ? 1 : Kg <= 8 ? 2 : 0;
             const int var = mixed ? 9 + (qp ? 2 : ac ? 1 : 0) : (qp ? 6 : ac ? 3 : 0) + kt;
             constexpr int NWV = 8;
-            typedef void (*Kern)(QIn, QOut, const bf16_t*, const float*, int, int, int, int, int, const float*, int);
+            typedef void (*Kern)(QIn, QOut, const bf16_t*, const float*, int, int, int, int, int, const float*, int, TouchArgs);
             static const Kern kerns[12] = {
                 q2p_chain_kernel<false, false, 0, NWV>, q2p_chain_kernel<false, false, 4, NWV>, q2p_chain_kernel<false, false, 8, NWV>,
                 q2p_chain_kernel<false, true, 0, NWV>, q2p_chain_kernel<false, true, 4, NWV>, q2p_chain_kernel<false, true, 8, NWV>,
@@ -807,7 +827,14 @@
                 attr_set[var] = true;
             }
             const int hstride = i[8] > 0 ? i[8] : 32;
-            hipLaunchKernelGGL(kern, dim3(8, i[0]), dim3(NWV * 64), dyn, s, in, out, (const bf16_t*)p[1], (const float*)p[2], i[2], HWp, i[5], i[6], hstride, qpre, Kg);
+#ifdef ATT_TIMELINE
+            const int extra = 0;
+#else
+            if (!qtouch_from_op(op, "attn_q2p (chain form)", 14, 11, 15, 12, tc)) return -2;
+            const int extra = (tc.a_bytes > 0 || tc.b_bytes > 0) ? i[13] : 0;
+            if (extra < 0 || (extra & 7) || (long)(8 + extra) * i[0] > 4096) { cutie_set_error("attn_q2p (chain form): i13 = %d touch workgroups per object: a multiple of 8, (8 + i13) K <= 4096", i[13]); return -2; }
+#endif
+            hipLaunchKernelGGL(kern, dim3(8 + extra, i[0]), dim3(NWV * 64), dyn, s, in, out, (const bf16_t*)p[1], (const float*)p[2], i[2], HWp, i[5], i[6], hstride, qpre, Kg, tc);
             break;
         }
         case CUTIE_OP_ATTN_SELF:
@@ -815,7 +842,10 @@
             if ((op->flags & 14) != 14) { cutie_set_error("attn_self (chain form): flags 2 | 4 | 8 required"); return -2; }
             if (!qin_from_op(op, in, out, "attn_self", 0, 3)) return -2;
             if (!in.add || !in.ln_g || !in.ln_b || !in.bias || !in.abias) { cutie_set_error("attn_self (chain form): query embedding, LayerNorm and both biases are required"); return -2; }
-            hipLaunchKernelGGL(self_chain_kernel, dim3(8, i[0]), dim3(512), 0, s, in, out);
+#ifndef ATT_TIMELINE
+            if (!qtouch_from_op(op, "attn_self (chain form)", 14, 11, 15, 12, tc)) return -2;
+#endif
+            hipLaunchKernelGGL(self_chain_kernel, dim3(8, i[0]), dim3(512), 0, s, in, out, tc);
             break;
         case CUTIE_OP_ATTN_P2Q:
             if (i[1] != 16 || i[3] != 256 || i[4] != 8 || (i[7] > 0 && i[7] != 256)) { cutie_set_error("attn_p2q (chain form): Q = 16, C = 256, 8 heads, dense rows"); return -2; }
@@ -850,7 +880,8 @@
 #else
             if (op->flags & 32) { cutie_set_error("attn_p2q (flags&32: output projection inside): only in the diagnostic library (make DIAG=1)"); return -2; }
 #endif
-            hipLaunchKernelGGL(p2q_chain_kernel, dim3((i[2] + 255) / 256 + (nq.W ? 1 : 0), 8, i[0]), dim3(256), 0, s, in, (const bf16_t*)p[0], (bf16_t*)p[3], i[2], i[5], nq);
+            if (!qtouch_from_op(op, "attn_p2q (chain form)", 2, 9, 4, 10, tc)) return -2;
+            hipLaunchKernelGGL(p2q_chain_kernel, dim3((i[2] + 255) / 256 + (nq.W ? 1 : 0), 8, i[0]), dim3(256), 0, s, in, (const bf16_t*)p[0], (bf16_t*)p[3], i[2], i[5], nq, tc);
         }
             break;
         case CUTIE_OP_QFFN: {
@@ -868,8 +899,9 @@
             in.tl = (unsigned long long*)p[15];
 #endif
             QFfn a = {(const bf16_t*)p[4], (const float*)p[5], (const bf16_t*)p[6], (long long*)p[7], i[1]};
-            if (HS == 64) hipLaunchKernelGGL(qffn_kernel<64>, dim3(i[1] / 64, i[0] / 16), dim3(256), 0, s, in, a);
-            else hipLaunchKernelGGL(qffn_kernel<128>, dim3(i[1] / 128, i[0] / 16), dim3(256), 0, s, in, a);
+            if (!qtouch_from_op(op, "qffn", 8, 3, 9, 4, tc)) return -2;
+            if (HS == 64) hipLaunchKernelGGL(qffn_kernel<64>, dim3(i[1] / 64, i[0] / 16), dim3(256), 0, s, in, a, tc);
+            else hipLaunchKernelGGL(qffn_kernel<128>, dim3(i[1] / 128, i[0] / 16), dim3(256), 0, s, in, a, tc);
             break;
         }
         default:
diff --git a/cutie_amd/model/cutie.py b/cutie_amd/model/cutie.py
--- a/cutie_amd/model/cutie.py
+++ b/cutie_amd/model/cutie.py
@@ -128,6 +128,15 @@
                 W[q + ln + '.bias'] = sd[q + ln + '.bias'].to(dev).contiguous()
             W[q + '.ffn.linear1'] = pack_linear(sd[q + '.ffn.linear1.weight'], sd[q + '.ffn.linear1.bias'], dev)
             W[q + '.ffn.linear2'] = pack_linear(sd[q + '.ffn.linear2.weight'], sd[q + '.ffn.linear2.bias'], dev)
+        chain = [f'{t}.blocks.{b}{s}' for b in range(ot['num_blocks']) for s in ('.read_from_pixel.q', '.read_from_pixel.out', '.self_attn.qkv',
+                                                                                 '.self_attn.out', '.ffn.linear1', '.ffn.linear2', '.read_from_query.kv')]
+        if chain and all(W[n].weight.numel() % 8 == 0 for n in chain):
+            blob = torch.cat([W[n].weight.reshape(-1) for n in chain])
+            off = 0
+            for n in chain:
+                k = W[n].weight.numel()
+                W[n].weight = blob[off:off + k].view(W[n].weight.shape)
+                off += k
         conv(t + '.pixel_init_proj')
         for b in range(ot['num_blocks'] + 1):
             conv(f'{t}.mask_pred.{b}.1')
@@ -196,6 +205,7 @@
         e.__dict__.pop('_query_bufs', None)
         e.__dict__.pop('_md_bufs', None)
         e.__dict__.pop('_qinit_state', None)
+        e.__dict__.pop('_chain_prev', None)
         return e
 
     def plan(self, key, builder, *args):
@@ -209,7 +219,14 @@
                 arenas[kind] = plans.Arena(self.device)
             p.pack_into(arenas[kind])
             self._plans[key] = p
+        if key[0] in self.CHAIN_PLANS:
+            prev = self.__dict__.get('_chain_prev')
+            if prev is not None and prev is not p:
+                prev.then(p)
+            self._chain_prev = p
         return p
+
+    CHAIN_PLANS = frozenset(('fuse', 'rq', 'seg', 'emask', 'ls_fuse', 'ls_rq', 'ls_seg', 'ls_emask'))
 
 
 class _Container(nn.Module):
diff --git a/cutie_amd/model/plans.py b/cutie_amd/model/plans.py
--- a/cutie_amd/model/plans.py
+++ b/cutie_amd/model/plans.py
@@ -255,6 +255,18 @@
             self.bufs[name] = self.arena.tensor[off:off + n].view(dtype).view(shape)
 
     graph_head = 0
+
+    def then(self, nxt):
+        if self.__dict__.get('_then') is nxt:
+            return
+        self._then = nxt
+        ol = self.ol
+        head = nxt.ol.head_ranges() if ol.touch_next_weights else ()
+        if tuple(ol.next_head) == tuple(head):
+            return
+        ol.next_head = tuple(head)
+        if ol.arr is not None:
+            ol.wire_next_weights()
 
     def run(self, **dyn):
         if not self.tuned:
diff --git a/cutie_amd/ops.py b/cutie_amd/ops.py
--- a/cutie_amd/ops.py
+++ b/cutie_amd/ops.py
@@ -104,6 +104,8 @@
 NUM_CU = 256
 WEIGHT_PREFETCH = int(os.environ.get('CUTIE_AMD_WPF', str(8 << 20)))
 WEIGHT_PREFETCH_BLOCK = int(os.environ.get('CUTIE_AMD_WPF_BLOCK', str(48 << 10)))
+WEIGHT_PREFETCH_CHAIN = os.environ.get('CUTIE_AMD_WPF_CHAIN', '0') not in ('', '0')
+TOUCH_OFF = frozenset(s for s in os.environ.get('CUTIE_AMD_WPF_OFF', '').split(',') if s)
 
 
 COUT1_TILE = 19
@@ -314,6 +316,10 @@
         self.recs = []
         self.keep = []
         self.wbytes = {}
+        self.wranges = {}
+        self.next_head = ()
+        self.touchers = {}
+        self.untouched = {}
         self.dyn = {}
         self.arr = None
         self._words = None
@@ -335,6 +341,15 @@
         self.arr = self._words = None
         return idx
 
+    @staticmethod
+    def _wb(w):
+        t = getattr(w, 'weight', w)
+        return t.numel() * t.element_size()
+
+    def _weights(self, idx, *slots):
+        self.wranges[idx] = [(slot, self._wb(w)) for slot, w in slots if w is not None]
+        return idx
+
     def finalize(self):
         arr = np.zeros(len(self.recs), dtype=OP_DTYPE)
         for n, (kind, flags, ints, floats, ptrs) in enumerate(self.recs):
@@ -348,14 +363,136 @@
         self.wire_next_weights()
         return arr
 
+    TOUCH_SLOTS = {CONV: ((9, 'i', 22), (10, 'i', 23)), UPSAMPLE2X_ADD: ((3, 'i', 7), (4, 'i', 8)), ECA_APPLY: ((9, 'i', 3), (10, 'i', 4)),
+                   GRU: ((3, 'i', 2), (4, 'i', 3)), AREA_DOWN3: ((6, 'f', 0), (7, 'f', 1)), UP4_SOFTMAX: ((5, 'i', 6), (6, 'i', 7)),
+                   ATTN_Q2P: ((14, 'i', 11), (15, 'i', 12)), ATTN_SELF: ((14, 'i', 11), (15, 'i', 12)), QFFN: ((8, 'i', 3), (9, 'i', 4)),
+                   ATTN_P2Q: ((2, 'i', 9), (4, 'i', 10))}
+
+    @staticmethod
+    def q2p_touch_groups(K):
+        return max(0, ((NUM_CU // max(K, 1) - 8) // 8) * 8)
+
+    def touch_blocks(self, n):
+        arr = self.arr
+        kind, fl, i = int(arr['kind'][n]), int(arr['flags'][n]), [int(v) for v in arr['i'][n]]
+        if kind == CONV:
+            return pc_blocks(i[17], i[0], i[7], i[8], i[9]) if i[17] in PC_TILES else 0
+        if not WEIGHT_PREFETCH_CHAIN or KIND_NAMES.get(kind) in TOUCH_OFF:
+            return 0
+        if kind == UPSAMPLE2X_ADD:
+            return -(-(i[0] * 4 * i[1] * i[2] * (i[3] // 8)) // 256)
+        if kind == ECA_APPLY:
+            return -(-i[1] // 32) * i[0]
+        if kind == GRU:
+            return -(-(i[0] * i[1] // 4) // 256) if not (fl & 1) and i[1] % 4 == 0 else 0
+        if kind == AREA_DOWN3:
+            total = 0
+            for q in range(3):
+                B, H, W, C, _, _, r, _ = i[8 * q:8 * q + 8]
+                total += B * (H // r) * (W // r) * (1 if (fl >> q) & 1 else C // 8)
+            return -(-total // 256)
+        if kind == UP4_SOFTMAX:
+            return -(-((i[1] // 4) * (i[2] // 4)) // 4) * max(i[4], 1) if (fl & 5) == 5 and not i[5] else 0
+        if kind == ATTN_Q2P:
+            return self.q2p_touch_groups(i[0]) * i[0] if (fl & 8) else 0
+        if kind == ATTN_SELF:
+            return 8 * i[0] if (fl & 8) else 0
+        if kind == QFFN:
+            return (i[1] // (i[2] or 64)) * (i[0] // 16)
+        if kind == ATTN_P2Q:
+            return (-(-i[2] // 256) + (1 if fl & 16 else 0)) * 8 * i[0] if (fl & 4) and not (fl & 32) else 0
+        return 0
+
+    def weight_ranges(self, n):
+        out = []
+        for slot, nbytes in self.wranges.get(n, ()):
+            ptr = int(self.arr['p'][n, slot])
+            if not ptr or nbytes <= 0:
+                continue
+            if out and out[-1][0] + out[-1][1] == ptr:
+                out[-1] = (out[-1][0], out[-1][1] + nbytes)
+            else:
+                out.append((ptr, nbytes))
+        return out
+
+    def head_ranges(self):
+        if self.arr is None:
+            self.finalize()
+        first = min(self.wranges) if self.wranges else None
+        if first is None or not (WEIGHT_PREFETCH and WEIGHT_PREFETCH_CHAIN and self.touch_next_weights) or 'RING' in TOUCH_OFF:
+            return ()
+        if any(self.touch_blocks(n) for n in range(first)):
+            return ()
+        return tuple(self.weight_ranges(first))
+
+    def _clear_touch(self):
+        arr = self.arr
+        for kind, slots in self.TOUCH_SLOTS.items():
+            rows = np.nonzero(arr['kind'] == kind)[0]
+            if kind in (ATTN_Q2P, ATTN_SELF, ATTN_P2Q):
+                rows = [n for n in rows if int(arr['flags'][n]) & (4 if kind == ATTN_P2Q else 8) and not (kind == ATTN_P2Q and int(arr['flags'][n]) & 32)]
+            for n in rows:
+                for ps, fld, ix in slots:
+                    arr['p'][n, ps] = 0
+                    arr[fld][n, ix] = 0
+                if kind == ATTN_Q2P:
+                    arr['i'][n, 13] = 0
+
     def wire_next_weights(self):
         arr = self.arr
-        convs = [n for n in range(len(arr)) if arr['kind'][n] == CONV]
-        for n in convs:
-            arr['p'][n, 9:11] = 0
-            arr['i'][n, 22:24] = 0
+        self._clear_touch()
+        self.touchers, self.untouched = {}, {}
         if not (WEIGHT_PREFETCH and self.touch_next_weights):
             return
+        if not WEIGHT_PREFETCH_CHAIN:
+            return self._wire_convs()
+        N = len(arr)
+        targets = sorted(n for n in self.wranges if self.weight_ranges(n))
+        ranges = {n: self.weight_ranges(n) for n in targets}
+        if self.next_head:
+            targets.append(N)
+            ranges[N] = list(self.next_head)
+        blocks = {n: self.touch_blocks(n) for n in range(N) if int(arr['kind'][n]) in self.TOUCH_SLOTS}
+        left = {n: WEIGHT_PREFETCH_BLOCK * -(-b // 8) for n, b in blocks.items() if b > 0}
+        used = {n: 0 for n in left}
+        pc = lambda n: n >= 0 and int(arr['kind'][n]) == CONV and n in left
+
+        def stretch(lo, hi):
+            c = [n for n in range(hi - 1, max(lo, 0) - 1, -1) if n in left and used[n] < 2 and left[n] > 0]
+            if lo in c and pc(lo) and hi < N:
+                c.remove(lo)
+                c.insert(0, lo)
+            return c
+        for k, t in enumerate(targets):
+            lo = targets[k - 1] if k else 0
+            for ptr, nbytes in ranges[t]:
+                near = stretch(lo, t)
+                best = near[0] if near else None
+                if k and (best is None or (not pc(best) and left[best] < nbytes)):
+                    far = [n for n in stretch(targets[k - 2] if k > 1 else 0, lo) if best is None or left[n] > left[best]]
+                    best = far[0] if far else best
+                if best is None:
+                    self.untouched[t] = ('the first launch of its list' if not k and not any(b > 0 for n, b in blocks.items() if n < t)
+                                         else 'no launch between it and the two weight-carrying launches in front can touch (or has a slot and budget left)')
+                    continue
+                take = min(nbytes, WEIGHT_PREFETCH, left[best])
+                ps, fld, ix = self.TOUCH_SLOTS[int(arr['kind'][best])][used[best]]
+                arr['p'][best, ps], arr[fld][best, ix] = ptr, take
+                used[best] += 1
+                left[best] -= take
+                self.touchers.setdefault(t, []).append((best, ptr, take))
+                if take < nbytes:
+                    self.untouched[t] = 'the budget of its toucher covers only the head of its weights'
+        for n in left:
+            if int(arr['kind'][n]) == ATTN_Q2P and used[n]:
+                K = int(arr['i'][n, 0])
+                total = WEIGHT_PREFETCH_BLOCK * -(-blocks[n] // 8) - left[n]
+                per_xcd = -(-total // WEIGHT_PREFETCH_BLOCK)
+                arr['i'][n, 13] = min(self.q2p_touch_groups(K), 8 * -(-per_xcd // K))
+
+    def _wire_convs(self):
+        arr = self.arr
+        convs = [n for n in range(len(arr)) if arr['kind'][n] == CONV]
         nxt, nxt2 = None, None
         for n in reversed(convs):
             i = arr['i'][n]
@@ -431,6 +568,7 @@
             assert (tile in DMA_TILES or tile in PC_TILES) and not out_f32 and w.cout % 8 == 0 and ldy % 8 == 0, 'GAP accumulation needs an LDS-DMA conv (see conv_side_jobs_ok)'
         part = splitk_scratch(w.weight.device, self.scratch_owner)
         self.wbytes[len(self.recs)] = w.weight.numel() * w.weight.element_size()
+        self.wranges[len(self.recs)] = [(2, self.wbytes[len(self.recs)])]
         return self.add(CONV, flags,
                         [B, H, W, C1, C2, ldx1, ldx2, OH, OW, w.cout, ldy, w.kh, w.kw, stride, pad, ldr, w.kpad, tile, w.cin_real,
                          splitk, part.numel() // 1024, 0 if zero is None else zero.numel()],
@@ -559,8 +697,8 @@
             nb = zero.numel() * zero.element_size()
             assert nb % 16 == 0 and zero.is_contiguous()
             nz = nb // 16
-        return self.add(QUERY_INIT, 1, [rows, 256, nz], [], [obj_mem, query, query_emb, w_init.weight, w_init.bias, res_init,
-                                                             w_emb.weight, w_emb.bias, res_emb, zero])
+        return self._weights(self.add(QUERY_INIT, 1, [rows, 256, nz], [], [obj_mem, query, query_emb, w_init.weight, w_init.bias, res_init,
+                                                                           w_emb.weight, w_emb.bias, res_emb, zero]), (3, w_init), (6, w_emb))
 
     def aux_mask(self, logits, fg, nfg, *, K, HW):
         self.memset32(nfg, K, 0)
@@ -601,7 +739,7 @@
             assert proj is None and acc_in is None and out_proj is not None and logits is not None
             flags, ints, ptrs = self._proj_extras(3 | 16, [K, Q, HW, C, heads, ldkv, voff, 256], [q_pre, kv, logits, None, None], None, out_proj)
             ints[8] = hs
-            return self.add(ATTN_Q2P, flags, ints + [kg] + mixed, [], ptrs)
+            return self._weights(self.add(ATTN_Q2P, flags, ints + [kg] + mixed, [], ptrs), (12, out_proj[0]))
         if proj is not None:
             assert logits is not None
             ldx, ln_out, tail = self._proj(proj)
@@ -609,7 +747,7 @@
             flags, ints, ptrs = self._proj_extras(3, [K, Q, HW, C, heads, ldkv, voff, ldx], [proj['x'], kv, logits, ln_out, y] + tail, acc_in, out_proj)
             assert hs == 0 or out_proj is not None, 'a head stride needs the chain form'
             ints[8] = hs
-            return self.add(ATTN_Q2P, flags, ints + [kg] + mixed, [], ptrs)
+            return self._weights(self.add(ATTN_Q2P, flags, ints + [kg] + mixed, [], ptrs), (5, proj['W']), (12, out_proj[0] if out_proj is not None else None))
         assert acc_in is None and out_proj is None
         if logits is not None:
             return self.add(ATTN_Q2P, 1, [K, Q, HW, C, heads, ldkv, voff], [], [q, kv, logits, None, y])
@@ -620,7 +758,7 @@
             ldx, ln_out, tail = self._proj(proj)
             assert out_proj is not None or acc_in is None, 'the chain form of ATTN_SELF needs out_proj'
             flags, ints, ptrs = self._proj_extras(2, [K, Q, C, heads, 0, 0, ldx], [proj['x'], None, y, ln_out, None] + tail, acc_in, out_proj)
-            return self.add(ATTN_SELF, flags, ints, [], ptrs)
+            return self._weights(self.add(ATTN_SELF, flags, ints, [], ptrs), (5, proj['W']), (12, out_proj[0] if out_proj is not None else None))
         assert acc_in is None and out_proj is None
         return self.add(ATTN_SELF, 0, [K, Q, C, heads, ldqk, ldv], [], [qk, v, y])
 
@@ -638,7 +776,7 @@
                 ptrs = ptrs + [None] * (16 - len(ptrs))
                 ptrs[8], ptrs[9] = next_q['ln']
                 ptrs[12], ptrs[13], ptrs[14], ptrs[15] = next_q['W'].weight, next_q['W'].bias, next_q['q_out'], next_q['xn_out']
-            return self.add(ATTN_P2Q, flags, ints, [], ptrs)
+            return self._weights(self.add(ATTN_P2Q, flags, ints, [], ptrs), (5, proj['W']), (12, next_q['W'] if next_q is not None else None))
         assert acc_in is None
         return self.add(ATTN_P2Q, 0, [K, Q, HW, C, heads, ldq, ldkv], [], [q, kq, vq, y])
 
@@ -651,7 +789,7 @@
         if acc_in is not None:
             assert acc_in[0].dtype == torch.int64
             ptrs[10], ptrs[11] = acc_in[0], acc_in[1]
-        return self.add(QFFN, 0, ints, [], ptrs)
+        return self._weights(self.add(QFFN, 0, ints, [], ptrs), (4, W1), (6, W2))
 
     def summarize(self, feat, wl, m16, y, *, K, HW, C, Q, scratch=None, feat_f32=False, ldf=None, ldw=None):
         if scratch is None:
```

After: 1169, median of 3. No clear change (+0.1%).
